# microsoft/tf2-gnn

Measured on AMD Instinct MI355X. Metric: edges/sec (fwd+bwd) RGCN H=320 L=4, PPI-shaped batch, 1/2/4/8 MI355X, higher is better.
Workload: dtype f32; 1 GPU; rmat30k: V=30000 E=900000 per GPU (one batch per rank, replicas) edge_types=4 D=320 H=320 layers=4 RGCN (PPI_RGCN.json stack settings), step = edge bucketing of the next batch (2nd stream, overlapped) + forward (training mode) + f...

## Files before the change

include/tfgnn.h:

```cpp
#ifndef TFGNN_H
#define TFGNN_H

#include <stddef.h>
#include <stdint.h>

#ifdef __cplusplus
extern "C" {
#endif

typedef enum {
  TFGNN_OK = 0,
  TFGNN_ERR_INVALID_ARGUMENT = -1,
  TFGNN_ERR_OUT_OF_RANGE = -2,
  TFGNN_ERR_HIP = -3,
  TFGNN_ERR_UNSUPPORTED = -4
} tfgnn_status;

typedef enum {
  TFGNN_ACT_NONE = 0,
  TFGNN_ACT_RELU = 1,
  TFGNN_ACT_TANH = 2,
  TFGNN_ACT_LEAKY_RELU = 3,
  TFGNN_ACT_ELU = 4,
  TFGNN_ACT_SELU = 5,
// ... 2 lines not shown
} tfgnn_activation;

typedef enum {
  TFGNN_REDUCE_SUM = 0,
  TFGNN_REDUCE_MAX = 1
} tfgnn_reduce;

const char* tfgnn_last_error(void);
const char* tfgnn_version(void);
#define TFGNN_ABI_VERSION 5
int tfgnn_abi_version(void);

typedef enum {
  TFGNN_KFAM_GEMM_FP32 = 0,
  TFGNN_KFAM_GEMM_BF16X3 = 1,
  TFGNN_KFAM_SP_NT = 2,
  TFGNN_KFAM_SP_TN = 3,
  TFGNN_KFAM_GATHER_SP = 4,
  TFGNN_KFAM_GATHER = 5,
  TFGNN_KFAM_FUSED_NT = 6,
  TFGNN_KFAM_GEMM_STREAM = 7,
  TFGNN_KFAM_STREAM_F16X2 = 8,
  TFGNN_KFAM_COUNT = 9
} tfgnn_kernel_family;
int tfgnn_launch_counts(int64_t* out_counts, int n);

typedef struct tfgnn_graph tfgnn_graph;

int tfgnn_graph_create(int num_edge_types, int64_t num_nodes, const int32_t* const* d_adjacency,
                       const int64_t* num_edges, void* stream, tfgnn_graph** out_graph);
int tfgnn_graph_destroy(tfgnn_graph* graph);
int tfgnn_graph_create_async(int num_edge_types, int64_t num_nodes, const int32_t* const* d_adjacency,
                             const int64_t* num_edges, void* stream, tfgnn_graph** out_graph);
int tfgnn_graph_wait(tfgnn_graph* graph);
int tfgnn_graph_destroy_async(tfgnn_graph* graph, void* last_use_stream);

typedef enum {
  TFGNN_GRAPH_PART_PLAN_TYPED = 1,
  TFGNN_GRAPH_PART_PLAN_NODE = 2,
  TFGNN_GRAPH_PART_COMPACT = 4,
  TFGNN_GRAPH_PART_EDGE_MAPS = 8,
  TFGNN_GRAPH_PART_EDGE_IDS = 16,
  TFGNN_GRAPH_PART_DST_PATTERN = 32,
  TFGNN_GRAPH_PARTS_DEFAULT = 31,
  TFGNN_GRAPH_PARTS_ALL = 63
} tfgnn_graph_part;
int tfgnn_graph_create_parts_async(int num_edge_types, int64_t num_nodes, const int32_t* const* d_adjacency,
                                   const int64_t* num_edges, unsigned parts, void* stream, tfgnn_graph** out_graph);
int tfgnn_graph_ensure(tfgnn_graph* graph, unsigned parts, void* stream);
unsigned tfgnn_graph_parts(const tfgnn_graph* graph);

typedef enum {
  TFGNN_G_ROWPTR_BY_DST = 0,
  TFGNN_G_COL_BY_DST = 1,
  TFGNN_G_EID_BY_DST = 2,
  TFGNN_G_COLL_BY_DST = 3,
  TFGNN_G_ROWPTR_BY_SRC = 4,
  TFGNN_G_COL_BY_SRC = 5,
  TFGNN_G_EID_BY_SRC = 6,
  TFGNN_G_COLL_BY_SRC = 7,
  TFGNN_G_INVDEG_BY_DST = 8,
  TFGNN_G_INVDEG_EDGE_BY_SRC = 9,
  TFGNN_G_NODEPTR_BY_DST = 10,
  TFGNN_G_NODEPTR_BY_SRC = 11,
  TFGNN_G_INVDEG_EDGE_BY_DST = 12,
  TFGNN_G_SRC2DST_POS = 13,
  TFGNN_G_TARGET_BY_DST = 14,
  TFGNN_G_NZ_CPOS_BY_DST = 15,
  TFGNN_G_NZ_ROW_BY_DST = 16,
  TFGNN_G_NZ_NODE_BY_DST = 17,
  TFGNN_G_NZ_OFF_BY_DST = 18,
  TFGNN_G_NZ_NODEPTR_BY_DST = 19,
  TFGNN_G_NZ_COL_BY_DST = 20,
  TFGNN_G_NZ_CPOS_BY_SRC = 21,
  TFGNN_G_NZ_ROW_BY_SRC = 22,
  TFGNN_G_NZ_NODE_BY_SRC = 23,
  TFGNN_G_NZ_OFF_BY_SRC = 24,
  TFGNN_G_NZ_NODEPTR_BY_SRC = 25,
  TFGNN_G_NZ_COL_BY_SRC = 26,
  TFGNN_G_PATTERN_POS_BY_DST = 27,
  TFGNN_G_PATTERN_NODE_BY_DST = 28,
  TFGNN_G_PATTERN_TILEMASK_BY_DST = 29,
  TFGNN_G_PATTERN_NODE_BY_SRC = 30,
  TFGNN_G_PATTERN_TILEMASK_BY_SRC = 31
} tfgnn_graph_array_id;

int tfgnn_graph_array(const tfgnn_graph* graph, int array_id, const void** d_ptr, int64_t* count);
int tfgnn_graph_nonempty_offsets(const tfgnn_graph* graph, int by_src, int32_t* h_offsets);
int tfgnn_graph_dims(const tfgnn_graph* graph, int64_t* num_nodes, int* num_edge_types,
                     int64_t* num_edges);

int tfgnn_graph_scales(const tfgnn_graph* graph, int normalize_by_num_incoming, int aggregation_mode,
                       float* d_row_scale, float* d_node_scale, float* d_edge_weight_by_src,
                       float* d_edge_weight_by_dst, void* stream);

int tfgnn_graph_target_multiplier(const tfgnn_graph* graph, const float* d_row_scale, float* d_k,
                                  int32_t* d_ident_ptr, int32_t* d_node_of_row, void* stream);

int tfgnn_csr_gather_reduce(const int32_t* d_rowptr, const int32_t* d_col,
                            const float* d_edge_weight, const float* d_row_scale,
                            int64_t num_rows, const float* d_in, int64_t ld_in, int width,
                            float* d_out, int64_t ld_out, int reduce_op, int pre_act, int post_act,
                            void* stream);

typedef enum {
  TFGNN_VIEW_BY_DST_TYPED = 0,
  TFGNN_VIEW_BY_DST_NODE = 1,
  TFGNN_VIEW_BY_SRC_TYPED = 2,
  TFGNN_VIEW_BY_SRC_NODE = 3,
  TFGNN_VIEW_BY_DST_TYPED_COMPACT = 4,
  TFGNN_VIEW_BY_SRC_TYPED_COMPACT = 5,
  TFGNN_VIEW_BY_DST_TYPED_PATTERN = 6
} tfgnn_graph_view;
size_t tfgnn_graph_gather_workspace_bytes(const tfgnn_graph* graph, int view, int width);
int tfgnn_graph_gather_reduce(const tfgnn_graph* graph, int view, const int32_t* d_col_override,
                              const float* d_edge_weight, int ew_heads, const float* d_row_scale,
                              const float* d_in, int64_t ld_in, int width, float* d_out, int64_t ld_out,
                              int reduce_op, int pre_act, int post_act, void* d_workspace,
                              size_t workspace_bytes, void* stream);

int tfgnn_edge_pair_combine(const int32_t* d_index_a, const int32_t* d_index_b, const float* d_P,
                            const float* d_Q, int64_t num_edges, int width, int act, float* d_out,
                            void* stream);

int tfgnn_film_edge_forward(const float* d_msg, const int32_t* d_msg_row, const float* d_film, const int32_t* d_film_row,
                            const float* d_edge_weight, int64_t num_edges, int width, float* d_out, void* stream);
int tfgnn_film_edge_backward(const float* d_grad, const float* d_msg, const int32_t* d_msg_row, const float* d_film,
                             const int32_t* d_film_row, const float* d_edge_weight, int64_t num_edges, int width,
                             float* d_grad_msg, float* d_grad_film, void* stream);

int tfgnn_edge_aggregate_backward(int64_t num_edges, int64_t width, const float* d_msg, int64_t ld_msg,
                                  const int32_t* d_msg_row, const int32_t* d_target, const float* d_edge_weight,
                                  const float* d_node_scale, int pre_act, int reduce_op, const float* d_grad_agg,
                                  const float* d_agg_max, const float* d_num_selected, int phase, float* d_out,
                                  void* stream);

int tfgnn_film_combine_forward(const float* d_Z, const float* d_film, const int32_t* d_rowptr_typed,
                               const float* d_node_scale, int64_t num_nodes, int num_edge_types, int64_t hidden,
                               int act, float* d_pre, float* d_out, void* stream);
int tfgnn_film_combine_backward(const float* d_grad_pre, const float* d_Z, const float* d_film,
                                const int32_t* d_rowptr_typed, const float* d_node_scale, int64_t num_nodes,
                                int num_edge_types, int64_t hidden, float* d_dZ, float* d_dfilm, void* stream);

int tfgnn_batch_offset_edges(const int32_t* d_local_edges, int64_t num_edges, const int32_t* d_edge_ptr,
                             const int32_t* d_node_ptr, int num_graphs, int32_t* d_out, int* d_bad_flag, void* stream);
int tfgnn_batch_node_to_graph_map(const int32_t* d_node_ptr, int num_graphs, int64_t num_nodes, int32_t* d_out,
                                  void* stream);
int tfgnn_adjacency_append(const int32_t* d_edges, int64_t num_edges, int flip, int32_t* d_out, void* stream);
int tfgnn_adjacency_self_loops(int64_t num_nodes, int32_t* d_out, void* stream);
int tfgnn_adjacency_in_degrees(const int32_t* d_edges, int64_t num_edges, int64_t num_nodes, float* d_counts,
                               void* stream);
int tfgnn_graph_original_order(const tfgnn_graph* graph, const float* d_weight_by_dst, int32_t* d_src_l,
                               int32_t* d_tgt_l, int32_t* d_tgt_node, float* d_weight, void* stream);

size_t tfgnn_gemm_workspace_bytes(int64_t M, int64_t N, int64_t K);
int tfgnn_gemm(int trans_a, int trans_b, int64_t M, int64_t N, int64_t K, const float* d_A,
               int64_t lda, const float* d_B, int64_t ldb, float* d_C, int64_t ldc,
               const float* d_bias, int act, int accumulate, void* d_workspace,
               size_t workspace_bytes, void* stream);

enum { TFGNN_GEMM_FP32 = 0, TFGNN_GEMM_F16X2 = 3, TFGNN_GEMM_BF16X3 = 6, TFGNN_GEMM_BF16X3_EXACT = 9 };
int tfgnn_gemm_set_mode(int mode);
int tfgnn_gemm_get_mode(void);

int tfgnn_gemm_grad_epilogue(int trans_a, int trans_b, int64_t M, int64_t N, int64_t K, const float* d_A,
                             int64_t lda, const float* d_B, int64_t ldb, float* d_C, int64_t ldc,
                             const float* d_mul, int64_t ld_mul, int act_of_saved, const float* d_saved,
// ... 422 lines not shown
```

tf2_gnn_amd/csrc/aux_jobs.hip:

```cpp
#include <algorithm>

#include "aux_jobs.hpp"

namespace tfgnn {

constexpr int AUX_MAX_JOBS = 8;
struct AuxJobTable {
  tfgnn_aux_job j[AUX_MAX_JOBS];
  int n;
};

typedef const __attribute__((address_space(4))) tfgnn_aux_job* aux_job_cptr;

template <class P>
__device__ __forceinline__ P aux_payload(aux_job_cptr j) {
  constexpr int W = (int)((sizeof(P) + 7) / 8);
  union {
    P p;
    unsigned long long w[W];
  } u;
  const __attribute__((address_space(4))) unsigned long long* src =
      (const __attribute__((address_space(4))) unsigned long long*)&j->payload[0];
#pragma unroll
  for (int i = 0; i < W; ++i) u.w[i] = src[i];
  return u.p;
}

__global__ void __launch_bounds__(256) aux_jobs_kernel(AuxJobTable table) {
  aux_job_cptr jobs = (aux_job_cptr)__builtin_amdgcn_kernarg_segment_ptr();
  unsigned b = blockIdx.x;
  int k = 0;
  const int n = table.n;
  while (k < n - 1 && b >= jobs[k].num_blocks) {
    b -= jobs[k].num_blocks;
    ++k;
  }
  aux_job_cptr j = jobs + k;
  const unsigned nb = j->num_blocks;
  if (b >= nb) return;
  switch (j->kind) {
    case AUX_SPLIT_ROWS: {
      const AuxSplitRows a = aux_payload<AuxSplitRows>(j);
      sp_split_rows_body(a.src, a.ld, a.seg_len, a.seg_stride, a.R, a.C, a.sb, a.dst, a.ld_dst, a.inv, a.fixed_inv, b);
      break;
    }
    case AUX_SPLIT_COLS: {
      const AuxSplitCols a = aux_payload<AuxSplitCols>(j);
      sp_split_cols_body(a.src, a.ld, a.K, a.N, a.dst, a.ld_dst, a.inv, b % a.ncx, b / a.ncx, a.ncy, a.colmax_parts, a.nparts);
      break;
    }
    case AUX_COL_ABSMAX: {
      const AuxColAbsmax a = aux_payload<AuxColAbsmax>(j);
      col_absmax_body(a, b);
      break;
    }
    case AUX_COMBINE_SP: {
      const AuxCombineSp a = aux_payload<AuxCombineSp>(j);
      combine_sp_body(a, b);
      break;
    }
    default:
      break;
  }
}

}

extern "C" int tfgnn_aux_launch(const tfgnn_aux_job* jobs, int num_jobs, void* stream) {
  using namespace tfgnn;
  TFGNN_REQUIRE(num_jobs >= 0 && (num_jobs == 0 || jobs != nullptr), "tfgnn_aux_launch: bad arguments");
  int i = 0;
  while (i < num_jobs) {
    AuxJobTable t{};
    uint64_t blocks = 0;
    while (i < num_jobs && t.n < AUX_MAX_JOBS) {
      const tfgnn_aux_job& j = jobs[i++];
      if (j.kind == AUX_NONE || j.num_blocks == 0) continue;
      TFGNN_REQUIRE(j.kind == AUX_SPLIT_ROWS || j.kind == AUX_SPLIT_COLS || j.kind == AUX_COMBINE_SP || j.kind == AUX_COL_ABSMAX,
                    "tfgnn_aux_launch: unknown job kind %d", j.kind);
      t.j[t.n++] = j;
      blocks += j.num_blocks;
    }
    if (t.n == 0) continue;
    TFGNN_REQUIRE(blocks < (1ull << 31), "tfgnn_aux_launch: too many workgroups");
    hipLaunchKernelGGL(aux_jobs_kernel, dim3((unsigned)blocks), dim3(256), 0, (hipStream_t)stream, t);
    TFGNN_LAUNCH_CHECK();
  }
  return TFGNN_OK;
}
```

tf2_gnn_amd/csrc/aux_jobs.hpp:

```cpp
#pragma once
#include <hip/hip_runtime.h>

#include <cstdint>

#include "common.hpp"
#include "sp16.hpp"
#include "tfgnn.h"

namespace tfgnn {

enum AuxKind { AUX_NONE = 0, AUX_SPLIT_ROWS = 1, AUX_SPLIT_COLS = 2, AUX_COMBINE_SP = 4, AUX_COL_ABSMAX = 6 };

struct AuxSplitRows {
  const float* src;
  int64_t ld, seg_len, seg_stride, R, C;
  int sb;
  uint8_t* dst;
  int64_t ld_dst;
  float* inv;
  const float* fixed_inv;
};
struct AuxSplitCols {
  const float* src;
  int64_t ld, K, N;
  uint8_t* dst;
  int64_t ld_dst;
  float* inv;
  unsigned ncx, ncy;
  const float* colmax_parts;
  int nparts;
};
struct AuxColAbsmax {
  const float* src;
  int64_t ld, K, N;
  float* part;
  int nparts;
  unsigned nchunks;
};
static_assert(sizeof(AuxColAbsmax) <= sizeof(((tfgnn_aux_job*)0)->payload), "tfgnn_aux_job payload too small");
struct AuxTnReduce {
  const float* partial;
  int splits;
  int64_t M, N;
  const float* ref;
  int64_t a_col0;
  int a_sb;
  float* C;
  int64_t group_rows, stride_group, stride_row, stride_col;
  int accumulate;
  int64_t slab;
  int ref_ld;
};
struct AuxCombineSp {
  const int32_t *multi_row, *multi_base, *multi_n;
  int num_multi;
  const float* row_scale;
  const float* partial;
  int width;
  const int32_t* out_row_map;
  uint8_t* out_sp;
  int64_t ld_out_sp;
  float* inv_out;
  const float* fixed_inv;
};
static_assert(sizeof(AuxSplitRows) <= sizeof(((tfgnn_aux_job*)0)->payload) && sizeof(AuxSplitCols) <= sizeof(((tfgnn_aux_job*)0)->payload) &&
                  sizeof(AuxCombineSp) <= sizeof(((tfgnn_aux_job*)0)->payload),
              "tfgnn_aux_job payload too small");

template <class P>
static inline void aux_job_set(tfgnn_aux_job* j, int kind, unsigned blocks, const P& p) {
  j->kind = kind;
  j->num_blocks = blocks;
  memset(j->payload, 0, sizeof(j->payload));
  memcpy(j->payload, &p, sizeof(P));
}

__device__ __forceinline__ void sp_split_rows_body(const float* __restrict__ src, int64_t ld, int64_t seg_len,
                                                   int64_t seg_stride, int64_t R, int64_t C, int sb,
                                                   uint8_t* __restrict__ dst, int64_t ld_dst, float* __restrict__ inv,
                                                   const float* __restrict__ fixed_inv, unsigned block) {
  const int lane = threadIdx.x & 63;
  const int nblk = (int)(C / sb);
  const int64_t item = (int64_t)block * 4 + (threadIdx.x >> 6);
  if (item >= R * nblk) return;
  const int64_t r = item / nblk;
  const int blk = (int)(item - r * nblk);
  const float* srow = src + r * ld;
  const int64_t c0 = (int64_t)blk * sb;
  float s, iv;
  if (fixed_inv) {
    iv = fixed_inv[0];
    s = 1.f / iv;
  } else {
    float mx = 0.f;
    for (int c = lane * 4; c < sb; c += 256) {
      const int64_t cc = c0 + c;
      const int64_t sg = cc / seg_len;
      const float4 v = *reinterpret_cast<const float4*>(srow + sg * seg_stride + (cc - sg * seg_len));
      mx = fmaxf(mx, fmaxf(fmaxf(fabsf(v.x), fabsf(v.y)), fmaxf(fabsf(v.z), fabsf(v.w))));
    }
    for (int o = 32; o; o >>= 1) mx = fmaxf(mx, __shfl_xor(mx, o, 64));
    s = sp_scale_for_max(mx, &iv);
  }
  if (inv && lane == 0) inv[item] = iv;
  uint8_t* drow = dst + r * ld_dst;
  for (int c = lane * 4; c < sb; c += 256) {
    const int64_t cc = c0 + c;
    const int64_t sg = cc / seg_len;
    const float4 v = *reinterpret_cast<const float4*>(srow + sg * seg_stride + (cc - sg * seg_len));
    sp_store4(drow, cc, v, s);
  }
}

__device__ __forceinline__ void col_absmax_body(const AuxColAbsmax& a, unsigned block) {
  const unsigned s = block / a.nchunks, chunk = block - s * a.nchunks;
  const int64_t per = (a.K + a.nparts - 1) / a.nparts;
  const int64_t k0 = (int64_t)s * per, k1 = k0 + per < a.K ? k0 + per : a.K;
  const int64_t c = ((int64_t)chunk * 256 + threadIdx.x) * 4;
  if (c >= a.N) return;
  const float* p = a.src + c;
  float4 mx = {0.f, 0.f, 0.f, 0.f};
  int64_t k = k0;
  for (; k + 8 <= k1; k += 8) {
    float4 v[8];
#pragma unroll
    for (int u = 0; u < 8; ++u) v[u] = *reinterpret_cast<const float4*>(p + (k + u) * a.ld);
#pragma unroll
    for (int u = 0; u < 8; ++u) {
      mx.x = fmaxf(mx.x, fabsf(v[u].x)); mx.y = fmaxf(mx.y, fabsf(v[u].y));
      mx.z = fmaxf(mx.z, fabsf(v[u].z)); mx.w = fmaxf(mx.w, fabsf(v[u].w));
    }
  }
  for (; k < k1; ++k) {
    const float4 v = *reinterpret_cast<const float4*>(p + k * a.ld);
    mx.x = fmaxf(mx.x, fabsf(v.x)); mx.y = fmaxf(mx.y, fabsf(v.y));
    mx.z = fmaxf(mx.z, fabsf(v.z)); mx.w = fmaxf(mx.w, fabsf(v.w));
  }
  *reinterpret_cast<float4*>(a.part + (int64_t)s * a.N + c) = mx;
}

__device__ __forceinline__ void sp_split_cols_body(const float* __restrict__ src, int64_t ld, int64_t K, int64_t N,
                                                   uint8_t* __restrict__ dst, int64_t ld_dst, float* __restrict__ inv,
                                                   unsigned bx, unsigned by, unsigned ny, const float* __restrict__ colmax_parts = nullptr,
                                                   int nparts = 0) {
  __shared__ float red[64][4];
  __shared__ float tile[2][16][65];
  __shared__ float sc[16];
  const int tid = threadIdx.x;
  const int64_t n0 = (int64_t)bx * 16;
// ... 45 lines not shown
    float* r = &red[(tid >> 6) * 4 + (tid & 3)][0];
    r[0] = mx.x; r[1] = mx.y; r[2] = mx.z; r[3] = mx.w;
  }
  __syncthreads();
  if (tid < 16) {
    float m = 0.f;
#pragma unroll
    for (int w = 0; w < 4; ++w) m = fmaxf(m, red[w * 4 + (tid >> 2)][tid & 3]);
    float iv;
    sc[tid] = sp_scale_for_max(m, &iv);
    if (inv && by == 0 && n0 + tid < N) inv[n0 + tid] = iv;
  }
  __syncthreads();
  const int64_t kper = (((K + ny - 1) / ny) + 63) & ~63ll;
  const int64_t kend = (by + 1) * kper < K ? (by + 1) * kper : K;
  const int rr = tid >> 4, k4 = (tid & 15) * 4;
  if (in_regs) {
    const int i0 = (int)((by * kper) >> 6), i1 = (int)((kend + 63) >> 6);
#pragma unroll
    for (int i = 0; i < NV; ++i) {
      if (i >= i0 && i < i1) {
        float (*t)[65] = tile[i & 1];
        t[nq + 0][kq] = v[i].x; t[nq + 1][kq] = v[i].y; t[nq + 2][kq] = v[i].z; t[nq + 3][kq] = v[i].w;
        __syncthreads();
        const int64_t kb = (int64_t)i * 64;
        if (n0 + rr < N && kb + k4 < K) {
          const float4 o = {t[rr][k4], t[rr][k4 + 1], t[rr][k4 + 2], t[rr][k4 + 3]};
          sp_store4(dst + (n0 + rr) * ld_dst, kb + k4, o, sc[rr]);
        }
      }
    }
    return;
  }
  for (int64_t kb = by * kper; kb < kend; kb += 64) {
    const int64_t k = kb + kq;
    float4 w4 = {0.f, 0.f, 0.f, 0.f};
    if (ok && k < K) w4 = *reinterpret_cast<const float4*>(src + k * ld + n0 + nq);
    tile[0][nq + 0][kq] = w4.x; tile[0][nq + 1][kq] = w4.y; tile[0][nq + 2][kq] = w4.z; tile[0][nq + 3][kq] = w4.w;
    __syncthreads();
    if (n0 + rr < N && kb + k4 < K) {
      const float4 o = {tile[0][rr][k4], tile[0][rr][k4 + 1], tile[0][rr][k4 + 2], tile[0][rr][k4 + 3]};
      sp_store4(dst + (n0 + rr) * ld_dst, kb + k4, o, sc[rr]);
    }
    __syncthreads();
  }
}

__device__ __forceinline__ void sp_tn_reduce_body(const AuxTnReduce& a, unsigned block, unsigned nblocks) {
  const int64_t total = a.M * a.N;
  for (int64_t i = (int64_t)block * 256 + threadIdx.x; i < total; i += (int64_t)nblocks * 256) {
    const int64_t m = i / a.N, n = i - m * a.N;
    const int64_t blk = (a.a_col0 + m) / a.a_sb;
    float s = 0.f;
    int z = 0;
    if (a.ref_ld > 0) {
      for (; z + 8 <= a.splits; z += 8) {
        float v[8], r[8];
#pragma unroll
        for (int u = 0; u < 8; ++u) {
          v[u] = a.partial[(int64_t)(z + u) * a.slab + i];
          r[u] = a.ref[(int64_t)(z + u) * a.ref_ld + blk];
        }
#pragma unroll
        for (int u = 0; u < 8; ++u) s += v[u] * r[u];
      }
      for (; z < a.splits; ++z) s += a.partial[(int64_t)z * a.slab + i] * a.ref[(int64_t)z * a.ref_ld + blk];
    } else {
      for (; z + 8 <= a.splits; z += 8) {
        float v[8];
#pragma unroll
        for (int u = 0; u < 8; ++u) v[u] = a.partial[(int64_t)(z + u) * a.slab + i];
#pragma unroll
        for (int u = 0; u < 8; ++u) s += v[u];
      }
      for (; z < a.splits; ++z) s += a.partial[(int64_t)z * a.slab + i];
      s *= a.ref[blk];
    }
    const int64_t gi = m / a.group_rows, mi = m - gi * a.group_rows;
    float* dst = a.C + gi * a.stride_group + mi * a.stride_row + n * a.stride_col;
    *dst = a.accumulate ? *dst + s : s;
  }
}

__device__ __forceinline__ void combine_sp_body(const AuxCombineSp& a, unsigned block) {
  const int m = (int)block * 4 + (threadIdx.x >> 6);
  if (m >= a.num_multi) return;
  const int lane = threadIdx.x & 63;
  const int64_t row = a.multi_row[m];
  const int32_t base = a.multi_base[m], n = a.multi_n[m];
  const float rs = a.row_scale ? a.row_scale[row] : 1.f;
  float4 sum[8];
  float mx = 0.f;
#pragma unroll
  for (int i = 0; i < 8; ++i) {
    const int c = (lane + i * 64) * 4;
    sum[i] = make_float4(0.f, 0.f, 0.f, 0.f);
    if (c < a.width) {
      int k = 0;
      for (; k + 4 <= n; k += 4) {
        float4 p[4];
#pragma unroll
        for (int u = 0; u < 4; ++u) p[u] = *reinterpret_cast<const float4*>(a.partial + (int64_t)(base + k + u) * a.width + c);
#pragma unroll
        for (int u = 0; u < 4; ++u) { sum[i].x += p[u].x; sum[i].y += p[u].y; sum[i].z += p[u].z; sum[i].w += p[u].w; }
      }
      for (; k < n; ++k) {
        const float4 p = *reinterpret_cast<const float4*>(a.partial + (int64_t)(base + k) * a.width + c);
        sum[i].x += p.x; sum[i].y += p.y; sum[i].z += p.z; sum[i].w += p.w;
      }
      sum[i].x *= rs; sum[i].y *= rs; sum[i].z *= rs; sum[i].w *= rs;
      mx = fmaxf(mx, fmaxf(fmaxf(fabsf(sum[i].x), fabsf(sum[i].y)), fmaxf(fabsf(sum[i].z), fabsf(sum[i].w))));
    }
  }
  const int64_t orow = a.out_row_map ? a.out_row_map[row] : row;
  float iv, sc;
  if (a.fixed_inv) {
    iv = a.fixed_inv[0];
    sc = 1.f / iv;
  } else {
#pragma unroll
    for (int o = 32; o; o >>= 1) mx = fmaxf(mx, __shfl_xor(mx, o, 64));
    sc = sp_scale_for_max(mx, &iv);
    if (lane == 0) a.inv_out[orow] = iv;
  }
  uint8_t* drow = a.out_sp + orow * a.ld_out_sp;
#pragma unroll
  for (int i = 0; i < 8; ++i) {
    const int c = (lane + i * 64) * 4;
    if (c < a.width) sp_store4(drow, c, sum[i], sc);
  }
}

}
```

tf2_gnn_amd/csrc/graph.hip:

```cpp
#include <algorithm>
#include <cstdlib>
#include <mutex>
#include <vector>

#include "common.hpp"
#include "graph.hpp"

namespace tfgnn {

static thread_local char g_err[512] = "";

void set_error(const char* fmt, ...) {
  va_list ap;
  va_start(ap, fmt);
  vsnprintf(g_err, sizeof(g_err), fmt, ap);
  va_end(ap);
}

static int64_t g_launch_counts[TFGNN_KFAM_COUNT] = {0};
void count_launch(int family) {
  if (family >= 0 && family < TFGNN_KFAM_COUNT) __atomic_fetch_add(&g_launch_counts[family], 1, __ATOMIC_RELAXED);
}

}
// ... 243 lines not shown
    if (valid && rank == 0) mine_base[d] = mine_base[d] + cnt;
    __builtin_amdgcn_wave_barrier();
  }
  __syncthreads();
  int32_t tot = 0, before = 0;
  {
    const int32_t* __restrict__ row = hist + (int64_t)(side * RS_RADIX + tid) * nblk_ld;
    const int me = (int)blockIdx.x;
    for (int b0 = 0; b0 < nblk; b0 += 16) {
      int4 v[4];
#pragma unroll
      for (int u = 0; u < 4; ++u)
        v[u] = b0 + 4 * u < nblk ? *reinterpret_cast<const int4*>(row + b0 + 4 * u) : make_int4(0, 0, 0, 0);
#pragma unroll
      for (int u = 0; u < 4; ++u) {
        const int b = b0 + 4 * u;
        const int e[4] = {v[u].x, v[u].y, v[u].z, v[u].w};
#pragma unroll
        for (int k = 0; k < 4; ++k)
          if (b + k < nblk) {
            tot += e[k];
            if (b + k < me) before += e[k];
          }
      }
    }
  }
  int32_t incl = tot;
#pragma unroll
  for (int o = 1; o < 64; o <<= 1) {
    const int32_t t = __shfl_up(incl, o, 64);
    if (lane >= o) incl += t;
  }
  if (lane == 63) wtot[wave] = incl;
  __syncthreads();
  {
    int32_t off = 0;
    for (int w = 0; w < wave; ++w) off += wtot[w];
    int32_t running = off + incl - tot + before;
#pragma unroll
    for (int w = 0; w < RS_WAVES; ++w) {
      const int32_t c = wbase[w][tid];
      wbase[w][tid] = running;
      running += c;
    }
  }
  __syncthreads();
#pragma unroll
  for (int r = 0; r < RS_ROUNDS; ++r) {
    const bool valid = (info[r] >> 16) & 1;
    const int d = (int)((key[r] >> shift) & (RS_RADIX - 1));
    const int rank = info[r] & 255, cnt = (info[r] >> 8) & 255;
    const int32_t b = valid ? mine_base[d] : 0;
    __builtin_amdgcn_wave_barrier();
    if (valid && rank == 0) mine_base[d] = b + cnt;
    __builtin_amdgcn_wave_barrier();
    if (valid) {
      kout[b + rank] = key[r];
      if (PAY) pout[b + rank] = pl[r];
    }
  }
}

template <typename KeyT>
__global__ void rowptr_from_sorted_kernel(const KeyT* __restrict__ comp_d, const KeyT* __restrict__ comp_s, int64_t E,
                                          int sec_bits, int64_t R, int32_t* __restrict__ rowptr_d,
                                          int32_t* __restrict__ rowptr_s) {
  const KeyT* __restrict__ comp = blockIdx.y ? comp_s : comp_d;
  int32_t* __restrict__ rowptr = blockIdx.y ? rowptr_s : rowptr_d;
  for (int64_t r = (int64_t)blockIdx.x * blockDim.x + threadIdx.x; r <= R; r += (int64_t)gridDim.x * blockDim.x) {
    int64_t lo = 0, hi = E;
    while (lo < hi) {
      const int64_t mid = (lo + hi) >> 1;
      if ((int64_t)((uint64_t)comp[mid] >> sec_bits) < r) lo = mid + 1; else hi = mid;
    }
    rowptr[r] = (int32_t)lo;
  }
}

struct PlanJob {
  const int32_t* rowptr;
  int64_t R;
  int thr, chunk;
  int32_t* counters;
  int32_t *item_row, *item_chunk, *item_slot, *multi_row, *multi_base, *multi_n;
  int32_t *bin_count, *bin_cursor, *short_rows;
  int want_items;
};
struct PlanJobs {
  PlanJob j[2];
};

__device__ __forceinline__ void plan_rows_body(const int32_t* __restrict__ rowptr, int64_t R, int long_threshold, int chunk_edges,
                                 int32_t* __restrict__ counters,
                                 int32_t* __restrict__ item_row, int32_t* __restrict__ item_chunk,
                                 int32_t* __restrict__ item_slot, int32_t* __restrict__ multi_row,
                                 int32_t* __restrict__ multi_base, int32_t* __restrict__ multi_n) {
  for (int64_t r = (int64_t)blockIdx.x * blockDim.x + threadIdx.x; r < R; r += (int64_t)gridDim.x * blockDim.x) {
    const int32_t len = rowptr[r + 1] - rowptr[r];
    if (len <= long_threshold) continue;
    const int32_t n = (len + chunk_edges - 1) / chunk_edges;
    const int32_t base = atomicAdd(&counters[0], n);
    int32_t pb = -1;
    if (n > 1) {
      const int32_t m = atomicAdd(&counters[1], 1);
      pb = atomicAdd(&counters[2], n);
      multi_row[m] = (int32_t)r;
      multi_base[m] = pb;
      multi_n[m] = n;
    }
    for (int32_t i = 0; i < n; ++i) {
      item_row[base + i] = (int32_t)r;
      item_chunk[base + i] = i;
      item_slot[base + i] = n > 1 ? pb + i : -1;
    }
  }
}

__device__ __forceinline__ void
short_hist_body(const int32_t* __restrict__ rowptr, int64_t R, int thr, int32_t* __restrict__ bin_count,
                int32_t* __restrict__ num_short, int* h, int& n_short) {
  for (int i = threadIdx.x; i <= thr; i += 256) h[i] = 0;
  if (threadIdx.x == 0) n_short = 0;
  __syncthreads();
  int mine = 0;
  for (int64_t r = (int64_t)blockIdx.x * blockDim.x + threadIdx.x; r < R; r += (int64_t)gridDim.x * blockDim.x) {
    const int32_t len = rowptr[r + 1] - rowptr[r];
    if (len <= thr) {
      atomicAdd(&h[len], 1);
      ++mine;
    }
  }
  if (mine) atomicAdd(&n_short, mine);
  __syncthreads();
  for (int i = threadIdx.x; i <= thr; i += 256)
    if (h[i]) atomicAdd(&bin_count[i], h[i]);
  if (threadIdx.x == 0 && n_short) atomicAdd(num_short, n_short);
}

__global__ void __launch_bounds__(256) plan_hist_kernel(PlanJobs jobs) {
  __shared__ int h[SHORT_BINS];
  __shared__ int n_short;
  const PlanJob& j = jobs.j[blockIdx.y & 1];
  if (j.R <= 0) return;
  if ((blockIdx.y >> 1) == 0) {
    short_hist_body(j.rowptr, j.R, j.thr, j.bin_count, j.counters + 3, h, n_short);
  } else if (j.want_items) {
    plan_rows_body(j.rowptr, j.R, j.thr, j.chunk, j.counters, j.item_row, j.item_chunk, j.item_slot, j.multi_row, j.multi_base,
                   j.multi_n);
  }
}

constexpr int SHORT_TILE_ROWS = 8;
__global__ void __launch_bounds__(256) short_scatter_kernel(PlanJobs jobs) {
  __shared__ int h[SHORT_BINS], base[SHORT_BINS], start[SHORT_BINS];
  const PlanJob& j = jobs.j[blockIdx.y];
  const int32_t* __restrict__ rowptr = j.rowptr;
  const int64_t R = j.R;
  const int thr = j.thr;
  const int32_t* __restrict__ bin_count = j.bin_count;
  int32_t* __restrict__ bin_cursor = j.bin_cursor;
  int32_t* __restrict__ short_rows = j.short_rows;
  if (R <= 0) return;
  if (threadIdx.x == 0) {
    int acc = 0;
    for (int i = thr; i >= 0; --i) {
      start[i] = acc;
      acc += bin_count[i];
    }
  }
  constexpr int TILE = 256 * SHORT_TILE_ROWS;
  for (int64_t tile = blockIdx.x; tile * TILE < R; tile += gridDim.x) {
    for (int i = threadIdx.x; i <= thr; i += 256) h[i] = 0;
    __syncthreads();
    int32_t len[SHORT_TILE_ROWS];
    int rank[SHORT_TILE_ROWS];
#pragma unroll
    for (int k = 0; k < SHORT_TILE_ROWS; ++k) {
      const int64_t r = tile * TILE + k * 256 + threadIdx.x;
      len[k] = r < R ? rowptr[r + 1] - rowptr[r] : -1;
      rank[k] = (len[k] >= 0 && len[k] <= thr) ? atomicAdd(&h[len[k]], 1) : 0;
    }
    __syncthreads();
    for (int i = threadIdx.x; i <= thr; i += 256)
      if (h[i]) base[i] = atomicAdd(&bin_cursor[i], h[i]);
    __syncthreads();
#pragma unroll
    for (int k = 0; k < SHORT_TILE_ROWS; ++k)
      if (len[k] >= 0 && len[k] <= thr)
        short_rows[start[len[k]] + base[len[k]] + rank[k]] = (int32_t)(tile * TILE + k * 256 + threadIdx.x);
    __syncthreads();
  }
}

__global__ void nz_flags_kernel(const int32_t* __restrict__ rowptr, int64_t V, int L, int32_t* __restrict__ flags,
                                int32_t* __restrict__ node_cnt) {
  const int64_t R = V * L;
  for (int64_t i = (int64_t)blockIdx.x * blockDim.x + threadIdx.x; i <= R; i += (int64_t)gridDim.x * blockDim.x) {
    if (i < R) {
      const int64_t l = i / V, v = i - l * V;
      const int64_t r = v * L + l;
      flags[i] = rowptr[r + 1] > rowptr[r] ? 1 : 0;
    } else {
      flags[i] = 0;
    }
    if (i <= V) {
      int32_t c = 0;
      if (i < V)
        for (int l = 0; l < L; ++l) c += rowptr[i * L + l + 1] > rowptr[i * L + l] ? 1 : 0;
      node_cnt[i] = c;
    }
  }
}

__global__ void nz_fill_kernel(const int32_t* __restrict__ rowptr, const int32_t* __restrict__ scan_t, int64_t V,
                               int L, int32_t* __restrict__ cpos, int32_t* __restrict__ nzrow,
                               int32_t* __restrict__ nz_node, int32_t* __restrict__ nz_off) {
  const int64_t R = V * L;
  for (int64_t i = (int64_t)blockIdx.x * blockDim.x + threadIdx.x; i < R; i += (int64_t)gridDim.x * blockDim.x) {
    const int64_t l = i / V, v = i - l * V;
    const int64_t r = v * L + l;
    const int32_t c = scan_t[i];
    if (rowptr[r + 1] > rowptr[r]) {
      cpos[r] = c;
      nzrow[c] = (int32_t)r;
      nz_node[c] = (int32_t)v;
    } else {
      cpos[r] = -1;
    }
    if (v == 0) nz_off[l] = c;
    if (i == R - 1) nz_off[L] = scan_t[R];
  }
// ... 179 lines not shown
  }
  {
    std::lock_guard<std::mutex> lock(g_pool_mutex);
    if (g_dev_pool.size() < POOL_MAX_ENTRIES) {
      g_dev_pool.push_back({p, bytes, ev});
      return;
    }
  }
  if (ev) (void)hipEventDestroy(ev);
  (void)hipFree(p);
}
static hipError_t pinned_alloc(void** p, size_t bytes, size_t* got) {
  if (bytes < 4096) bytes = 4096;
  *p = pool_take(g_pinned_pool, bytes, got, nullptr);
  if (*p) return hipSuccess;
  *got = bytes;
  return hipHostMalloc(p, bytes, hipHostMallocDefault);
}
static void pinned_release(void* p, size_t bytes) {
  if (!p) return;
  {
    std::lock_guard<std::mutex> lock(g_pool_mutex);
    if (g_pinned_pool.size() < POOL_MAX_ENTRIES) {
      g_pinned_pool.push_back({p, bytes, nullptr});
      return;
    }
  }
  (void)hipHostFree(p);
}
}

namespace {
struct SlabPlan {
  size_t total = 0;
  size_t take(size_t bytes) {
    size_t off = total;
    total += (bytes + 255) & ~(size_t)255;
    return off;
  }
};
}

static void graph_release_all(tfgnn_graph* g, hipStream_t last_use = nullptr, bool in_use = false) {
  using namespace tfgnn;
  if (!g) return;
  if (g->event) (void)hipEventDestroy((hipEvent_t)g->event);
  dev_release(g->scratch, g->scratch_bytes, last_use, in_use);
  dev_release(g->slab, g->slab_bytes, last_use, in_use);
  pinned_release(g->pinned, g->pinned_bytes);
  delete g;
}

namespace {
using namespace tfgnn;

constexpr unsigned kPartsAll = TFGNN_GRAPH_PART_PLAN_TYPED | TFGNN_GRAPH_PART_PLAN_NODE | TFGNN_GRAPH_PART_COMPACT |
                               TFGNN_GRAPH_PART_EDGE_MAPS | TFGNN_GRAPH_PART_EDGE_IDS | TFGNN_GRAPH_PART_DST_PATTERN;

void view_plan_parameters(int view_long[4], int view_chunk[4]) {
  const int dl[4] = {LONG_ROW_THRESHOLD_TYPED, LONG_ROW_THRESHOLD, LONG_ROW_THRESHOLD_TYPED, LONG_ROW_THRESHOLD};
  const int dc[4] = {ITEM_CHUNK_TYPED, ITEM_CHUNK, ITEM_CHUNK_TYPED, ITEM_CHUNK};
  for (int v = 0; v < 4; ++v) {
    view_long[v] = dl[v];
    view_chunk[v] = dc[v];
    if (view_long[v] > SHORT_BINS - 1) view_long[v] = SHORT_BINS - 1;
    if (view_chunk[v] < view_long[v]) view_chunk[v] = view_long[v];
  }
}

unsigned blocks_for(int64_t n) { return (unsigned)std::max<int64_t>(1, std::min<int64_t>(ceil_div(n, 256), 8192)); }

int build_plans(tfgnn_graph* g, int node_views, int32_t* counters, int32_t* bins, hipStream_t s) {
  PlanJobs jobs{};
  int64_t max_rows = 0;
  for (int k = 0; k < 2; ++k) {
    const int v = 2 * k + node_views;
    CsrPlan& pl = g->views[v].plan;
    PlanJob& j = jobs.j[k];
    j.rowptr = g->views[v].rowptr;
    j.R = g->views[v].num_rows;
    j.thr = pl.long_threshold;
    j.chunk = pl.item_chunk_edges;
    j.counters = counters + 16 + 4 * v;
    j.item_row = pl.item_row; j.item_chunk = pl.item_chunk; j.item_slot = pl.item_slot;
    j.multi_row = pl.multi_row; j.multi_base = pl.multi_base; j.multi_n = pl.multi_n;
    j.bin_count = bins + (size_t)v * 2 * SHORT_BINS;
    j.bin_cursor = j.bin_count + SHORT_BINS;
    j.short_rows = pl.short_rows;
    j.want_items = g->E > 0;
    max_rows = std::max(max_rows, j.R);
  }
  if (max_rows <= 0) return TFGNN_OK;
  hipLaunchKernelGGL(plan_hist_kernel, dim3(blocks_for(max_rows), 4), dim3(256), 0, s, jobs);
  TFGNN_LAUNCH_CHECK();
  const unsigned scat_blocks = (unsigned)std::min<int64_t>(ceil_div(max_rows, 256 * SHORT_TILE_ROWS), 4096);
  hipLaunchKernelGGL(short_scatter_kernel, dim3(scat_blocks, 2), dim3(256), 0, s, jobs);
  TFGNN_LAUNCH_CHECK();
  return TFGNN_OK;
}

size_t compact_scratch_bytes(int64_t R, int64_t V) {
  return (size_t)(R + 2) * 4 + 256 + (scan_scratch_elems(R + 1) + scan_scratch_elems(V + 1)) * 4 + 64;
}

int build_compact(tfgnn_graph* g, char* scratch, hipStream_t s) {
  const int L = g->L;
  const int64_t V = g->V, R = g->R;
  int32_t* flags = (int32_t*)scratch;
  int32_t* scan_tmp = (int32_t*)(scratch + (((size_t)(R + 2) * 4 + 255) & ~(size_t)255));
  for (int side = 0; side < 2; ++side) {
    CompactBuckets& cb = g->compact[side];
    const int32_t* rp = side == 0 ? g->rowptr_d : g->rowptr_s;
    if (L > 0) {
      hipLaunchKernelGGL(nz_flags_kernel, dim3(blocks_for(R + 1)), dim3(256), 0, s, rp, V, L, flags, cb.nodeptr_nz);
      int rc = exclusive_scan_i32(flags, flags, R + 1, scan_tmp, s);
      if (rc) return rc;
      rc = exclusive_scan_i32(cb.nodeptr_nz, cb.nodeptr_nz, V + 1, scan_tmp, s);
      if (rc) return rc;
      if (R > 0) {
        hipLaunchKernelGGL(nz_fill_kernel, dim3(blocks_for(R)), dim3(256), 0, s, rp, flags, V, L, cb.cpos, cb.nzrow,
                           cb.nz_node, cb.nz_off);
        hipLaunchKernelGGL(nz_cols_kernel, dim3(blocks_for(V)), dim3(256), 0, s, cb.cpos, cb.nodeptr_nz, V, L, cb.col_nz);
      } else {
        TFGNN_HIP_CHECK(hipMemsetAsync(cb.nz_off, 0, (size_t)(L + 1) * 4, s));
      }
    } else {
      TFGNN_HIP_CHECK(hipMemsetAsync(cb.nz_off, 0, (size_t)(L + 1) * 4, s));
      TFGNN_HIP_CHECK(hipMemsetAsync(cb.nodeptr_nz, 0, (V + 1) * 4, s));
    }
    TFGNN_HIP_CHECK(hipMemcpyAsync((char*)g->pinned + 256 + (size_t)(L + 1) * 16 + (size_t)side * (L + 1) * 4, cb.nz_off,
                                   (size_t)(L + 1) * 4, hipMemcpyDeviceToHost, s));
  }
  TFGNN_LAUNCH_CHECK();
  return TFGNN_OK;
}

int build_dst_pattern(tfgnn_graph* g, int32_t* pat, hipStream_t s) {
  if (g->V <= 0 || g->L <= 0 || g->L > 8) return TFGNN_OK;
  const unsigned blocks = (unsigned)std::min<int64_t>(ceil_div(g->V, 256), 1024);
  hipLaunchKernelGGL(pattern_count_kernel, dim3(blocks), dim3(256), 0, s, (const int32_t*)g->rowptr_d, g->V, g->L, pat);
  hipLaunchKernelGGL(pattern_place_kernel, dim3(blocks), dim3(256), 0, s, (const int32_t*)g->rowptr_d, g->V, g->L, (const int32_t*)pat,
                     pat + 256, g->pat_pos_d, g->pat_node_d, g->pat_rowmap_d);
  hipLaunchKernelGGL(pattern_tilemask_kernel, dim3((unsigned)ceil_div(g->V, 128)), dim3(128), 0, s, (const int32_t*)g->rowptr_d,
                     (const int32_t*)g->pat_node_d, g->V, g->L, g->pat_tilemask_d);
  int32_t* pat_s = pat + 512;
  hipLaunchKernelGGL(pattern_count_kernel, dim3(blocks), dim3(256), 0, s, (const int32_t*)g->rowptr_s, g->V, g->L, pat_s);
  hipLaunchKernelGGL(pattern_place_kernel, dim3(blocks), dim3(256), 0, s, (const int32_t*)g->rowptr_s, g->V, g->L, (const int32_t*)pat_s,
                     pat_s + 256, (int32_t*)nullptr, g->pat_node_s, (int32_t*)nullptr);
  hipLaunchKernelGGL(pattern_tilemask_kernel, dim3((unsigned)ceil_div(g->V, 128)), dim3(128), 0, s, (const int32_t*)g->rowptr_s,
                     (const int32_t*)g->pat_node_s, g->V, g->L, g->pat_tilemask_s);
  TFGNN_LAUNCH_CHECK();
  return TFGNN_OK;
}

int build_edge_maps(tfgnn_graph* g, hipStream_t s) {
  if (g->E > 0) {
    hipLaunchKernelGGL(src2dst_kernel, dim3(blocks_for(g->E)), dim3(256), 0, s, g->eid_s, g->eid2pos, g->E, g->src2dst, g->dst2src);
    TFGNN_LAUNCH_CHECK();
  }
  return TFGNN_OK;
}

template <typename KeyT, bool PAY>
int build_core(tfgnn_graph* g, const EdgeLists& el, char* keys, char* pays, int32_t* hist, int nblk, int nblk_ld,
               int32_t* counters, hipStream_t s) {
  const int64_t E = g->E, R = g->R, V = g->V;
  const int L = g->L;
  const int sec_bits = g->sec_bits, total_bits = g->total_bits;
// ... 58 lines not shown
    for (int l = 0; l < EL_INLINE; ++l) el.adj_v[l] = l < L ? g->h_adj[l] : nullptr;
    for (int l = 0; l <= EL_INLINE; ++l) el.off_v[l] = l <= L ? g->h_off[l] : g->E;
  } else {
    const int32_t** d_ptrs = (const int32_t**)(scratch + cs.ptrs);
    int64_t* d_off = (int64_t*)(scratch + cs.off);
    char* hp = (char*)g->pinned + 256;
    const int32_t** h_ptrs = (const int32_t**)hp;
    int64_t* h_off = (int64_t*)(hp + (size_t)(L + 1) * 8);
    for (int l = 0; l < L; ++l) h_ptrs[l] = g->h_adj[l];
    for (int l = 0; l <= L; ++l) h_off[l] = g->h_off[l];
    TFGNN_HIP_CHECK(hipMemcpyAsync(d_ptrs, h_ptrs, (size_t)L * 8, hipMemcpyHostToDevice, s));
    TFGNN_HIP_CHECK(hipMemcpyAsync(d_off, h_off, (size_t)(L + 1) * 8, hipMemcpyHostToDevice, s));
    el.adj = d_ptrs;
    el.edge_off = d_off;
  }
  char* keys = scratch + cs.keys;
  char* pays = scratch + cs.pays;
  int32_t* hist = (int32_t*)(scratch + cs.hist);
  int32_t* counters = (int32_t*)(scratch + cs.counters);
  if (g->total_bits <= 32)
    return pay ? build_core<uint32_t, true>(g, el, keys, pays, hist, cs.nblk, cs.nblk_ld, counters, s)
               : build_core<uint32_t, false>(g, el, keys, pays, hist, cs.nblk, cs.nblk_ld, counters, s);
  return pay ? build_core<uint64_t, true>(g, el, keys, pays, hist, cs.nblk, cs.nblk_ld, counters, s)
             : build_core<uint64_t, false>(g, el, keys, pays, hist, cs.nblk, cs.nblk_ld, counters, s);
}
}

static int graph_create_impl(int num_edge_types, int64_t num_nodes, const int32_t* const* d_adjacency,
                             const int64_t* num_edges, unsigned parts, void* stream, tfgnn_graph** out_graph) {
  using namespace tfgnn;
  TFGNN_REQUIRE(out_graph != nullptr, "out_graph is NULL");
  *out_graph = nullptr;
  TFGNN_REQUIRE(num_edge_types >= 0 && num_nodes >= 0, "negative sizes");
  TFGNN_REQUIRE(num_edge_types == 0 || (d_adjacency && num_edges), "adjacency arrays are NULL");
  TFGNN_REQUIRE((parts & ~kPartsAll) == 0, "unknown graph part bits 0x%x", parts);
  hipStream_t s = (hipStream_t)stream;
  (void)dropout_epoch_word();
  const int L = num_edge_types;
  const int64_t V = num_nodes;
  std::vector<int64_t> edge_off(L + 1, 0);
  for (int l = 0; l < L; ++l) {
    TFGNN_REQUIRE(num_edges[l] >= 0, "num_edges[%d] < 0", l);
    TFGNN_REQUIRE(num_edges[l] == 0 || d_adjacency[l] != nullptr, "adjacency list %d is NULL", l);
    edge_off[l + 1] = edge_off[l] + num_edges[l];
  }
  const int64_t E = edge_off[L];
  const int64_t R = V * (int64_t)L;
  TFGNN_REQUIRE(R < ((int64_t)1 << 31) - 1 && E < ((int64_t)1 << 31) - 1,
                "graph too large for int32 indexing (V*L=%lld, E=%lld)", (long long)R, (long long)E);
  TFGNN_REQUIRE(L <= 256, "at most 256 edge types are supported (got %d)", L);

  tfgnn_graph* g = new tfgnn_graph();
  g->L = L;
  g->V = V;
  g->E = E;
  g->R = R;

  SlabPlan plan;
  const size_t o_rowptr_d = plan.take((R + 1) * 4), o_rowptr_s = plan.take((R + 1) * 4);
  const size_t o_col_d = plan.take(E * 4), o_eid_d = plan.take(E * 4), o_coll_d = plan.take(E * 4);
  const size_t o_col_s = plan.take(E * 4), o_eid_s = plan.take(E * 4), o_coll_s = plan.take(E * 4);
  const size_t o_nodeptr_d = plan.take((V + 1) * 4), o_nodeptr_s = plan.take((V + 1) * 4);
  const size_t o_src2dst = plan.take(E * 4), o_dst2src = plan.take(E * 4);
  const size_t o_tgt_d = plan.take(E * 4), o_eid2pos = plan.take(E * 4);
  const size_t o_pat_pos = plan.take((V + 1) * 4), o_pat_node = plan.take((V + 1) * 4), o_pat_rowmap = plan.take((R + 1) * 4);
  const size_t o_pat_mask = plan.take((size_t)ceil_div(V > 0 ? V : 1, 128) + 16);
  const size_t o_pat_node_s = plan.take((V + 1) * 4), o_pat_mask_s = plan.take((size_t)ceil_div(V > 0 ? V : 1, 128) + 16);
  const size_t o_invdeg_d = plan.take((R + 1) * 4);
  const size_t o_invdeg_es = plan.take(E * 4), o_invdeg_ed = plan.take(E * 4);
  size_t o_cb[2][6];
  for (int side = 0; side < 2; ++side) {
    o_cb[side][0] = plan.take((R + 1) * 4);
    o_cb[side][1] = plan.take((R + 1) * 4);
    o_cb[side][2] = plan.take((R + 1) * 4);
    o_cb[side][3] = plan.take((size_t)(L + 1) * 4);
    o_cb[side][4] = plan.take((V + 1) * 4);
    o_cb[side][5] = plan.take((R + 1) * 4);
  }
  int view_long[4], view_chunk[4];
  view_plan_parameters(view_long, view_chunk);
  const int min_long = std::min(std::min(view_long[0], view_long[1]), std::min(view_long[2], view_long[3]));
  const int min_chunk = std::min(std::min(view_chunk[0], view_chunk[1]), std::min(view_chunk[2], view_chunk[3]));
  const size_t max_items = (size_t)(E / min_long + 1), max_multi = (size_t)(E / min_chunk + 1);
  size_t o_item[4][3], o_multi[4][3];
  for (int v = 0; v < 4; ++v) {
    for (int k = 0; k < 3; ++k) o_item[v][k] = plan.take(max_items * 4);
    for (int k = 0; k < 3; ++k) o_multi[v][k] = plan.take(max_multi * 4);
  }
  size_t o_short[4];
  for (int v = 0; v < 4; ++v) o_short[v] = plan.take((size_t)((v & 1) ? V : R) * 4 + 4);
  const size_t persistent = plan.total;
  if (parts & TFGNN_GRAPH_PART_EDGE_MAPS) parts |= TFGNN_GRAPH_PART_EDGE_IDS;
  const bool with_ids = (parts & TFGNN_GRAPH_PART_EDGE_IDS) != 0;
  const CoreScratch cs = core_scratch(E, L, with_ids);
  const size_t t_compact = (cs.total + 255) & ~(size_t)255;
  const size_t scratch_total = t_compact + ((parts & TFGNN_GRAPH_PART_COMPACT) ? compact_scratch_bytes(R, V) : 0);
  g->h_adj.assign(d_adjacency, d_adjacency + L);
  g->h_off = edge_off;
  {
    int sec_bits = 1;
    while (((int64_t)1 << sec_bits) < V) ++sec_bits;
    int row_bits = 1;
    while (((int64_t)1 << row_bits) < (R > 0 ? R : 1)) ++row_bits;
    g->sec_bits = sec_bits;
    g->total_bits = sec_bits + row_bits;
  }

  char* slab = nullptr;
  char* scratch = nullptr;
  const size_t pinned_need = 256 + (size_t)(L + 1) * 16 + (size_t)(L + 1) * 8;
  hipError_t he = dev_alloc((void**)&slab, persistent, &g->slab_bytes, s);
  if (he == hipSuccess) {
    g->slab = slab;
    he = dev_alloc((void**)&scratch, scratch_total, &g->scratch_bytes, s);
  }
  if (he == hipSuccess) {
    g->scratch = scratch;
    he = pinned_alloc(&g->pinned, pinned_need, &g->pinned_bytes);
  }
  if (he == hipSuccess) {
    hipEvent_t ev;
    he = hipEventCreateWithFlags(&ev, hipEventDisableTiming);
    if (he == hipSuccess) g->event = ev;
  }
  if (he != hipSuccess) {
    set_error("graph allocation failed (%zu + %zu bytes): %s", persistent, scratch_total, hipGetErrorString(he));
    graph_release_all(g);
    return TFGNN_ERR_HIP;
  }
  g->slab = slab;
  g->rowptr_d = (int32_t*)(slab + o_rowptr_d);
  g->rowptr_s = (int32_t*)(slab + o_rowptr_s);
  g->col_d = (int32_t*)(slab + o_col_d);
  g->eid_d = (int32_t*)(slab + o_eid_d);
  g->coll_d = (int32_t*)(slab + o_coll_d);
  g->col_s = (int32_t*)(slab + o_col_s);
  g->eid_s = (int32_t*)(slab + o_eid_s);
  g->coll_s = (int32_t*)(slab + o_coll_s);
  g->nodeptr_d = (int32_t*)(slab + o_nodeptr_d);
  g->nodeptr_s = (int32_t*)(slab + o_nodeptr_s);
  g->src2dst = (int32_t*)(slab + o_src2dst);
  g->dst2src = (int32_t*)(slab + o_dst2src);
  g->tgt_d = (int32_t*)(slab + o_tgt_d);
  g->eid2pos = (int32_t*)(slab + o_eid2pos);
  g->pat_pos_d = (int32_t*)(slab + o_pat_pos);
  g->pat_node_d = (int32_t*)(slab + o_pat_node);
  g->pat_rowmap_d = (int32_t*)(slab + o_pat_rowmap);
  g->pat_tilemask_d = (uint8_t*)(slab + o_pat_mask);
  g->pat_node_s = (int32_t*)(slab + o_pat_node_s);
  g->pat_tilemask_s = (uint8_t*)(slab + o_pat_mask_s);
  g->invdeg_d = (float*)(slab + o_invdeg_d);
  g->invdeg_edge_s = (float*)(slab + o_invdeg_es);
  g->invdeg_edge_d = (float*)(slab + o_invdeg_ed);
  for (int side = 0; side < 2; ++side) {
    CompactBuckets& cb = g->compact[side];
    cb.cpos = (int32_t*)(slab + o_cb[side][0]);
    cb.nzrow = (int32_t*)(slab + o_cb[side][1]);
    cb.nz_node = (int32_t*)(slab + o_cb[side][2]);
    cb.nz_off = (int32_t*)(slab + o_cb[side][3]);
    cb.nodeptr_nz = (int32_t*)(slab + o_cb[side][4]);
    cb.col_nz = (int32_t*)(slab + o_cb[side][5]);
  }
  g->views[0].rowptr = g->rowptr_d;  g->views[0].num_rows = R; g->views[0].col = g->col_d;
  g->views[1].rowptr = g->nodeptr_d; g->views[1].num_rows = V; g->views[1].col = g->coll_d;
  g->views[2].rowptr = g->rowptr_s;  g->views[2].num_rows = R; g->views[2].col = g->col_s;
  g->views[3].rowptr = g->nodeptr_s; g->views[3].num_rows = V; g->views[3].col = g->coll_s;
  for (int v = 0; v < 4; ++v) {
    CsrPlan& pl = g->views[v].plan;
    pl.item_row = (int32_t*)(slab + o_item[v][0]);
    pl.item_chunk = (int32_t*)(slab + o_item[v][1]);
    pl.item_slot = (int32_t*)(slab + o_item[v][2]);
    pl.multi_row = (int32_t*)(slab + o_multi[v][0]);
    pl.multi_base = (int32_t*)(slab + o_multi[v][1]);
    pl.multi_n = (int32_t*)(slab + o_multi[v][2]);
    pl.long_threshold = view_long[v];
    pl.item_chunk_edges = view_chunk[v];
    pl.short_rows = (int32_t*)(slab + o_short[v]);
  }

  int32_t* counters = (int32_t*)(scratch + cs.counters);
  int32_t* bins = counters + 64;

  int rc = TFGNN_OK;
  auto fail = [&](int code) {
    (void)hipStreamSynchronize(s);
    graph_release_all(g);
    return code;
  };
#define G_CHECK(expr)                                                                          \
  do {                                                                                         \
    hipError_t _e = (expr);                                                                    \
    if (_e != hipSuccess) {                                                                    \
      set_error("%s failed: %s (%s:%d)", #expr, hipGetErrorString(_e), __FILE__, __LINE__);    \
      return fail(TFGNN_ERR_HIP);                                                              \
    }                                                                                          \
  } while (0)

  G_CHECK(hipMemsetAsync(counters, 0, (size_t)(64 + 4 * 2 * SHORT_BINS + 1024) * 4, s));
  if (E > 0) {
    rc = run_core(g, with_ids, scratch, cs, s);
    if (rc) return fail(rc);
  } else {
    G_CHECK(hipMemsetAsync(g->rowptr_d, 0, (R + 1) * 4, s));
    G_CHECK(hipMemsetAsync(g->rowptr_s, 0, (R + 1) * 4, s));
    if (L > 0) {
      hipLaunchKernelGGL((unpack_kernel<uint32_t, false>), dim3(blocks_for(R + 1), 1), dim3(256), 0, s, (const uint32_t*)nullptr,
                         (const uint32_t*)nullptr, (const uint32_t*)nullptr, (const uint32_t*)nullptr, 0, (int64_t)0, L, R,
                         (const int32_t*)g->rowptr_d, (const int32_t*)g->rowptr_s, g->col_d, g->eid_d, g->coll_d, g->invdeg_edge_d,
                         g->eid2pos, g->tgt_d, g->col_s, g->eid_s, g->coll_s, g->invdeg_edge_s, g->invdeg_d, g->nodeptr_d,
                         g->nodeptr_s, 2);
    } else {
      G_CHECK(hipMemsetAsync(g->nodeptr_d, 0, (V + 1) * 4, s));
      G_CHECK(hipMemsetAsync(g->nodeptr_s, 0, (V + 1) * 4, s));
    }
  }
  if (parts & TFGNN_GRAPH_PART_PLAN_TYPED) {
    rc = build_plans(g, 0, counters, bins, s);
    if (rc) return fail(rc);
  }
  if (parts & TFGNN_GRAPH_PART_PLAN_NODE) {
    rc = build_plans(g, 1, counters, bins, s);
    if (rc) return fail(rc);
  }
  if (parts & TFGNN_GRAPH_PART_EDGE_MAPS) {
    rc = build_edge_maps(g, s);
    if (rc) return fail(rc);
  }
  if (parts & TFGNN_GRAPH_PART_DST_PATTERN) {
    rc = build_dst_pattern(g, bins + 4 * 2 * SHORT_BINS, s);
    if (rc) return fail(rc);
  }
  if (parts & TFGNN_GRAPH_PART_COMPACT) {
    rc = build_compact(g, scratch + t_compact, s);
    if (rc) return fail(rc);
  }
  {
    hipError_t le = hipGetLastError();
    if (le != hipSuccess) {
      set_error("graph build kernel launch failed: %s", hipGetErrorString(le));
      return fail(TFGNN_ERR_HIP);
    }
  }
  G_CHECK(hipMemcpyAsync(g->pinned, counters, 64 * 4, hipMemcpyDeviceToHost, s));
  G_CHECK(hipEventRecord((hipEvent_t)g->event, s));
#undef G_CHECK
  g->parts = parts;
  g->pending = true;
  *out_graph = g;
  return TFGNN_OK;
}

extern "C" int tfgnn_graph_create_async(int num_edge_types, int64_t num_nodes, const int32_t* const* d_adjacency,
                                        const int64_t* num_edges, void* stream, tfgnn_graph** out_graph) {
  return graph_create_impl(num_edge_types, num_nodes, d_adjacency, num_edges, TFGNN_GRAPH_PARTS_DEFAULT, stream, out_graph);
// ... 136 lines not shown
    if (r < R) {
      const float c = (float)(rowptr_d[r + 1] - rowptr_d[r]);
      k[r] = row_scale ? c * row_scale[r] : c;
      node_of_row[r] = (int32_t)(r / L);
    }
  }
}
}

extern "C" int tfgnn_graph_scales(const tfgnn_graph* g, int normalize_by_num_incoming, int aggregation_mode,
                                  float* d_row_scale, float* d_node_scale, float* d_edge_weight_by_src,
                                  float* d_edge_weight_by_dst, void* stream) {
  using namespace tfgnn;
  TFGNN_REQUIRE(g != nullptr, "graph is NULL");
  TFGNN_REQUIRE(aggregation_mode >= 0 && aggregation_mode <= 2, "unknown aggregation mode %d", aggregation_mode);
  const int64_t R = g->R, E = g->E;
  const int64_t n = R > E ? R : E;
  if (n == 0) return TFGNN_OK;
  TFGNN_REQUIRE((R == 0 || (d_row_scale && d_node_scale)) && (E == 0 || (d_edge_weight_by_src && d_edge_weight_by_dst)),
                "NULL output");
  unsigned blocks = (unsigned)std::min<int64_t>(ceil_div(n, 256), 8192);
  hipLaunchKernelGGL(graph_scales_kernel, dim3(blocks), dim3(256), 0, (hipStream_t)stream, g->nodeptr_d,
                     g->invdeg_d, g->invdeg_edge_s, g->invdeg_edge_d, g->col_s, g->V, g->L, E,
                     normalize_by_num_incoming, aggregation_mode, d_row_scale, d_node_scale,
                     d_edge_weight_by_src, d_edge_weight_by_dst);
  TFGNN_LAUNCH_CHECK();
  return TFGNN_OK;
}

extern "C" int tfgnn_graph_target_multiplier(const tfgnn_graph* g, const float* d_row_scale, float* d_k,
                                             int32_t* d_ident_ptr, int32_t* d_node_of_row, void* stream) {
  using namespace tfgnn;
  TFGNN_REQUIRE(g != nullptr && d_ident_ptr != nullptr, "NULL argument");
  TFGNN_REQUIRE(g->R == 0 || (d_k && d_node_of_row), "NULL output");
  unsigned blocks = (unsigned)std::min<int64_t>(ceil_div(g->R + 1, 256), 8192);
  hipLaunchKernelGGL(target_multiplier_kernel, dim3(blocks), dim3(256), 0, (hipStream_t)stream, g->rowptr_d,
                     d_row_scale, g->R, g->L > 0 ? g->L : 1, d_k, d_ident_ptr, d_node_of_row);
  TFGNN_LAUNCH_CHECK();
  return TFGNN_OK;
}

extern "C" int tfgnn_graph_destroy(tfgnn_graph* graph) {
  if (!graph) return TFGNN_OK;
  (void)hipDeviceSynchronize();
  graph_release_all(graph);
  return TFGNN_OK;
}

extern "C" int tfgnn_graph_destroy_async(tfgnn_graph* graph, void* last_use_stream) {
  if (!graph) return TFGNN_OK;
  if (graph->pending) (void)hipEventSynchronize((hipEvent_t)graph->event);
  graph_release_all(graph, (hipStream_t)last_use_stream, true);
  return TFGNN_OK;
}

extern "C" int tfgnn_graph_nonempty_offsets(const tfgnn_graph* g, int by_src, int32_t* h_offsets) {
  TFGNN_REQUIRE(g != nullptr && h_offsets != nullptr, "NULL argument");
  TFGNN_REQUIRE(!g->pending, "tfgnn_graph_wait has not been called");
  {
    const int rc = tfgnn::graph_require_parts(g, TFGNN_GRAPH_PART_COMPACT, "tfgnn_graph_nonempty_offsets");
    if (rc) return rc;
  }
  for (int l = 0; l <= g->L; ++l) h_offsets[l] = g->compact[by_src ? 1 : 0].h_nz_off[l];
  return TFGNN_OK;
}

extern "C" int tfgnn_graph_dims(const tfgnn_graph* g, int64_t* num_nodes, int* num_edge_types,
                                int64_t* num_edges) {
  TFGNN_REQUIRE(g != nullptr, "graph is NULL");
  if (num_nodes) *num_nodes = g->V;
  if (num_edge_types) *num_edge_types = g->L;
  if (num_edges) *num_edges = g->E;
  return TFGNN_OK;
}

extern "C" int tfgnn_graph_array(const tfgnn_graph* g, int array_id, const void** d_ptr, int64_t* count) {
  TFGNN_REQUIRE(g != nullptr && d_ptr != nullptr && count != nullptr, "NULL argument");
  {
    unsigned need = 0;
    if (array_id == TFGNN_G_SRC2DST_POS) need = TFGNN_GRAPH_PART_EDGE_MAPS;
    if (array_id == TFGNN_G_EID_BY_DST || array_id == TFGNN_G_EID_BY_SRC) need = TFGNN_GRAPH_PART_EDGE_IDS;
    if (array_id >= TFGNN_G_PATTERN_POS_BY_DST && array_id <= TFGNN_G_PATTERN_TILEMASK_BY_SRC) need = TFGNN_GRAPH_PART_DST_PATTERN;
    if (array_id >= TFGNN_G_NZ_CPOS_BY_DST && array_id <= TFGNN_G_NZ_COL_BY_SRC) need = TFGNN_GRAPH_PART_COMPACT;
    if (need) {
      const int rc = tfgnn::graph_require_parts(g, need, "tfgnn_graph_array");
      if (rc) return rc;
    }
  }
  switch (array_id) {
    case TFGNN_G_ROWPTR_BY_DST: *d_ptr = g->rowptr_d; *count = g->R + 1; break;
    case TFGNN_G_COL_BY_DST: *d_ptr = g->col_d; *count = g->E; break;
    case TFGNN_G_EID_BY_DST: *d_ptr = g->eid_d; *count = g->E; break;
    case TFGNN_G_COLL_BY_DST: *d_ptr = g->coll_d; *count = g->E; break;
    case TFGNN_G_ROWPTR_BY_SRC: *d_ptr = g->rowptr_s; *count = g->R + 1; break;
    case TFGNN_G_COL_BY_SRC: *d_ptr = g->col_s; *count = g->E; break;
    case TFGNN_G_EID_BY_SRC: *d_ptr = g->eid_s; *count = g->E; break;
    case TFGNN_G_COLL_BY_SRC: *d_ptr = g->coll_s; *count = g->E; break;
    case TFGNN_G_INVDEG_BY_DST: *d_ptr = g->invdeg_d; *count = g->R; break;
    case TFGNN_G_INVDEG_EDGE_BY_SRC: *d_ptr = g->invdeg_edge_s; *count = g->E; break;
    case TFGNN_G_NODEPTR_BY_DST: *d_ptr = g->nodeptr_d; *count = g->V + 1; break;
    case TFGNN_G_NODEPTR_BY_SRC: *d_ptr = g->nodeptr_s; *count = g->V + 1; break;
    case TFGNN_G_INVDEG_EDGE_BY_DST: *d_ptr = g->invdeg_edge_d; *count = g->E; break;
    case TFGNN_G_SRC2DST_POS: *d_ptr = g->src2dst; *count = g->E; break;
    case TFGNN_G_TARGET_BY_DST: *d_ptr = g->tgt_d; *count = g->E; break;
    case TFGNN_G_PATTERN_POS_BY_DST: *d_ptr = g->L <= 8 ? g->pat_pos_d : nullptr; *count = g->L <= 8 ? g->V : 0; break;
    case TFGNN_G_PATTERN_NODE_BY_DST: *d_ptr = g->L <= 8 ? g->pat_node_d : nullptr; *count = g->L <= 8 ? g->V : 0; break;
    case TFGNN_G_PATTERN_TILEMASK_BY_DST: *d_ptr = g->L <= 8 ? (const void*)g->pat_tilemask_d : nullptr; *count = g->L <= 8 ? ceil_div(g->V, 128) : 0; break;
    case TFGNN_G_PATTERN_NODE_BY_SRC: *d_ptr = g->L <= 8 ? g->pat_node_s : nullptr; *count = g->L <= 8 ? g->V : 0; break;
    case TFGNN_G_PATTERN_TILEMASK_BY_SRC: *d_ptr = g->L <= 8 ? (const void*)g->pat_tilemask_s : nullptr; *count = g->L <= 8 ? ceil_div(g->V, 128) : 0; break;
    case TFGNN_G_NZ_CPOS_BY_DST: case TFGNN_G_NZ_CPOS_BY_SRC:
      *d_ptr = g->compact[array_id >= TFGNN_G_NZ_CPOS_BY_SRC].cpos; *count = g->R; break;
    case TFGNN_G_NZ_ROW_BY_DST: case TFGNN_G_NZ_ROW_BY_SRC:
      *d_ptr = g->compact[array_id >= TFGNN_G_NZ_CPOS_BY_SRC].nzrow; *count = g->compact[array_id >= TFGNN_G_NZ_CPOS_BY_SRC].num_nz; break;
    case TFGNN_G_NZ_NODE_BY_DST: case TFGNN_G_NZ_NODE_BY_SRC:
      *d_ptr = g->compact[array_id >= TFGNN_G_NZ_CPOS_BY_SRC].nz_node; *count = g->compact[array_id >= TFGNN_G_NZ_CPOS_BY_SRC].num_nz; break;
    case TFGNN_G_NZ_OFF_BY_DST: case TFGNN_G_NZ_OFF_BY_SRC:
      *d_ptr = g->compact[array_id >= TFGNN_G_NZ_CPOS_BY_SRC].nz_off; *count = g->L + 1; break;
    case TFGNN_G_NZ_NODEPTR_BY_DST: case TFGNN_G_NZ_NODEPTR_BY_SRC:
      *d_ptr = g->compact[array_id >= TFGNN_G_NZ_CPOS_BY_SRC].nodeptr_nz; *count = g->V + 1; break;
    case TFGNN_G_NZ_COL_BY_DST: case TFGNN_G_NZ_COL_BY_SRC:
      *d_ptr = g->compact[array_id >= TFGNN_G_NZ_CPOS_BY_SRC].col_nz; *count = g->compact[array_id >= TFGNN_G_NZ_CPOS_BY_SRC].num_nz; break;
    default:
      tfgnn::set_error("unknown graph array id %d", array_id);
      return TFGNN_ERR_INVALID_ARGUMENT;
  }
  return TFGNN_OK;
}
```

tf2_gnn_amd/csrc/graph.hpp:

```cpp
#pragma once
#include <cstddef>
#include <cstdint>
#include <vector>

namespace tfgnn {

constexpr int LONG_ROW_THRESHOLD = 32;
constexpr int ITEM_CHUNK = 512;
constexpr int LONG_ROW_THRESHOLD_TYPED = 48;
constexpr int ITEM_CHUNK_TYPED = 512;

struct CsrPlan {
  int32_t long_threshold = LONG_ROW_THRESHOLD;
  int32_t item_chunk_edges = ITEM_CHUNK;
  int32_t num_items = 0;
  int32_t num_multi = 0;
  int32_t num_partials = 0;
  int32_t* item_row = nullptr;
  int32_t* item_chunk = nullptr;
  int32_t* item_slot = nullptr;
  int32_t* multi_row = nullptr;
  int32_t* multi_base = nullptr;
  int32_t* multi_n = nullptr;
  int32_t* short_rows = nullptr;
  int32_t num_short = 0;
};
constexpr int SHORT_BINS = 257;

struct CompactBuckets {
  int32_t num_nz = 0;
  int32_t* cpos = nullptr;
  int32_t* nzrow = nullptr;
  int32_t* nz_node = nullptr;
  int32_t* nz_off = nullptr;
  int32_t* nodeptr_nz = nullptr;
  int32_t* col_nz = nullptr;
  int32_t h_nz_off[257] = {0};
};

struct GraphView {
  const int32_t* rowptr = nullptr;
  int64_t num_rows = 0;
  const int32_t* col = nullptr;
  CsrPlan plan;
};

}

struct tfgnn_graph {
  int L = 0;
  int64_t V = 0, E = 0, R = 0;
  void* slab = nullptr;
  int32_t *rowptr_d = nullptr, *col_d = nullptr, *eid_d = nullptr, *coll_d = nullptr;
  int32_t *rowptr_s = nullptr, *col_s = nullptr, *eid_s = nullptr, *coll_s = nullptr;
  int32_t *nodeptr_d = nullptr, *nodeptr_s = nullptr, *src2dst = nullptr, *dst2src = nullptr, *tgt_d = nullptr;
  int32_t* eid2pos = nullptr;
  int32_t *pat_pos_d = nullptr, *pat_node_d = nullptr, *pat_rowmap_d = nullptr;
  uint8_t* pat_tilemask_d = nullptr;
  int32_t* pat_node_s = nullptr;
  uint8_t* pat_tilemask_s = nullptr;
  unsigned parts = 0;
  int sec_bits = 0, total_bits = 0;
  std::vector<const int32_t*> h_adj;
  std::vector<int64_t> h_off;
  float *invdeg_d = nullptr, *invdeg_edge_s = nullptr, *invdeg_edge_d = nullptr;
  tfgnn::GraphView views[4];
  tfgnn::CompactBuckets compact[2];
  size_t slab_bytes = 0;
  void* scratch = nullptr;
  size_t scratch_bytes = 0;
  void* pinned = nullptr;
  size_t pinned_bytes = 0;
  void* event = nullptr;
  bool pending = false;
};

namespace tfgnn {
int graph_require_parts(const tfgnn_graph* g, unsigned need, const char* who);
}
```

tf2_gnn_amd/csrc/mp_layer.hip:

```cpp
#include <cstring>

#include "common.hpp"
#include "tfgnn.h"

using namespace tfgnn;

extern "C" int tfgnn_mp_forward(const tfgnn_mp_forward_args* a, void* stream) {
  TFGNN_REQUIRE(a != nullptr && a->struct_size == sizeof(tfgnn_mp_forward_args),
                "tfgnn_mp_forward: args is NULL or was built against another header (struct_size)");
  TFGNN_REQUIRE(a->kind == TFGNN_MP_AGGREGATE_FIRST, "tfgnn_mp_forward: unknown layer kind %d", a->kind);
  TFGNN_REQUIRE(a->graph && a->x && a->wt_sp && a->wt_inv_scale && a->agg_sp && a->agg_inv_scale && (a->out || a->out_sp),
                "tfgnn_mp_forward: NULL pointer");
  TFGNN_REQUIRE(a->view == TFGNN_VIEW_BY_DST_TYPED || a->view == TFGNN_VIEW_BY_DST_TYPED_PATTERN,
                "tfgnn_mp_forward: the forward pass gathers over the by-target typed buckets (view %d)", a->view);
  int64_t V = 0, E = 0;
  int L = 0;
  int rc = tfgnn_graph_dims(a->graph, &V, &L, &E);
  if (rc) return rc;
  const int64_t D = a->in_dim, H = a->hidden_dim, K = (int64_t)L * D;
  TFGNN_REQUIRE(V > 0 && L > 0 && D > 0 && H > 0, "tfgnn_mp_forward: empty layer");
  tfgnn_aux_job own[2];
  std::memset(own, 0, sizeof(own));
  rc = tfgnn_graph_gather_reduce_sp_deferred(a->graph, a->view, nullptr, nullptr, a->row_scale, a->x, a->ldx, (int)D, a->agg_sp,
                                             D * 4, a->agg_inv_scale, nullptr, a->workspace, a->workspace_bytes, &own[0], stream);
  if (rc) return rc;
  if (a->w) {
    rc = tfgnn_sp_split_cols_job(a->w, H, K, H, a->wt_sp, a->ld_wt_sp_bytes, a->wt_inv_scale, &own[1]);
    if (rc) return rc;
  }
  rc = tfgnn_aux_launch(own, 2, stream);
  if (rc) return rc;
  return tfgnn_sp_gemm_nt_rows(V, H, K, a->agg_sp, K * 4, a->agg_inv_scale, (int)D, nullptr, a->wt_sp, a->ld_wt_sp_bytes, a->wt_inv_scale,
                               a->out, a->ld_out, a->bias, a->act, 0, nullptr, 0, TFGNN_ACT_NONE, nullptr, 0, 1.f, a->out_sp,
                               a->ld_out_sp_bytes, a->out_inv_scale, a->dropout_rate, a->dropout_seed, a->tile_kmask, a->row_map, stream);
}

extern "C" int tfgnn_mp_backward(const tfgnn_mp_backward_args* a, void* stream) {
  TFGNN_REQUIRE(a != nullptr && a->struct_size == sizeof(tfgnn_mp_backward_args),
                "tfgnn_mp_backward: args is NULL or was built against another header (struct_size)");
  TFGNN_REQUIRE(a->kind == TFGNN_MP_AGGREGATE_FIRST, "tfgnn_mp_backward: unknown layer kind %d", a->kind);
  TFGNN_REQUIRE(a->graph && a->d_pre && a->wh_sp && a->wh_inv_scale && a->g_sp && a->g_inv_scale && (a->dx || a->dx_sp),
                "tfgnn_mp_backward: NULL pointer");
  TFGNN_REQUIRE(!a->dw || (a->x_sp && a->x_inv_scale), "tfgnn_mp_backward: the kernel gradients need the layer input as a split operand");
  int64_t V = 0, E = 0;
  int L = 0;
  int rc = tfgnn_graph_dims(a->graph, &V, &L, &E);
  if (rc) return rc;
  const int64_t D = a->in_dim, H = a->hidden_dim, K = (int64_t)L * H;
  TFGNN_REQUIRE(V > 0 && L > 0 && D > 0 && H > 0, "tfgnn_mp_backward: empty layer");
  tfgnn_aux_job own[2];
  std::memset(own, 0, sizeof(own));
  rc = tfgnn_graph_gather_reduce_sp_deferred(a->graph, TFGNN_VIEW_BY_SRC_TYPED, nullptr, a->edge_weight, nullptr, a->d_pre, a->ld_d_pre,
                                                 (int)H, a->g_sp, H * 4, a->g_inv_scale, nullptr, a->workspace, a->workspace_bytes, &own[0],
                                                 stream);
  if (rc) return rc;
  if (a->w) {
    rc = tfgnn_sp_split_rows_job(a->w, H, H, D * H, D, K, (int)K, a->wh_sp, a->ld_wh_sp_bytes, a->wh_inv_scale, nullptr, &own[1]);
    if (rc) return rc;
  }
  rc = tfgnn_aux_launch(own, 2, stream);
  if (rc) return rc;
  rc = tfgnn_sp_gemm_nt_rows(V, D, K, a->g_sp, K * 4, a->g_inv_scale, (int)H, a->a_rows, a->wh_sp, a->ld_wh_sp_bytes, a->wh_inv_scale, a->dx,
                             a->ld_dx, nullptr, TFGNN_ACT_NONE, a->accumulate, a->mul, a->ld_mul, a->act_of_saved, a->saved, a->ld_saved,
                             a->saved_scale, a->dx_sp, a->ld_dx_sp_bytes, a->dx_inv_scale, a->dropout_rate, a->dropout_seed, a->tile_kmask,
                             a->row_map, stream);
  if (rc) return rc;
  if (a->dw)
    rc = tfgnn_sp_gemm_tn(K, D, V, a->g_sp, K * 4, 0, a->g_inv_scale, K, (int)H, a->x_sp, a->ld_x_sp_bytes, 0, a->x_inv_scale, a->dw, H, D * H, 1,
                          H, 0, a->tn_workspace, a->tn_workspace_bytes, stream);
  return rc;
}
```

tf2_gnn_amd/csrc/spmm.hip:

```cpp
#include <algorithm>
#include <cstdlib>

#include "aux_jobs.hpp"
#include "common.hpp"
#include "graph.hpp"
#include "sp16.hpp"

namespace tfgnn {

template <int VEC>
struct VecT;
template <>
struct VecT<4> {
  using type = float4;
};
template <>
struct VecT<1> {
  using type = float;
};

template <int VEC>
__device__ __forceinline__ typename VecT<VEC>::type vload(const float* p);
template <>
__device__ __forceinline__ float4 vload<4>(const float* p) {
  return *reinterpret_cast<const float4*>(p);
}
template <>
__device__ __forceinline__ float vload<1>(const float* p) {
  return *p;
}

template <int VEC>
__device__ __forceinline__ void vstore(float* p, const float* v);
template <>
__device__ __forceinline__ void vstore<4>(float* p, const float* v) {
  *reinterpret_cast<float4*>(p) = make_float4(v[0], v[1], v[2], v[3]);
}
template <>
__device__ __forceinline__ void vstore<1>(float* p, const float* v) {
  *p = v[0];
}

template <int VEC>
__device__ __forceinline__ void vunpack(const typename VecT<VEC>::type& v, float* o);
template <>
__device__ __forceinline__ void vunpack<4>(const float4& v, float* o) {
  o[0] = v.x;
  o[1] = v.y;
  o[2] = v.z;
  o[3] = v.w;
}
template <>
__device__ __forceinline__ void vunpack<1>(const float& v, float* o) {
  o[0] = v;
}

enum { MODE_SUM = 0, MODE_HEADS = 1, MODE_GENERAL = 2, MODE_HEADS_DOT = 3 };
__host__ __device__ constexpr bool mode_heads(int mode) { return mode == MODE_HEADS || mode == MODE_HEADS_DOT; }

template <int S>
__device__ __forceinline__ float dpp_partner(float v) {
  constexpr int ctrl = S == 0 ? 0xB1 : S == 1 ? 0x4E : S == 2 ? 0x141 : 0x140;
  return __int_as_float(__builtin_amdgcn_update_dpp(0, __float_as_int(v), ctrl, 0xF, 0xF, false));
}
template <int N, int L2>
__device__ __forceinline__ float dpp_split_sum(const float (&p)[N], int lane, int& which) {
  static_assert(N == 1 || N == 2 || N == 4, "values per lane");
  static_assert((1 << L2) >= N && L2 <= 4, "group");
  if constexpr (N == 4) {
    const bool hi = (lane >> (L2 - 1)) & 1;
    float q[2];
    q[0] = (hi ? p[2] : p[0]) + dpp_partner<L2 - 1>(hi ? p[0] : p[2]);
    q[1] = (hi ? p[3] : p[1]) + dpp_partner<L2 - 1>(hi ? p[1] : p[3]);
    int w;
    const float r = dpp_split_sum<2, L2 - 1>(q, lane, w);
    which = (hi ? 2 : 0) + w;
    return r;
  } else if constexpr (N == 2) {
    const bool hi = (lane >> (L2 - 1)) & 1;
    float q[1];
    q[0] = (hi ? p[1] : p[0]) + dpp_partner<L2 - 1>(hi ? p[0] : p[1]);
    int w;
    const float r = dpp_split_sum<1, L2 - 1>(q, lane, w);
    which = hi ? 1 : 0;
    return r;
  } else {
    float v = p[0];
    if constexpr (L2 >= 4) v += dpp_partner<3>(v);
    if constexpr (L2 >= 3) v += dpp_partner<2>(v);
    if constexpr (L2 >= 2) v += dpp_partner<1>(v);
    if constexpr (L2 >= 1) v += dpp_partner<0>(v);
    which = 0;
    return v;
  }
}

__device__ __forceinline__ float dpp_group_sum(float v, int log2n) {
  int x;
  if (log2n >= 1) { x = __builtin_amdgcn_update_dpp(0, __float_as_int(v), 0xB1, 0xF, 0xF, false); v += __int_as_float(x); }
  if (log2n >= 2) { x = __builtin_amdgcn_update_dpp(0, __float_as_int(v), 0x4E, 0xF, 0xF, false); v += __int_as_float(x); }
  if (log2n >= 3) { x = __builtin_amdgcn_update_dpp(0, __float_as_int(v), 0x141, 0xF, 0xF, false); v += __int_as_float(x); }
  if (log2n >= 4) { x = __builtin_amdgcn_update_dpp(0, __float_as_int(v), 0x140, 0xF, 0xF, false); v += __int_as_float(x); }
  return v;
}

struct GatherArgs {
  const int32_t* rowptr;
  const int32_t* col;
  const int32_t* short_rows;
  int64_t num_short;
  const float* ew;
  const float* row_scale;
  int64_t num_rows;
  const float* in;
  int64_t ld_in;
  int width;
  float* out;
  int64_t ld_out;
  int pre_act;
  int post_act;
  int is_max;
  int ew_heads;
  int head_width;
  const float* dot_rows;
  int64_t ld_dot;
  float* dot_out;
  const int32_t* dot_pos;
  int dot_lph_log2;
  int long_threshold;
  const int32_t* out_row_map;
  const int32_t* item_row;
  const int32_t* item_chunk;
  const int32_t* item_slot;
  float* partial;
  int item_chunk_edges;
  const int32_t* multi_row;
  const int32_t* multi_base;
  const int32_t* multi_n;
  int num_multi;
  uint8_t* out_sp;
  int64_t ld_out_sp;
  float* inv_out;
  const float* fixed_inv;
  tfgnn_aux_job* combine_job;
  bool multi_pairs;
};

template <int LANES>
__device__ __forceinline__ float sp_row_scale(const GatherArgs& a, float mx, int64_t orow, bool writer) {
  float iv, sc;
  if (a.fixed_inv) {
    iv = a.fixed_inv[0];
    sc = 1.f / iv;
  } else {
#pragma unroll
    for (int o = LANES / 2; o; o >>= 1) mx = fmaxf(mx, __shfl_xor(mx, o, LANES));
    sc = sp_scale_for_max(mx, &iv);
    if (writer) a.inv_out[orow] = iv;
  }
  return sc;
}

template <int LPR, int VPL, int VEC, int UNROLL, int MODE>
__device__ __forceinline__ void accumulate_edges(const GatherArgs& a, int32_t beg, int32_t end, int f0,
                                                 const bool (&live)[VPL], float (&acc)[VPL][VEC], int64_t row) {
  using V = typename VecT<VEC>::type;
  const bool is_max = MODE == MODE_GENERAL && a.is_max;
  int hidx[VPL];
  if (mode_heads(MODE)) {
#pragma unroll
    for (int i = 0; i < VPL; ++i) hidx[i] = live[i] ? (f0 + i * LPR * VEC) / a.head_width : 0;
  }
  float yv[VPL][VEC];
  bool dot_writer = false;
  if constexpr (MODE == MODE_HEADS_DOT) {
    const float* yrow = a.dot_rows + row * a.ld_dot + f0;
#pragma unroll
    for (int i = 0; i < VPL; ++i) {
#pragma unroll
      for (int c = 0; c < VEC; ++c) yv[i][c] = 0.f;
      if (live[i]) vunpack<VEC>(vload<VEC>(yrow + i * LPR * VEC), yv[i]);
    }
    dot_writer = ((threadIdx.x % LPR) & ((1 << a.dot_lph_log2) - 1)) == 0;
  }
  constexpr bool CAN_SPLIT = MODE == MODE_HEADS_DOT && (VPL == 2 || VPL == 4);
  const bool split = CAN_SPLIT && (1 << a.dot_lph_log2) >= VPL;
  bool split_writer = false;
  int split_head = 0;
  if (split) {
    constexpr int SPLIT_BITS = VPL == 4 ? 2 : 1;
    const int lane = threadIdx.x % LPR;
    const int which = (lane >> (a.dot_lph_log2 - SPLIT_BITS)) & (VPL - 1);
    const int f = f0 + which * LPR * VEC;
    split_writer = (lane & ((1 << (a.dot_lph_log2 - SPLIT_BITS)) - 1)) == 0 && f < a.width;
    split_head = f / a.head_width;
  }
  for (int32_t e = beg; e < end; e += UNROLL) {
    int32_t idx[UNROLL];
    int32_t eid[UNROLL];
    int32_t dpos[UNROLL];
    float w[UNROLL];
    bool ok[UNROLL];
#pragma unroll
    for (int u = 0; u < UNROLL; ++u) {
      int32_t ee = e + u;
      ok[u] = ee < end;
      ee = ok[u] ? ee : end - 1;
      eid[u] = ee;
      idx[u] = a.col[ee];
      if constexpr (MODE == MODE_HEADS_DOT) dpos[u] = a.dot_pos ? a.dot_pos[ee] : ee;
      w[u] = (!mode_heads(MODE) && a.ew) ? a.ew[ee] : 1.f;
    }
    V v[UNROLL][VPL];
    float wh[UNROLL][VPL];
#pragma unroll
    for (int u = 0; u < UNROLL; ++u) {
      const float* src = a.in + (int64_t)idx[u] * a.ld_in + f0;
#pragma unroll
      for (int i = 0; i < VPL; ++i) {
        if (live[i]) {
          v[u][i] = vload<VEC>(src + i * LPR * VEC);
          if (mode_heads(MODE)) wh[u][i] = a.ew[(int64_t)eid[u] * a.ew_heads + hidx[i]];
        }
      }
    }
#pragma unroll
    for (int u = 0; u < UNROLL; ++u) {
// ... 162 lines not shown
  for (int r = 0; r < R; ++r)
#pragma unroll
    for (int i = 0; i < VPL; ++i)
#pragma unroll
      for (int c = 0; c < VEC; ++c) acc[r][i][c] = 0.f;

  for (int32_t j = 0; j < maxlen; j += U) {
    int32_t idx[R][U];
    float w[R][U];
    bool ok[R][U];
#pragma unroll
    for (int r = 0; r < R; ++r)
#pragma unroll
      for (int u = 0; u < U; ++u) {
        ok[r][u] = j + u < len[r];
        idx[r][u] = 0;
        w[r][u] = 1.f;
        if (ok[r][u]) {
          const int32_t e = beg[r] + j + u;
          idx[r][u] = a.col[e];
          if (a.ew) w[r][u] = a.ew[e];
        }
      }
    V v[R][U][VPL];
#pragma unroll
    for (int r = 0; r < R; ++r)
#pragma unroll
      for (int u = 0; u < U; ++u)
        if (ok[r][u]) {
          const float* src = a.in + (int64_t)idx[r][u] * a.ld_in + f0;
#pragma unroll
          for (int i = 0; i < VPL; ++i)
            if (live[i]) v[r][u][i] = vload<VEC>(src + i * LPR * VEC);
        }
#pragma unroll
    for (int r = 0; r < R; ++r)
#pragma unroll
      for (int u = 0; u < U; ++u)
        if (ok[r][u]) {
#pragma unroll
          for (int i = 0; i < VPL; ++i)
            if (live[i]) {
              float x[VEC];
              vunpack<VEC>(v[r][u][i], x);
#pragma unroll
              for (int c = 0; c < VEC; ++c) {
                float m = w[r][u] * x[c];
                acc[r][i][c] += m;
              }
            }
        }
  }

#pragma unroll
  for (int r = 0; r < R; ++r) {
    if (!on[r]) continue;
    if constexpr (SP) {
      float mx = 0.f;
#pragma unroll
      for (int i = 0; i < VPL; ++i)
#pragma unroll
        for (int c = 0; c < VEC; ++c) {
          acc[r][i][c] *= rs[r];
          if (live[i]) mx = fmaxf(mx, fabsf(acc[r][i][c]));
        }
      const float sc = sp_row_scale<LPR>(a, mx, orow[r], gl == 0);
      uint8_t* drow = a.out_sp + orow[r] * a.ld_out_sp;
#pragma unroll
      for (int i = 0; i < VPL; ++i)
        if (live[i])
          sp_store4(drow, f0 + i * LPR * VEC,
                    make_float4(acc[r][i][0], acc[r][i][VEC > 1 ? 1 : 0], acc[r][i][VEC > 2 ? 2 : 0], acc[r][i][VEC > 3 ? 3 : 0]), sc);
    } else {
      float* dst = a.out + orow[r] * a.ld_out + f0;
#pragma unroll
      for (int i = 0; i < VPL; ++i)
        if (live[i]) {
          float o[VEC];
#pragma unroll
          for (int c = 0; c < VEC; ++c) o[c] = act_apply(a.post_act, acc[r][i][c] * rs[r]);
          vstore<VEC>(dst + i * LPR * VEC, o);
        }
    }
  }
}

template <int LPR, int VPL, int VEC, int UNROLL, int MODE, bool SP = false>
__device__ __forceinline__ void gather_item_block(const GatherArgs& a, int item, unsigned window,
                                                  float (&red)[256 / LPR][LPR * VPL * VEC]) {
  constexpr int GROUPS = 256 / LPR;
  constexpr int WINDOW = LPR * VPL * VEC;
  const int tid = threadIdx.x;
  const int group = tid / LPR;
  const int gl = tid % LPR;
  const int64_t row = a.item_row[item];
  const int32_t rbeg = a.rowptr[row], rend = a.rowptr[row + 1];
  const int32_t ibeg = rbeg + a.item_chunk[item] * a.item_chunk_edges;
  const int32_t iend = min(rend, ibeg + a.item_chunk_edges);
  int per = (iend - ibeg + GROUPS - 1) / GROUPS;
  per = (per + UNROLL - 1) / UNROLL * UNROLL;
  const int32_t beg = min(iend, ibeg + group * per);
  const int32_t end = min(iend, beg + per);
  const int w0 = window * WINDOW;
  const int f0 = w0 + gl * VEC;
  const bool is_max = MODE == MODE_GENERAL && a.is_max;

  float acc[VPL][VEC];
  bool live[VPL];
#pragma unroll
  for (int i = 0; i < VPL; ++i) {
    live[i] = (f0 + i * LPR * VEC) < a.width;
#pragma unroll
    for (int c = 0; c < VEC; ++c) acc[i][c] = is_max ? kFloatLowest : 0.f;
  }
  accumulate_edges<LPR, VPL, VEC, UNROLL, MODE>(a, beg, end, f0, live, acc, row);
#pragma unroll
  for (int i = 0; i < VPL; ++i)
#pragma unroll
    for (int c = 0; c < VEC; ++c) red[group][(gl + i * LPR) * VEC + c] = acc[i][c];
  __syncthreads();
  const int32_t slot = a.item_slot[item];
  const float rs = a.row_scale ? a.row_scale[row] : 1.f;
  if constexpr (SP) {
    if (slot < 0) {
      float mx = 0.f;
      for (int f = tid; f < WINDOW; f += 256) {
        if (w0 + f >= a.width) break;
        float v = red[0][f];
#pragma unroll
        for (int g = 1; g < GROUPS; ++g) v += red[g][f];
        v *= rs;
        red[0][f] = v;
        mx = fmaxf(mx, fabsf(v));
      }
#pragma unroll
      for (int o = 32; o; o >>= 1) mx = fmaxf(mx, __shfl_xor(mx, o, 64));
      __syncthreads();
      if ((tid & 63) == 0) red[1][tid >> 6] = mx;
      __syncthreads();
      mx = fmaxf(fmaxf(red[1][0], red[1][1]), fmaxf(red[1][2], red[1][3]));
      const int64_t orow = a.out_row_map ? a.out_row_map[row] : row;
      float iv, sc;
      if (a.fixed_inv) {
        iv = a.fixed_inv[0];
        sc = 1.f / iv;
      } else {
        sc = sp_scale_for_max(mx, &iv);
        if (tid == 0) a.inv_out[orow] = iv;
      }
      uint8_t* drow = a.out_sp + orow * a.ld_out_sp;
      for (int c4 = tid; c4 * 4 < WINDOW; c4 += 256)
        if (w0 + c4 * 4 < a.width)
          sp_store4(drow, w0 + c4 * 4, make_float4(red[0][c4 * 4], red[0][c4 * 4 + 1], red[0][c4 * 4 + 2], red[0][c4 * 4 + 3]), sc);
      return;
    }
  }
  for (int f = tid; f < WINDOW; f += 256) {
    if (w0 + f >= a.width) break;
    float s = red[0][f];
#pragma unroll
    for (int g = 1; g < GROUPS; ++g) s = is_max ? fmaxf(s, red[g][f]) : s + red[g][f];
    if (slot < 0) {
      const int64_t orow = a.out_row_map ? a.out_row_map[row] : row;
      a.out[orow * a.ld_out + w0 + f] = act_apply(a.post_act, s * rs);
    } else {
      a.partial[(int64_t)slot * a.width + w0 + f] = s;
    }
  }
}

__global__ void __launch_bounds__(256) csr_gather_combine_kernel(GatherArgs a) {
  const int64_t total = (int64_t)a.num_multi * a.width;
  for (int64_t i = (int64_t)blockIdx.x * blockDim.x + threadIdx.x; i < total; i += (int64_t)gridDim.x * blockDim.x) {
    const int m = (int)(i / a.width);
    const int f = (int)(i - (int64_t)m * a.width);
    const int64_t row = a.multi_row[m];
    const int32_t base = a.multi_base[m], n = a.multi_n[m];
    float s = a.partial[(int64_t)base * a.width + f];
    for (int k = 1; k < n; ++k) {
      const float p = a.partial[(int64_t)(base + k) * a.width + f];
      s = a.is_max ? fmaxf(s, p) : s + p;
    }
    const float rs = a.row_scale ? a.row_scale[row] : 1.f;
    const int64_t orow = a.out_row_map ? a.out_row_map[row] : row;
    a.out[orow * a.ld_out + f] = act_apply(a.post_act, s * rs);
  }
}

static AuxCombineSp combine_sp_args(const GatherArgs& a) {
  AuxCombineSp c{};
  c.multi_row = a.multi_row; c.multi_base = a.multi_base; c.multi_n = a.multi_n; c.num_multi = a.num_multi;
  c.row_scale = a.row_scale; c.partial = a.partial; c.width = a.width; c.out_row_map = a.out_row_map;
  c.out_sp = a.out_sp; c.ld_out_sp = a.ld_out_sp; c.inv_out = a.inv_out; c.fixed_inv = a.fixed_inv;
  return c;
}
__global__ void __launch_bounds__(256) csr_gather_combine_sp_kernel(AuxCombineSp a) { combine_sp_body(a, blockIdx.x); }

template <int LPR, int VPL, int VEC, int UNROLL, int MODE, bool SP = false>
__global__ void __launch_bounds__(256) csr_gather_reduce_kernel(GatherArgs a, int num_items) {
  __shared__ float red[256 / LPR][LPR * VPL * VEC];
  const unsigned unit = blockIdx.x, window = blockIdx.y;
  if ((int)unit < num_items)
    gather_item_block<LPR, VPL, VEC, UNROLL, MODE, SP>(a, (int)unit, window, red);
  else
    gather_rows_block<LPR, VPL, VEC, UNROLL, MODE, SP>(a, unit - (unsigned)num_items, window);
}

template <int LPR, int VPL, int VEC, int UNROLL, bool SP, int R, int U>
__global__ void __launch_bounds__(256) csr_gather_reduce_multi_kernel(GatherArgs a, int num_items) {
  __shared__ float red[256 / LPR][LPR * VPL * VEC];
  const unsigned unit = blockIdx.x;
  if ((int)unit < num_items)
    gather_item_block<LPR, VPL, VEC, UNROLL, MODE_SUM, SP>(a, (int)unit, 0, red);
  else
    gather_rows_block_multi<LPR, VPL, VEC, SP, R, U>(a, unit - (unsigned)num_items);
}

template <int LPR, int VPL, int VEC, int UNROLL, bool SP, int R, int U>
static void launch_multi(GatherArgs a, int num_items, hipStream_t s) {
  const unsigned units = (unsigned)(num_items + ceil_div(a.short_rows ? a.num_short : a.num_rows, (256 / LPR) * R));
  hipLaunchKernelGGL((csr_gather_reduce_multi_kernel<LPR, VPL, VEC, UNROLL, SP, R, U>), dim3(units, 1), dim3(256), 0, s, a, num_items);
}

template <int LPR, int VPL, int VEC, int UNROLL, int MODE, bool SP = false>
static int launch_mode(GatherArgs a, int num_items, hipStream_t s) {
  constexpr int GROUPS_PER_BLOCK = 256 / LPR;
  constexpr int WINDOW = LPR * VPL * VEC;
  const unsigned windows = (unsigned)ceil_div(a.width, WINDOW);
  const unsigned units = (unsigned)(num_items + ceil_div(a.short_rows ? a.num_short : a.num_rows, GROUPS_PER_BLOCK));
  dim3 block(256);
  bool multi_done = false;
  if constexpr (MODE == MODE_SUM && VEC == 4 && LPR * VPL <= 128) {
    if (a.multi_pairs && windows == 1 && (!SP || a.width <= 2048)) {
      launch_multi<LPR, VPL, VEC, UNROLL, SP, 2, 1>(a, num_items, s);
      multi_done = true;
    }
  }
  if constexpr (SP) {
    if (windows != 1 || a.width > 2048) {
      set_error("SP16 gather output needs the whole row in one feature window (width %d)", a.width);
      return TFGNN_ERR_UNSUPPORTED;
    }
    if (!multi_done)
      hipLaunchKernelGGL((csr_gather_reduce_kernel<LPR, VPL, VEC, UNROLL, MODE, true>), dim3(units, 1), block, 0, s, a, num_items);
    TFGNN_LAUNCH_CHECK();
    if (a.num_multi > 0) {
      if (a.combine_job) {
        aux_job_set(a.combine_job, AUX_COMBINE_SP, (unsigned)ceil_div(a.num_multi, 4), combine_sp_args(a));
      } else {
        hipLaunchKernelGGL(csr_gather_combine_sp_kernel, dim3((unsigned)ceil_div(a.num_multi, 4)), block, 0, s, combine_sp_args(a));
        TFGNN_LAUNCH_CHECK();
      }
    }
    return TFGNN_OK;
  }
  if (!multi_done)
    hipLaunchKernelGGL((csr_gather_reduce_kernel<LPR, VPL, VEC, UNROLL, MODE>), dim3(units, windows), block, 0, s, a,
                       num_items);
  TFGNN_LAUNCH_CHECK();
  if (a.num_multi > 0) {
    const int64_t total = (int64_t)a.num_multi * a.width;
    hipLaunchKernelGGL(csr_gather_combine_kernel, dim3((unsigned)std::min<int64_t>(ceil_div(total, 256), 4096)), block, 0, s, a);
    TFGNN_LAUNCH_CHECK();
  }
  return TFGNN_OK;
}

template <int LPR, int VPL, int VEC, int UNROLL>
static int launch_variant(const GatherArgs& a, int mode, int num_items, hipStream_t s) {
  if (mode == MODE_SUM) return launch_mode<LPR, VPL, VEC, UNROLL, MODE_SUM>(a, num_items, s);
  if (mode == MODE_HEADS) return launch_mode<LPR, VPL, VEC, UNROLL, MODE_HEADS>(a, num_items, s);
  if (mode == MODE_HEADS_DOT) {
    if constexpr (VEC == 4) {
      TFGNN_REQUIRE((1 << a.dot_lph_log2) <= LPR, "fused edge products: a head is wider than a lane group (width %d)", a.width);
      return launch_mode<LPR, VPL, VEC, UNROLL, MODE_HEADS_DOT>(a, num_items, s);
    } else {
      set_error("fused edge products need 16-byte aligned rows");
      return TFGNN_ERR_UNSUPPORTED;
    }
  }
  return launch_mode<LPR, VPL, VEC, UNROLL, MODE_GENERAL>(a, num_items, s);
}

constexpr double kMultiAvgLen = 1.5;

static int gather_dispatch(GatherArgs a, int num_items, hipStream_t s) {
  int mode = MODE_SUM;
  if (a.is_max || a.pre_act != TFGNN_ACT_NONE) mode = MODE_GENERAL;
  if (a.ew && a.ew_heads > 1) {
    TFGNN_REQUIRE(mode == MODE_SUM, "per-head edge weights only support plain sums");
    TFGNN_REQUIRE(a.head_width > 0 && a.width % a.head_width == 0 && a.width / a.head_width == a.ew_heads,
                  "width %d is not ew_heads %d x head_width %d", a.width, a.ew_heads, a.head_width);
    mode = MODE_HEADS;
    if (a.dot_out) {
      TFGNN_REQUIRE(a.dot_rows && a.ld_dot >= a.width && a.ld_dot % 4 == 0 && (uintptr_t)a.dot_rows % 16 == 0,
                    "fused edge products: bad row operand");
      mode = MODE_HEADS_DOT;
    }
  }
  TFGNN_REQUIRE(!a.dot_out || mode == MODE_HEADS_DOT, "fused edge products ride on the per-head weighted sums only");
  const bool vec4 = (a.width % 4 == 0) && (a.ld_in % 4 == 0) && (a.ld_out % 4 == 0) &&
                    (((uintptr_t)a.in | (uintptr_t)a.out) % 16 == 0) && (!a.out_sp || a.ld_out_sp % 64 == 0) &&
                    (!mode_heads(mode) || a.head_width % 4 == 0);
  TFGNN_REQUIRE(vec4 || !a.out_sp, "SP16 gather output needs 16-byte aligned rows");
  if (!vec4) {
    return launch_variant<16, 4, 1, 2>(a, mode, num_items, s);
  }
  const int chunks = a.width / 4;
  if (a.out_sp) {
    TFGNN_REQUIRE(mode == MODE_SUM && a.width % 16 == 0, "SP16 gather output: plain sums of rows with width %% 16 == 0 only");
    if (chunks <= 8) return launch_mode<8, 1, 4, 8, MODE_SUM, true>(a, num_items, s);
    if (chunks <= 16) return launch_mode<16, 1, 4, 8, MODE_SUM, true>(a, num_items, s);
    if (chunks <= 32) return launch_mode<16, 2, 4, 4, MODE_SUM, true>(a, num_items, s);
    if (chunks <= 64) return launch_mode<16, 4, 4, 2, MODE_SUM, true>(a, num_items, s);
    if (chunks <= 80) return launch_mode<16, 5, 4, 2, MODE_SUM, true>(a, num_items, s);
    return launch_mode<32, 4, 4, 2, MODE_SUM, true>(a, num_items, s);
  }
  if (chunks <= 8) return launch_variant<8, 1, 4, 8>(a, mode, num_items, s);
  if (chunks <= 16) return launch_variant<16, 1, 4, 8>(a, mode, num_items, s);
  if (chunks <= 32) return launch_variant<16, 2, 4, 4>(a, mode, num_items, s);
  if (chunks <= 64) return launch_variant<16, 4, 4, 2>(a, mode, num_items, s);
  if (chunks % 80 == 0 || chunks <= 80) return launch_variant<16, 5, 4, 2>(a, mode, num_items, s);
  return launch_variant<32, 4, 4, 2>(a, mode, num_items, s);
}

static int check_common(int64_t num_rows, const void* rowptr, const void* in, const void* out, int64_t ld_in,
                        int64_t ld_out, int width, int reduce_op) {
  TFGNN_REQUIRE(rowptr && in && out, "NULL pointer");
  TFGNN_REQUIRE(ld_in >= width && ld_out >= width, "leading dimension smaller than width");
  TFGNN_REQUIRE(reduce_op == TFGNN_REDUCE_SUM || reduce_op == TFGNN_REDUCE_MAX, "unknown reduce op %d", reduce_op);
  TFGNN_REQUIRE(num_rows < ((int64_t)1 << 31), "too many rows");
  return TFGNN_OK;
}

}

extern "C" int tfgnn_csr_gather_reduce(const int32_t* d_rowptr, const int32_t* d_col,
                                       const float* d_edge_weight, const float* d_row_scale,
                                       int64_t num_rows, const float* d_in, int64_t ld_in, int width,
                                       float* d_out, int64_t ld_out, int reduce_op, int pre_act,
                                       int post_act, void* stream) {
  using namespace tfgnn;
  TFGNN_REQUIRE(num_rows >= 0 && width >= 0, "negative size");
  if (num_rows == 0 || width == 0) return TFGNN_OK;
  int rc = check_common(num_rows, d_rowptr, d_in, d_out, ld_in, ld_out, width, reduce_op);
  if (rc) return rc;
  GatherArgs a{};
  a.rowptr = d_rowptr; a.col = d_col; a.ew = d_edge_weight; a.row_scale = d_row_scale;
  a.num_rows = num_rows; a.in = d_in; a.ld_in = ld_in; a.width = width; a.out = d_out; a.ld_out = ld_out;
  a.pre_act = pre_act; a.post_act = post_act; a.is_max = reduce_op == TFGNN_REDUCE_MAX;
  a.ew_heads = 1; a.head_width = width;
  return gather_dispatch(a, 0, (hipStream_t)stream);
}

extern "C" size_t tfgnn_graph_gather_workspace_bytes(const tfgnn_graph* g, int view, int width) {
  if (!g || view < 0 || view > 7 || width <= 0) return 0;
  if (view >= 4) view = (view == 4 || view == 6) ? 0 : 2;
  return (size_t)g->views[view].plan.num_partials * (size_t)width * 4;
}

extern "C" int tfgnn_graph_gather_dot_supported(int width, int ew_heads);
static int graph_gather_impl(const tfgnn_graph* g, int view, const int32_t* d_col_override,
                             const float* d_edge_weight, int ew_heads, const float* d_row_scale,
                             const float* d_in, int64_t ld_in, int width, float* d_out,
                             int64_t ld_out, int reduce_op, int pre_act, int post_act,
                             void* d_workspace, size_t workspace_bytes, void* stream, void* d_out_sp, int64_t ld_out_sp,
                             float* d_inv_scale, const float* d_fixed_inv, tfgnn_aux_job* combine_job = nullptr,
                             const float* d_dot_rows = nullptr, int64_t ld_dot = 0, const int32_t* d_dot_pos = nullptr,
                             float* d_dot_out = nullptr) {
  using namespace tfgnn;
  TFGNN_REQUIRE(g != nullptr, "graph is NULL");
  TFGNN_REQUIRE(view >= 0 && view <= 6, "unknown graph view %d", view);
  TFGNN_REQUIRE(width >= 0 && ew_heads >= 1, "bad sizes");
  {
    unsigned need = (view == 1 || view == 3) ? TFGNN_GRAPH_PART_PLAN_NODE : TFGNN_GRAPH_PART_PLAN_TYPED;
    if (view == 4 || view == 5) need |= TFGNN_GRAPH_PART_COMPACT;
    if (view == 6) need |= TFGNN_GRAPH_PART_DST_PATTERN;
    const int prc = graph_require_parts(g, need, "tfgnn_graph_gather_reduce");
    if (prc) return prc;
  }
  const int32_t* out_map = nullptr;
  int64_t compact_nz = -1;
  if (view == 6) {
    TFGNN_REQUIRE(g->L <= 8, "TFGNN_VIEW_BY_DST_TYPED_PATTERN: at most 8 edge types");
    out_map = g->pat_rowmap_d;
    view = 0;
  } else if (view >= 4) {
    out_map = g->compact[view - 4].cpos;
    compact_nz = g->compact[view - 4].num_nz;
    view = view == 4 ? 0 : 2;
  }
  const GraphView& gv = g->views[view];
  if (gv.num_rows == 0 || width == 0) return TFGNN_OK;
  int rc = check_common(gv.num_rows, gv.rowptr, d_in, d_out_sp ? (const void*)d_out_sp : (const void*)d_out, ld_in,
                        d_out_sp ? (int64_t)width : ld_out, width, reduce_op);
  if (rc) return rc;
  const CsrPlan& p = gv.plan;
  TFGNN_REQUIRE(p.num_partials == 0 || (d_workspace && workspace_bytes >= (size_t)p.num_partials * width * 4),
                "workspace too small: need %zu bytes", (size_t)p.num_partials * width * 4);
  GatherArgs a{};
  a.rowptr = gv.rowptr; a.col = d_col_override ? d_col_override : gv.col; a.ew = d_edge_weight;
  a.row_scale = d_row_scale; a.num_rows = gv.num_rows; a.in = d_in; a.ld_in = ld_in; a.width = width;
  a.out = d_out; a.ld_out = d_out_sp ? (int64_t)width : ld_out; a.pre_act = pre_act; a.post_act = post_act;
  a.out_sp = (uint8_t*)d_out_sp; a.ld_out_sp = ld_out_sp; a.inv_out = d_inv_scale; a.fixed_inv = d_fixed_inv;
  a.combine_job = combine_job;
  if (combine_job) combine_job->kind = 0, combine_job->num_blocks = 0;
  a.is_max = reduce_op == TFGNN_REDUCE_MAX; a.ew_heads = ew_heads; a.head_width = width / ew_heads;
  a.long_threshold = p.long_threshold;
  a.out_row_map = out_map;
  if (d_dot_out) {
    TFGNN_REQUIRE(ew_heads > 1 && d_edge_weight && width % ew_heads == 0, "tfgnn_graph_gather_reduce_dot: per-head edge weights only");
    const int lph = width / ew_heads / 4;
    TFGNN_REQUIRE(tfgnn_graph_gather_dot_supported(width, ew_heads), "tfgnn_graph_gather_reduce_dot: unsupported head width %d",
                  width / ew_heads);
    a.dot_rows = d_dot_rows; a.ld_dot = ld_dot; a.dot_out = d_dot_out; a.dot_pos = d_dot_pos;
    a.dot_lph_log2 = 31 - __builtin_clz((unsigned)lph);
  }
  a.item_row = p.item_row; a.item_chunk = p.item_chunk; a.item_slot = p.item_slot;
  a.partial = (float*)d_workspace; a.item_chunk_edges = p.item_chunk_edges;
  a.multi_row = p.multi_row; a.multi_base = p.multi_base; a.multi_n = p.multi_n; a.num_multi = p.num_multi;
  a.short_rows = p.short_rows;
  a.num_short = p.num_short;
  if (compact_nz >= 0) a.num_short = std::max<int64_t>(0, (int64_t)p.num_short - (gv.num_rows - compact_nz));
  {
    const char* multi_env = getenv("TFGNN_GATHER_MULTI");
    const int multi_knob = multi_env ? atoi(multi_env) : 0;
    const int64_t nslots = a.short_rows ? a.num_short : a.num_rows;
    if (multi_knob == 21) a.multi_pairs = true;
    else if (multi_knob == 0) a.multi_pairs = nslots > 0 && !a.is_max && ew_heads == 1 && (double)g->E <= kMultiAvgLen * (double)nslots;
  }
  count_launch(d_out_sp ? TFGNN_KFAM_GATHER_SP : TFGNN_KFAM_GATHER);
  return gather_dispatch(a, p.num_items, (hipStream_t)stream);
}

extern "C" int tfgnn_graph_gather_reduce(const tfgnn_graph* g, int view, const int32_t* d_col_override,
                                         const float* d_edge_weight, int ew_heads, const float* d_row_scale,
                                         const float* d_in, int64_t ld_in, int width, float* d_out,
                                         int64_t ld_out, int reduce_op, int pre_act, int post_act,
                                         void* d_workspace, size_t workspace_bytes, void* stream) {
  return graph_gather_impl(g, view, d_col_override, d_edge_weight, ew_heads, d_row_scale, d_in, ld_in, width, d_out, ld_out,
                           reduce_op, pre_act, post_act, d_workspace, workspace_bytes, stream, nullptr, 0, nullptr, nullptr);
}

extern "C" int tfgnn_graph_gather_dot_supported(int width, int ew_heads) {
  if (width <= 0 || ew_heads <= 1 || width % ew_heads) return 0;
  const int hw = width / ew_heads;
  if (hw % 4 || width % 4) return 0;
  const int lph = hw / 4, chunks = width / 4;
  if (lph & (lph - 1)) return 0;
  const int lanes_per_row = chunks <= 8 ? 8 : (chunks <= 80 ? 16 : 32);
  return lph <= 16 && lph <= lanes_per_row;
}

extern "C" int tfgnn_graph_gather_reduce_dot(const tfgnn_graph* g, int view, const float* d_edge_weight, int ew_heads,
                                             const float* d_in, int64_t ld_in, int width, float* d_out, int64_t ld_out,
                                             const float* d_dot_rows, int64_t ld_dot, const int32_t* d_dot_pos, float* d_dot_out,
                                             void* d_workspace, size_t workspace_bytes, void* stream) {
  using namespace tfgnn;
  TFGNN_REQUIRE(d_dot_rows && d_dot_out, "tfgnn_graph_gather_reduce_dot: NULL pointer");
  return graph_gather_impl(g, view, nullptr, d_edge_weight, ew_heads, nullptr, d_in, ld_in, width, d_out, ld_out, TFGNN_REDUCE_SUM,
                           TFGNN_ACT_NONE, TFGNN_ACT_NONE, d_workspace, workspace_bytes, stream, nullptr, 0, nullptr, nullptr, nullptr,
                           d_dot_rows, ld_dot, d_dot_pos, d_dot_out);
}

extern "C" int tfgnn_graph_gather_reduce_sp(const tfgnn_graph* g, int view, const int32_t* d_col_override,
                                            const float* d_edge_weight, const float* d_row_scale, const float* d_in,
                                            int64_t ld_in, int width, void* d_out_sp, int64_t ld_out_sp_bytes,
                                            float* d_inv_scale, const float* d_fixed_inv_scale, void* d_workspace,
                                            size_t workspace_bytes, void* stream) {
  using namespace tfgnn;
  TFGNN_REQUIRE(d_out_sp && (d_inv_scale || d_fixed_inv_scale), "tfgnn_graph_gather_reduce_sp: NULL output");
  TFGNN_REQUIRE(ld_out_sp_bytes >= (int64_t)width * 4 && ld_out_sp_bytes % 64 == 0 && (uintptr_t)d_out_sp % 64 == 0,
                "tfgnn_graph_gather_reduce_sp: bad SP16 leading dimension / alignment");
  return graph_gather_impl(g, view, d_col_override, d_edge_weight, 1, d_row_scale, d_in, ld_in, width, nullptr, 0,
                           TFGNN_REDUCE_SUM, TFGNN_ACT_NONE, TFGNN_ACT_NONE, d_workspace, workspace_bytes, stream, d_out_sp,
                           ld_out_sp_bytes, d_inv_scale, d_fixed_inv_scale);
}

extern "C" int tfgnn_graph_gather_reduce_sp_deferred(const tfgnn_graph* g, int view, const int32_t* d_col_override,
                                                     const float* d_edge_weight, const float* d_row_scale, const float* d_in,
                                                     int64_t ld_in, int width, void* d_out_sp, int64_t ld_out_sp_bytes,
                                                     float* d_inv_scale, const float* d_fixed_inv_scale, void* d_workspace,
                                                     size_t workspace_bytes, tfgnn_aux_job* combine_job, void* stream) {
  using namespace tfgnn;
  TFGNN_REQUIRE(d_out_sp && (d_inv_scale || d_fixed_inv_scale) && combine_job, "tfgnn_graph_gather_reduce_sp_deferred: NULL output");
  TFGNN_REQUIRE(ld_out_sp_bytes >= (int64_t)width * 4 && ld_out_sp_bytes % 64 == 0 && (uintptr_t)d_out_sp % 64 == 0,
                "tfgnn_graph_gather_reduce_sp_deferred: bad SP16 leading dimension / alignment");
  return graph_gather_impl(g, view, d_col_override, d_edge_weight, 1, d_row_scale, d_in, ld_in, width, nullptr, 0,
                           TFGNN_REDUCE_SUM, TFGNN_ACT_NONE, TFGNN_ACT_NONE, d_workspace, workspace_bytes, stream, d_out_sp,
                           ld_out_sp_bytes, d_inv_scale, d_fixed_inv_scale, combine_job);
}
```

tf2_gnn_amd/layers/gnn.py:

```python
from __future__ import annotations

from typing import Any, Dict, List, NamedTuple, Optional, Sequence, Tuple

import torch

from .. import ops
from ..utils.param_helpers import get_activation_function
from .graph_global_exchange import (
    GraphGlobalExchange,
    GraphGlobalExchangeInput,
    GraphGlobalGRUExchange,
    GraphGlobalMeanExchange,
    GraphGlobalMLPExchange,
)
from .message_passing import MessagePassing, MessagePassingInput, get_message_passing_class
from .message_passing.message_passing import Variable, _num_edge_types, default_device, get_graph, glorot_uniform


class GNNInput(NamedTuple):

    node_features: torch.Tensor
    adjacency_lists: Tuple[torch.Tensor, ...]
    node_to_graph_map: torch.Tensor
    num_graphs: Any
# ... 88 lines not shown
    variables = trainable_variables

    def zero_grad(self):
        for v in self.trainable_variables:
            v.grad = None

    def build(self, tensor_shapes: GNNInput):
        dev = default_device()
        D_in = int(tensor_shapes.node_features[-1])
        adjacency_list_shapes = tuple(tensor_shapes.adjacency_lists)
        H = self._hidden_dim
        embedded_shape = (None, H)
        name = f"{self._message_passing_class.__name__}_GNN"
        self._initial_projection_layer = Variable(
            f"{name}/gnn_initial_node_projection/kernel", glorot_uniform((D_in, H), device=dev)
        )
        for layer_idx in range(self._num_layers):
            mp = self._message_passing_class(self._params)
            mp.build(MessagePassingInput(embedded_shape, adjacency_list_shapes))
            for v in mp.variables:
                v.name = f"{name}/Layer_{layer_idx}/MessagePassing/{v.name}"
            self._mp_layers.append(mp)
            if self._use_inter_layer_layernorm:
                self._inter_layer_layernorms.append(
                    (
                        Variable(f"{name}/Layer_{layer_idx}/LayerNorm/gamma", torch.ones(H, dtype=torch.float32, device=dev)),
                        Variable(f"{name}/Layer_{layer_idx}/LayerNorm/beta", torch.zeros(H, dtype=torch.float32, device=dev)),
                    )
                )
            if layer_idx % self._dense_every_num_layers == 0:
                self._dense_layers[str(layer_idx)] = Variable(
                    f"{name}/Layer_{layer_idx}/Dense/kernel", glorot_uniform((H, H), device=dev)
                )
            if layer_idx and layer_idx % self._global_exchange_every_num_layers == 0:
                mode = self._params["global_exchange_mode"].lower()
                cls = {"mean": GraphGlobalMeanExchange, "gru": GraphGlobalGRUExchange, "mlp": GraphGlobalMLPExchange}[mode]
                ex = cls(
                    hidden_dim=H,
                    weighting_fun=self._params["global_exchange_weighting_fun"],
                    num_heads=self._params["global_exchange_num_heads"],
                    dropout_rate=self._params["global_exchange_dropout_rate"],
                )
                ex.build(GraphGlobalExchangeInput(embedded_shape, (None,), ()))
                for v in ex.trainable_variables:
                    v.name = f"{name}/Layer_{layer_idx}/Global_Exchange/{v.name}"
                self._global_exchange_layers[str(layer_idx)] = ex
        self.built = True

    def __call__(self, inputs: GNNInput, training: bool = False, return_all_representations: bool = False):
        if not self.built:
            self.build(
                GNNInput(
                    tuple(inputs.node_features.shape),
                    tuple((None, 2) for _ in range(_num_edge_types(inputs.adjacency_lists))),
                    (None,),
                    (),
                )
            )
        return self.call(inputs, training, return_all_representations)

    def call(self, inputs: GNNInput, training: bool = False, return_all_representations: bool = False):
        cur, all_reprs = self._internal_call(inputs, training, need_all_representations=return_all_representations)
        if return_all_representations:
            return cur, all_reprs
        return cur

    def graph_parts(self, num_nodes: int, edges_per_type) -> int:
        if not self._mp_layers:
            return ops.G_PARTS_DEFAULT
        parts = 0
        for mp in self._mp_layers:
            parts |= mp.graph_parts(num_nodes, edges_per_type, self._hidden_dim)
        return parts

    def _dense_f16x2(self, in_dim: int, out_dim: int) -> bool:
        if (not self._dense_split_ok or self._dense_tn_wide) and ops.REARM_EPOCH[0] != self._dense_demoted_epoch:
            self._dense_split_ok = True
            self._dense_tn_wide = False
            self._guard_sync_passes = max(self._guard_sync_passes, self._guard_sync_passes_init)
        if ops.env("TFGNN_DENSE_F16X2", "1") == "0" or not self._dense_split_ok:
            return False
        return ops.get_gemm_mode() == ops.GEMM_F16X2 and in_dim % 16 == 0 and in_dim >= 32 and ops.sp_tiles(out_dim)

    def _dense(self, x, w: Variable, act_name, drop=None):
        if x.shape[0] > 0 and self._dense_f16x2(w.value.shape[0], w.value.shape[1]):
            wt = ops.sp_weight_operand(w.value, "cols", lambda: ops.sp_split_cols(w.value, defer=True))
            if act_name == "gelu":
                pre = ops.sp_gemm_nt(ops.sp_rows_of(x), wt)
                return ops.activation_forward("gelu", pre), pre, False
            if drop is not None and ops.sp_one_tile(w.value.shape[1]):
                out, _ = ops.sp_gemm_nt_split(ops.sp_rows_of(x), wt, act=act_name, dropout=drop)
                return out, None, True
            return ops.sp_gemm_nt(ops.sp_rows_of(x), wt, act=act_name), None, False
        if act_name == "gelu":
            pre = ops.gemm(x, w.value)
            return ops.activation_forward("gelu", pre), pre, False
        return ops.gemm(x, w.value, act=act_name), None, False

    def _dense_backward(self, x, w: Variable, gpre, act_grad=None, need_input_grad=True):
        d_in, d_out = w.value.shape
        if x.shape[0] > 0 and self._dense_f16x2(d_in, d_out):
            g_sp = ops.sp_rows_of(gpre)
            if self._dense_tn_wide:
                w.grad = ops.sp_gemm_tn(ops.sp_rows_of(x), g_sp, out=torch.empty_like(w.value), wide=True)
            else:
                w.grad = ops.sp_gemm_tn(ops.sp_rows_of(x), g_sp)
            if not need_input_grad:
                return None
            if ops.sp_tiles(d_in):
                wr = ops.sp_weight_operand(w.value, "rows", lambda: ops.sp_split_rows(w.value, defer=True))
                return ops.sp_gemm_nt(g_sp, wr, act_grad=act_grad)
            return ops.gemm_grad(gpre, w.value, trans_b=True, act_grad=act_grad)
        w.grad = ops.gemm(x, gpre, trans_a=True)
        return ops.gemm_grad(gpre, w.value, trans_b=True, act_grad=act_grad) if need_input_grad else None

    def _fuse_dropout_statically(self, layer_idx: int) -> bool:
        if ops.get_gemm_mode() != ops.GEMM_F16X2:
            return False
        if layer_idx % self._residual_every_num_layers == 0 and not (layer_idx == 0 and self._residual_every_num_layers >= self._num_layers):
            return False
        if layer_idx == 0:
            return True
        prev = layer_idx - 1
        return not self._use_inter_layer_layernorm and str(prev) not in self._global_exchange_layers

    def _recompute_dropout(self, layer_idx: int, mp_layer, V: int, D: int, L: int) -> bool:
        if ops.env("TFGNN_RECOMPUTE_DROPOUT", "1") == "0" or ops.get_gemm_mode() != ops.GEMM_F16X2:
            return False
        if layer_idx % self._residual_every_num_layers == 0 and not (layer_idx == 0 and self._residual_every_num_layers >= self._num_layers):
            return False
        return bool(getattr(mp_layer, "built", False) and mp_layer.recomputes_input_dropout(V, D, L))

    def _internal_call(self, inputs: GNNInput, training: bool = False, need_all_representations: bool = True):
        X = inputs.node_features
        V = X.shape[0]
        adj = inputs.adjacency_lists
        if self._tn_demoted_epoch is not None and ops.REARM_EPOCH[0] != self._tn_demoted_epoch:
            for mp in self._mp_layers:
                if mp._grouped_tn_split_ok is False:
                    mp._grouped_tn_split_ok = True
            self._tn_demoted_epoch = None
            self._guard_sync_passes = max(self._guard_sync_passes, self._guard_sync_passes_init)
        graph = adj if isinstance(adj, ops.Graph) else get_graph(
            adj, V, parts=self.graph_parts(V, [int(a.shape[0]) if a.numel() else 0 for a in adj]))
        graph = get_graph(graph, V)
        rate = float(self._params["layer_input_dropout_rate"])
        steps = []
        NL = self._num_layers

        drop_seed, ex_seed = [None] * NL, {}
        for i in range(NL):
            if training and rate > 0.0:
                self._dropout_calls += 1
                drop_seed[i] = self.dropout_seed * 1000003 + self._dropout_calls
            if str(i) in self._global_exchange_layers:
                self._dropout_calls += 1
                ex_seed[i] = self.dropout_seed * 1000003 + self._dropout_calls

        def drop_for(i, producer_output_is_read):
            if i >= NL or drop_seed[i] is None or producer_output_is_read or not self._fuse_dropout_statically(i):
                return None
            return (rate, drop_seed[i])

        cur, pre0, dropped = self._dense(X, self._initial_projection_layer, self._init_act,
                                         drop=drop_for(0, need_all_representations))
        ctx = {"X": X, "h0": cur, "pre0": pre0, "steps": steps, "h0_scale": (1.0 - rate) if dropped else 1.0,
               "all_representations": need_all_representations}
        last = cur
        all_reprs = [cur]
        for layer_idx, mp_layer in enumerate(self._mp_layers):
            st = {}
            if drop_seed[layer_idx] is not None:
                if dropped:
                    st["drop"] = ops.DropoutSpec(rate, drop_seed[layer_idx], tuple(cur.shape), cur.device)
                    st["drop_by_producer"] = True
                elif self._recompute_dropout(layer_idx, mp_layer, V, int(cur.shape[1]), graph.num_edge_types):
                    st["drop"] = ops.DropoutSpec(rate, drop_seed[layer_idx], tuple(cur.shape), cur.device)
                    cur, _ = ops.dropout_forward(cur, rate, drop_seed[layer_idx], want_mask=False)
                else:
                    cur, st["mask"] = ops.dropout_forward(cur, rate, drop_seed[layer_idx])
            dropped = False
            if layer_idx % self._residual_every_num_layers == 0:
                tmp = cur
                if layer_idx > 0:
                    cur = ops.add_scale(cur, last, 0.5)
                last = tmp
            dense_here = layer_idx % self._dense_every_num_layers == 0
            has_ex = str(layer_idx) in self._global_exchange_layers
            want_split = (dense_here and not has_ex
                          and not self._use_inter_layer_layernorm and self._dense_f16x2(self._hidden_dim, self._hidden_dim))
            direct = not (dense_here or has_ex or self._use_inter_layer_layernorm)
            cur, dropped = mp_layer.call_with_epilogue(
                MessagePassingInput(node_embeddings=cur, adjacency_lists=graph), training=training, want_split_output=want_split,
                output_dropout=drop_for(layer_idx + 1, need_all_representations) if direct else None)
            all_reprs.append(cur)
            if has_ex:
                ex = self._global_exchange_layers[str(layer_idx)]
                ex.dropout_seed = ex_seed[layer_idx]
                cur = ex(GraphGlobalExchangeInput(cur, inputs.node_to_graph_map, inputs.num_graphs), training=training)
            if self._use_inter_layer_layernorm:
                g_, b_ = self._inter_layer_layernorms[layer_idx]
                st["ln_in"] = cur
                cur, st["ln_mean"], st["ln_rstd"] = ops.layernorm_forward(cur, g_.value, b_.value, 1e-3)
            if dense_here:
                st["dense_in"] = cur
                cur, st["dense_pre"], dropped = self._dense(cur, self._dense_layers[str(layer_idx)], self._dense_act,
                                                            drop=drop_for(layer_idx + 1, False))
                st["dense_out"] = cur
                st["dense_out_scale"] = (1.0 - rate) if dropped else 1.0
            steps.append(st)
        self._ctx = ctx
        return cur, (tuple(all_reprs) if need_all_representations else None)

    def dropout_masks(self):
        if self._ctx is None:
            raise RuntimeError("no forward pass recorded")
        out = []
        for st in self._ctx["steps"]:
            out.append(st["mask"] if "mask" in st else (st["drop"].mask() if "drop" in st else None))
        return out

    def _tail_first_backward_op(self, layer_idx: int, ctx):
        if layer_idx == 0:
            if self._init_act is None:
                return None
            return self._init_act, (ctx["pre0"] if self._init_act == "gelu" else ctx["h0"]), ctx.get("h0_scale", 1.0)
        prev = layer_idx - 1
        st = ctx["steps"][prev]
        if prev % self._dense_every_num_layers == 0:
            if self._dense_act is None:
                return None
            return (self._dense_act, (st["dense_pre"] if self._dense_act == "gelu" else st["dense_out"]),
                    st.get("dense_out_scale", 1.0))
        if self._use_inter_layer_layernorm or str(prev) in self._global_exchange_layers:
            return None
        return self._mp_layers[prev].activation_backward_spec()

    def backward(self, grad_output: Optional[torch.Tensor], need_input_grad: bool = False,
                 grad_all_representations: Optional[Sequence[Optional[torch.Tensor]]] = None):
        ctx = self._ctx
        if ctx is None:
            raise RuntimeError("backward called before a forward pass")
        extras = list(grad_all_representations) if grad_all_representations is not None else [None] * (self._num_layers + 1)
        if len(extras) != self._num_layers + 1:
            raise ValueError(f"grad_all_representations needs {self._num_layers + 1} entries, got {len(extras)}")
        if grad_all_representations is not None and not ctx.get("all_representations", True) and any(e is not None for e in extras):
            raise ValueError("grad_all_representations given, but the forward pass ran without return_all_representations=True "
                             "(the intermediate results were not materialised)")
        g = grad_output
# ... 10 lines not shown
                    raise RuntimeError("tf2_gnn_amd: this GNN's first backward passes are checked synchronously "
                                       f"(TFGNN_GUARD_SYNC_PASSES, {self._guard_sync_passes} left); run them eagerly before "
                                       "capturing the step (capture.CapturedStep warmup)")
                periodic = False
            if not (was_f16x2 and (self._guard_sync_passes > 0 or periodic)):
                self.guard_tripped_last_backward = bool(was_f16x2 and ops.f16x2_guard_flag_async())
                if was_f16x2:
                    self._unchecked_split_passes += 1
                    self._unchecked_epoch = ops.REARM_EPOCH[0]
                return self._backward_walk(ctx, g, g_is_pre, g_last, extras, need_input_grad)
            if self._guard_sync_passes > 0:
                self._guard_sync_passes -= 1
            self.guard_tripped_last_backward = False
            self._unchecked_split_passes = 0
            with ops.hold_spread_guard():
                result = self._backward_walk(ctx, g, g_is_pre, g_last, extras, need_input_grad)
                for attempt in range(4):
                    if not ops.f16x2_guard_tripped_sync():
                        break
                    self.guard_tripped_last_backward = True
                    what = self._demote_fragile_weight_gradients() if attempt < 3 else None
                    if what:
                        ops.rearm_spread_guard()
                        import warnings

                        warnings.warn(f"tf2_gnn_amd: operand rows of a weight-gradient product of this GNN are spread beyond the range "
                                      f"of the split-operand product that ran: {what}; the pass was recomputed")
                    else:
                        ops.demote_gemm_mode()
                    for v in self.trainable_variables:
                        v.grad = None
                    result = self._backward_walk(ctx, g, False, None, extras, need_input_grad)
            return result
        finally:
            ops.aux_flush()

    def guard_state(self) -> Dict[str, Any]:
        stage = "none"
        if self._dense_tn_wide:
            stage = "1a"
        if not self._dense_split_ok:
            stage = "1b"
        if self._tn_demoted_epoch is not None:
            stage = "2"
        if self._backward_passes and ops.get_gemm_mode() != ops.GEMM_F16X2:
            stage = "3" if stage != "none" or ops.f16x2_guard_flag_async() else stage
        return {"tripped": self.guard_tripped_last_backward, "stage": stage, "checked_passes_left": self._guard_sync_passes}

    def _on_late_guard_trip(self) -> Optional[str]:
        if self._unchecked_split_passes == 0 or self._unchecked_epoch != ops.REARM_EPOCH[0]:
            return None
        if self._late_trip_pass == self._backward_passes:
            return "(this stack's policy has moved a step for that pass already)"
        what = self._demote_fragile_weight_gradients()
        if what:
            self._late_trip_pass = self._backward_passes
            self._guard_sync_passes = max(self._guard_sync_passes, self._guard_sync_passes_init)
            self.guard_tripped_last_backward = True
        return what

    def _demote_fragile_weight_gradients(self) -> Optional[str]:
        if self._dense_split_ok and self._dense_f16x2(self._hidden_dim, self._hidden_dim):
            self._dense_demoted_epoch = ops.REARM_EPOCH[0]
            if not self._dense_tn_wide:
                self._dense_tn_wide = True
                return "the Dense / projection weight gradients (now on the two-factor split-operand product)"
            self._dense_split_ok = False
            return "the Dense / projection products (now on the exact bf16x3 kernels)"
        did = False
        for mp in self._mp_layers:
            if mp._grouped_tn_used and mp._grouped_tn_split_ok:
                mp._grouped_tn_split_ok = False
                did = True
        if did:
            self._tn_demoted_epoch = ops.REARM_EPOCH[0]
        return "the per-relation MLP weight gradients (now on the exact bf16x3 kernels)" if did else None

    @staticmethod
    def _activation_backward_scaled(act, g, saved, saved_scale):
        _, spec = ops.plain_epilogue(None, (act, saved, saved_scale))
        return ops.activation_backward(act, g, spec[1])

    def _backward_walk(self, ctx, g, g_is_pre, g_last, extras, need_input_grad):
        for layer_idx in range(self._num_layers - 1, -1, -1):
            st = ctx["steps"][layer_idx]
            mp = self._mp_layers[layer_idx]
            has_ln = self._use_inter_layer_layernorm
            has_ex = str(layer_idx) in self._global_exchange_layers
            if layer_idx % self._dense_every_num_layers == 0:
                w = self._dense_layers[str(layer_idx)]
                gpre = g
                if self._dense_act is not None and not g_is_pre:
                    gpre = self._activation_backward_scaled(
                        self._dense_act, g, st["dense_pre"] if self._dense_act == "gelu" else st["dense_out"],
                        st.get("dense_out_scale", 1.0))
                nxt = None if (has_ln or has_ex or extras[layer_idx + 1] is not None) else mp.activation_backward_spec()
                g = self._dense_backward(st["dense_in"], w, gpre, act_grad=nxt)
                g_is_pre = nxt is not None
            if has_ln:
                gam, bet = self._inter_layer_layernorms[layer_idx]
                g, gam.grad, bet.grad = ops.layernorm_backward(g, st["ln_in"], gam.value, st["ln_mean"], st["ln_rstd"])
            if has_ex:
                g = self._global_exchange_layers[str(layer_idx)].backward(g)
            if extras[layer_idx + 1] is not None:
                g = ops.add_scale(g, extras[layer_idx + 1], 1.0)
            residual_here = layer_idx % self._residual_every_num_layers == 0 and not (layer_idx == 0 and g_last is None)
            mask = st.get("mask", st.get("drop"))
            if not residual_here:
                nxt = None if extras[layer_idx] is not None else self._tail_first_backward_op(layer_idx, ctx)
                below_is_dense = layer_idx == 0 or (layer_idx - 1) % self._dense_every_num_layers == 0
                want_split = nxt is not None and below_is_dense and self._dense_f16x2(self._hidden_dim, self._hidden_dim)
                g = mp.backward_with_epilogue(g, grad_is_pre_activation=g_is_pre, out_mul=mask, out_act_grad=nxt,
                                              want_split_input_grad=want_split)
                g_is_pre = nxt is not None
            else:
                g = mp.backward_with_epilogue(g, grad_is_pre_activation=g_is_pre)
                g_is_pre = False
                if layer_idx > 0:
                    half = ops.add_scale(g, g, 0.25)
                    g = half if g_last is None else ops.add_scale(half, g_last, 1.0)
                    g_last = half
                else:
                    g = ops.add_scale(g, g_last, 1.0)
                    g_last = None
                if mask is not None:
                    g = ops.mul(g, mask.mask() if isinstance(mask, ops.DropoutSpec) else mask)
        if extras[0] is not None:
            g = ops.add_scale(g, extras[0], 1.0)
        gpre = g
        if self._init_act is not None and not g_is_pre:
            gpre = self._activation_backward_scaled(self._init_act, g, ctx["pre0"] if self._init_act == "gelu" else ctx["h0"],
                                                    ctx.get("h0_scale", 1.0))
        return self._dense_backward(ctx["X"], self._initial_projection_layer, gpre, need_input_grad=need_input_grad)


def _act_name(fn):
    return None if fn is None else fn.tfgnn_name
```

tf2_gnn_amd/layers/message_passing/gnn_edge_mlp.py:

```python
from __future__ import annotations

from typing import Any, Dict, List, Optional

import torch

from ... import _lib, ops
from .message_passing import (
    apply_gradient_epilogue,
    MessagePassing,
    MessagePassingInput,
    Variable,
    _edge_identity,
    default_device,
    get_graph,
    glorot_uniform,
    register_message_passing_implementation,
)


def mlp_hidden_sizes(out_size: int, hidden_layers) -> List[int]:
    if isinstance(hidden_layers, int):
        return [out_size] * hidden_layers
    return list(hidden_layers)

# ... 233 lines not shown
        if is_max:
            ctx["agg_max"] = out
        if separate_post:
            return ops.activation_forward(fuse_act, out)
        return self._split_gelu(out, fuse_act, ctx)

    @staticmethod
    def _split_gelu(pre, fuse_act, ctx):
        if fuse_act != "gelu":
            return pre
        ctx["pre"] = pre
        return ops.activation_forward("gelu", pre)

    def _message_grads(self, g, d_agg, ctx, msgs, msg_row, target, ew, node_scale, sel_col):
        pre = self._activation_name if self._pre_activation() else None
        d_agg = d_agg.contiguous()
        if self._aggregation_name == "max":
            sel = ops.edge_aggregate_backward(msgs, target, None, msg_row=msg_row, edge_weight=ew, pre_act=pre,
                                              reduce=ops.REDUCE_MAX, agg_max=ctx["agg_max"], phase=0)
            nsel = ops.graph_gather(g, ops.VIEW_BY_DST_NODE, sel, col=sel_col)
            return ops.edge_aggregate_backward(msgs, target, d_agg, msg_row=msg_row, edge_weight=ew, pre_act=pre,
                                               reduce=ops.REDUCE_MAX, agg_max=ctx["agg_max"], num_selected=nsel)
        return ops.edge_aggregate_backward(msgs, target, d_agg, msg_row=msg_row, edge_weight=ew, node_scale=node_scale,
                                           pre_act=pre, reduce=ops.REDUCE_SUM)

    @staticmethod
    def _ident_nz(g, nz):
        ident = g._cache.get(("ident_nz", nz))
        if ident is None:
            ident = torch.arange(nz + 1, dtype=torch.int32, device=g.device)
            g._cache[("ident_nz", nz)] = ident
        return ident

    @staticmethod
    def _orig_src_node(g, src_l):
        src_node = g._cache.get("orig_src_node")
        if src_node is None:
            src_node = torch.div(src_l, g.num_edge_types, rounding_mode="floor").to(torch.int32)
            g._cache["orig_src_node"] = src_node
        return src_node

    SPARSE_BUCKET_THRESHOLD = 0.85

    def _use_compact_buckets(self, g) -> bool:
        if not self._compact_opt_in:
            return False
        if self._use_target_state_as_input or g.num_edge_types == 0 or g.num_edges == 0:
            return False
        nz = g.nonempty_offsets(False)[-1]
        return nz < self.SPARSE_BUCKET_THRESHOLD * g.num_nodes * g.num_edge_types

    def _forward_A_compact(self, X, g, fuse_act):
        row_scale, _, _, _ = self._scales(g)
        W = self._edge_type_mlps.kernels[0]
        off_h = g.nonempty_offsets(False)
        Ac = ops.graph_gather(g, ops.VIEW_BY_DST_TYPED_COMPACT, X, row_scale=row_scale)
        Yc = ops.gemm_grouped_rows(Ac, g.array(ops.G_NZ_OFF_BY_DST), off_h, W)
        gelu_split = fuse_act == "gelu"
        pre = ops.gather_reduce(
            g.array(ops.G_NZ_NODEPTR_BY_DST), g.array(ops.G_NZ_COL_BY_DST), Yc, post_act=None if gelu_split else fuse_act
        )
        ctx = {"path": "Ac", "fused_act": fuse_act}
        return self._split_gelu(pre, fuse_act, ctx), ctx, False

    def _backward_A_compact(self, d_agg, ctx):
        g, X = ctx["graph"], ctx["X"]
        mlps = self._edge_type_mlps
        W = mlps.kernels[0]
        L = g.num_edge_types
        _, _, ew_s, _ = self._scales(g)
        off_h = g.nonempty_offsets(True)
        nz = off_h[-1]
        off_d = g.array(ops.G_NZ_OFF_BY_SRC)
        Gc = ops.graph_gather(g, ops.VIEW_BY_SRC_TYPED_COMPACT, d_agg, edge_weight=ew_s)
        Zc = ops.gemm_grouped_rows(Gc, off_d, off_h, W, trans_b=True)
        dX = ops.gather_reduce(g.array(ops.G_NZ_NODEPTR_BY_SRC), g.array(ops.G_NZ_COL_BY_SRC), Zc)
        Xc = ops.gather_reduce(self._ident_nz(g, nz), g.array(ops.G_NZ_NODE_BY_SRC), X)
        mlps.set_grads([ops.gemm_grouped_k(Xc, Gc, off_d, off_h, L)])
        return dX

    def _f16x2_eligible(self, V, D, L, H) -> bool:
        return (ops.get_gemm_mode() == ops.GEMM_F16X2 and not self._use_target_state_as_input and L > 0 and V > 0
                and D % 16 == 0 and D <= 512 and 32 <= H <= 512 and ops.sp_tiles(H) and ops.sp_tiles(D))

    def _forward_A(self, X, g, fuse_act, want_split=False, drop=None):
        if self._use_compact_buckets(g):
            return self._forward_A_compact(X, g, fuse_act)
        V, D = X.shape
        L, H = g.num_edge_types, self._hidden_dim
        T = self._use_target_state_as_input
        row_scale, _, _, _ = self._scales(g)
        W = self._edge_type_mlps.kernels[0]
        Din = W.shape[1]
        if not T and messages_per_edge(self, g, D, H):
            _, ew_d, _, node_scale = self._scales(g)
            src_l, _, _, _, off, _ = self._original_order(g, ew_d)
            src_node = self._orig_src_node(g, src_l)
            msgs = torch.empty((g.num_edges, H), dtype=torch.float32, device=X.device)
            for l, sl in _type_slices(off):
                ops.gemm_gathered(X, src_node[sl], W[l], out=msgs[sl])
            ctx = {"path": "A", "A": None, "fused_act": fuse_act, "f16x2": self._f16x2_eligible(V, D, L, H)}
            return self._gather_messages(g, msgs, g.array(ops.G_EID_BY_DST), ew_d, node_scale, fuse_act, ctx), ctx, False
        if self._f16x2_eligible(V, D, L, H):
            skip = _skip_empty_blocks(L, Din)
            kmask = g.array(ops.G_PATTERN_TILEMASK_BY_DST) if skip else None
            rmap = g.array(ops.G_PATTERN_NODE_BY_DST) if skip else None
            view = ops.VIEW_BY_DST_TYPED_PATTERN if skip else ops.VIEW_BY_DST_TYPED
            gelu_split = fuse_act == "gelu"
            want_split = want_split or self._always_split_output
            out_scale = 1.0
            fuse_drop = drop is not None and not gelu_split and ops.sp_one_tile(H) and type(self)._finish is GNN_Edge_MLP._finish
            split_out = fuse_drop or (want_split and not gelu_split and ops.sp_one_tile(H))
            if ops.mp_entry_enabled() and Din == D:
                pre, _ = ops.mp_forward(g, view, X, W, row_scale=row_scale, act=None if gelu_split else fuse_act,
                                        dropout=drop if fuse_drop else None, tile_kmask=kmask, row_map=rmap, want_split=split_out)
            else:
                A_sp = ops.graph_gather_sp(g, view, X, row_scale=row_scale, rows_per_operand_row=L, defer_combine=True)
                Wt_sp = ops.sp_weight_operand(W, "cols", lambda: ops.sp_split_cols(W.view(L * Din, H), defer=True))
                if split_out:
                    pre, _ = ops.sp_gemm_nt_split(A_sp, Wt_sp, act=fuse_act, dropout=drop if fuse_drop else None, tile_kmask=kmask,
                                                  row_map=rmap)
                else:
                    pre = ops.sp_gemm_nt(A_sp, Wt_sp, act=None if gelu_split else fuse_act, tile_kmask=kmask, row_map=rmap)
            if fuse_drop:
                out_scale = 1.0 - float(drop[0])
            ctx = {"path": "A", "A": None, "fused_act": fuse_act, "f16x2": True, "out_scale": out_scale}
            return self._split_gelu(pre, fuse_act, ctx), ctx, fuse_drop
        A = torch.empty((V, L * Din), dtype=torch.float32, device=X.device)
        Arows = A.view(V * L, Din)
        ops.graph_gather(g, ops.VIEW_BY_DST_TYPED, X, row_scale=row_scale, out=Arows[:, :D])
        if T:
            from ..graph_scales import target_multiplier

            k, ident_ptr, node_of_row = target_multiplier(g, row_scale)
            ops.gather_reduce(ident_ptr, node_of_row, X, edge_weight=k, out=Arows[:, D:])
        act = None if fuse_act == "gelu" else fuse_act
        if ops.get_gemm_mode() != ops.GEMM_FP32:
            Wt = ops.sp_weight_operand(W, "transposed", lambda: ops.transpose_batched(W.view(L * Din, H)))
            pre = ops.gemm(A, Wt, trans_b=True, act=act)
        else:
            pre = ops.gemm(A, W.view(L * Din, H), act=act)
        ctx = {"path": "A", "A": A, "fused_act": fuse_act}
        return self._split_gelu(pre, fuse_act, ctx), ctx, False

    @staticmethod
    def _skip_args(g, L, width, by_src):
        if not _skip_empty_blocks(L, width):
            return {}
        node_at = g.array(ops.G_PATTERN_NODE_BY_SRC if by_src else ops.G_PATTERN_NODE_BY_DST)
        kmask = g.array(ops.G_PATTERN_TILEMASK_BY_SRC if by_src else ops.G_PATTERN_TILEMASK_BY_DST)
        return dict(tile_kmask=kmask, a_rows=node_at, row_map=node_at)

    def _backward_A_f16x2(self, d_agg, ctx, g, X, ew_s, epilogue=None, want_split=False, accumulate=None):
        V, D = X.shape
        L, H = g.num_edge_types, self._hidden_dim
        mlps = self._edge_type_mlps
        W = mlps.kernels[0]
        skip = self._skip_args(g, L, H, True) if V > 0 else {}
        applied = accumulate is not None or epilogue is not None
        split = False
        if accumulate is not None:
            kw = dict(out=accumulate[0], accumulate=True, out_mul=accumulate[1])
        elif epilogue is not None:
            kw = dict(out_mul=epilogue[0], act_grad=epilogue[1])
            split = bool(want_split) and ops.sp_one_tile(D)
        else:
# ... 482 lines not shown
```

tf2_gnn_amd/layers/message_passing/message_passing.py:

```python
from __future__ import annotations

from abc import abstractmethod
from collections import OrderedDict
from typing import Any, Dict, List, NamedTuple, Optional, Sequence, Tuple, Union

import torch

from ... import ops
from ...utils.param_helpers import get_activation_function, get_aggregation_function


class MessagePassingInput(NamedTuple):

    node_embeddings: torch.Tensor
    adjacency_lists: Union[Tuple[torch.Tensor, ...], "ops.Graph"]


class Variable:

    def __init__(self, name: str, value: torch.Tensor, trainable: bool = True):
        self.name = name
        self.value = value
        self.trainable = trainable
        self.grad: Optional[torch.Tensor] = None
# ... 252 lines not shown
        for v in getattr(self, "_variables", []):
            if v.trainable and v.value.requires_grad:
                v.value.grad = None
                v.value.requires_grad_(False)

    def backward(self, grad_output: torch.Tensor) -> torch.Tensor:
        ctx = self._ctx
        if ctx is None or "per_type" not in ctx:
            raise RuntimeError("backward called before a forward pass in training mode (the generic path records its "
                               "autograd tape only when training=True or layer.record_tape_in_eval is set)")
        try:
            return self._generic_backward(ctx, grad_output)
        finally:
            self._release_tape()

    def _generic_backward(self, ctx, grad_output: torch.Tensor) -> torch.Tensor:
        if type(self)._compute_new_node_embeddings is not MessagePassing._compute_new_node_embeddings:
            raise NotImplementedError(
                f"{type(self).__name__} overrides _compute_new_node_embeddings; the generic backward covers the base class "
                "aggregation (message_passing.py:135-179) - implement backward() next to the override"
            )
        X, adjacency_lists, messages_per_type = ctx["X"], ctx["adjacency_lists"], ctx["messages"]
        V, H = X.shape[0], self._hidden_dim
        g = get_graph(adjacency_lists, V)
        E = g.num_edges
        dX = torch.zeros_like(X)
        for v in self._variables:
            v.grad = None
        if E == 0:
            for v in self._variables:
                if v.trainable:
                    v.grad = torch.zeros_like(v.value)
            return dX
        from ..graph_scales import graph_scales

        act = self._activation_name
        pre = act if self._message_activation_before_aggregation else None
        is_max = self._aggregation_name == "max"
        node_scale = graph_scales(g, False, self._aggregation_name)[3]
        eid_d = g.array(ops.G_EID_BY_DST)
        messages = torch.cat([m.detach() for m in messages_per_type], dim=0).contiguous()
        target = torch.cat([a[:, 1] for a in adjacency_lists], dim=0).to(torch.int32).contiguous()
        agg_raw = None
        if is_max or (pre is None and act == "gelu"):
            agg_raw = ops.graph_gather(g, ops.VIEW_BY_DST_NODE, messages, col=eid_d, row_scale=node_scale,
                                       reduce=ops.REDUCE_MAX if is_max else ops.REDUCE_SUM, pre_act=pre)
        d_agg = grad_output.contiguous()
        if pre is None and act is not None:
            d_agg = ops.activation_backward(act, d_agg, agg_raw if act == "gelu" else ctx["out"])
        if is_max:
            sel = ops.edge_aggregate_backward(messages, target, None, pre_act=pre, reduce=ops.REDUCE_MAX, agg_max=agg_raw, phase=0)
            nsel = ops.graph_gather(g, ops.VIEW_BY_DST_NODE, sel, col=eid_d)
            dM = ops.edge_aggregate_backward(messages, target, d_agg, pre_act=pre, reduce=ops.REDUCE_MAX, agg_max=agg_raw,
                                             num_selected=nsel)
        else:
            dM = ops.edge_aggregate_backward(messages, target, d_agg, node_scale=node_scale, pre_act=pre, reduce=ops.REDUCE_SUM)
        d_src, d_tgt, off = [], [], 0
        leaves = [v.value for v in self._variables if v.trainable]
        for (xs, xt), m in zip(ctx["per_type"], messages_per_type):
            n = m.shape[0]
            if n and m.grad_fn is None:
                raise NotImplementedError(
                    f"{type(self).__name__}._message_function returned a tensor without an autograd history (built from "
                    "kernels outside torch autograd?): write it with torch operations, or override backward()"
                )
            if n:
                torch.autograd.backward([m], [dM[off : off + n]], inputs=[xs, xt] + leaves)
            d_src.append(xs.grad if xs.grad is not None else torch.zeros_like(xs))
            d_tgt.append(xt.grad if xt.grad is not None else torch.zeros_like(xt))
            off += n
        dX = ops.graph_gather(g, ops.VIEW_BY_SRC_NODE, torch.cat(d_src, dim=0).contiguous(), col=g.array(ops.G_EID_BY_SRC))
        dX = ops.add_scale(dX, ops.graph_gather(g, ops.VIEW_BY_DST_NODE, torch.cat(d_tgt, dim=0).contiguous(), col=eid_d), 1.0)
        for v in self._variables:
            if v.trainable:
                v.grad = v.value.grad if v.value.grad is not None else torch.zeros_like(v.value)
        return dX

    def activation_backward_spec(self):
        return None

    def recomputes_input_dropout(self, num_nodes: int, in_dim: int, num_edge_types: int) -> bool:
        return False

    def call_with_epilogue(self, inputs: MessagePassingInput, training: bool = False, *, want_split_output: bool = False,
                           output_dropout=None):
        return self(inputs, training=training), False

    def backward_with_epilogue(self, grad_output, grad_is_pre_activation=False, out_mul=None, out_act_grad=None,
                               want_split_input_grad=False):
        if grad_is_pre_activation:
            raise ValueError(f"{type(self).__name__} does not accept an already activation-multiplied gradient")
        return apply_gradient_epilogue(self.backward(grad_output), out_mul, out_act_grad)


def apply_gradient_epilogue(g, out_mul, out_act_grad):
    out_mul, out_act_grad = ops.plain_epilogue(out_mul, out_act_grad)
    if out_mul is not None and out_act_grad is not None:
        return ops.activation_backward(out_act_grad[0], g, out_act_grad[1], mul=out_mul)
    if out_mul is not None:
        g = ops.mul(g, out_mul)
    if out_act_grad is not None:
        g = ops.activation_backward(out_act_grad[0], g, out_act_grad[1])
    return g


def _num_edge_types(adjacency_lists) -> int:
    if isinstance(adjacency_lists, ops.Graph):
        return adjacency_lists.num_edge_types
    return len(adjacency_lists)


def gather_rows(params: torch.Tensor, ids: torch.Tensor) -> torch.Tensor:
    n = ids.shape[0]
    if params.shape[0] == 0 and n:
        raise ValueError("gather from an empty tensor")
    rowptr = torch.arange(n + 1, dtype=torch.int32, device=params.device)
    if n and (int(ids.min()) < 0 or int(ids.max()) >= params.shape[0]):
        raise ValueError("index out of range in gather")
    return ops.gather_reduce(rowptr, ids.to(torch.int32).contiguous(), params.reshape(params.shape[0], -1))


MESSAGE_PASSING_IMPLEMENTATIONS: Dict[str, type] = {}


def register_message_passing_implementation(cls):
    MESSAGE_PASSING_IMPLEMENTATIONS[cls.__name__.lower()] = cls
    return cls


def calculate_type_to_num_incoming_edges(node_embeddings, adjacency_lists):
    num_nodes = node_embeddings.shape[0]
    g = get_graph(adjacency_lists, num_nodes)
    L = g.num_edge_types
    rowptr = g.array(ops.G_ROWPTR_BY_DST)
    counts = (rowptr[1:] - rowptr[:-1]).reshape(num_nodes, L)
    return counts.t().to(torch.float32).contiguous()
```

tf2_gnn_amd/ops.py:

```python
from __future__ import annotations

import ctypes
import threading
import weakref
import os
from typing import Optional, Sequence

import torch

from . import _lib

ACT_NONE, ACT_RELU, ACT_TANH, ACT_LEAKY_RELU, ACT_ELU, ACT_SELU, ACT_GELU, ACT_SIGMOID = range(8)
REDUCE_SUM, REDUCE_MAX = 0, 1

_ACT_BY_NAME = {
    "none": ACT_NONE,
    "relu": ACT_RELU,
    "tanh": ACT_TANH,
    "leaky_relu": ACT_LEAKY_RELU,
    "elu": ACT_ELU,
    "selu": ACT_SELU,
    "gelu": ACT_GELU,
    "sigmoid": ACT_SIGMOID,
}
# ... 75 lines not shown
            aux_flush()
        _AUX_STREAM[0] = st
        _AUX_PENDING.append((stage, job, keep))


def aux_flush() -> None:
    with _AUX_LOCK:
        batch = list(_AUX_PENDING)
        del _AUX_PENDING[:]
        for stage in (0, 1):
            live = [j for s, j, _ in batch if s == stage]
            if live:
                jobs = (_lib.AuxJob * len(live))(*live)
                _lib.check(_lib.load().tfgnn_aux_launch(jobs, len(jobs), _AUX_STREAM[0]))


def _ptr(t: Optional[torch.Tensor]):
    return None if t is None else ctypes.c_void_p(t.data_ptr())


def _require_dev(t: torch.Tensor, dtype, what: str):
    if not t.is_cuda:
        raise RuntimeError(
            f"tf2_gnn_amd: {what} must live on a ROCm device (got {t.device}); there is no CPU fallback"
        )
    if t.dtype != dtype:
        raise TypeError(f"tf2_gnn_amd: {what} must be {dtype}, got {t.dtype}")


def _rowmajor(t: torch.Tensor, what: str):
    if t.dim() != 2:
        raise ValueError(f"{what} must be 2-D, got shape {tuple(t.shape)}")
    if t.shape[1] > 1 and t.stride(1) != 1:
        t = t.contiguous()
    ld = t.stride(0) if t.shape[0] > 1 else max(t.shape[1], 1)
    if ld < t.shape[1]:
        t = t.contiguous()
        ld = max(t.shape[1], 1)
    return t, ld


def _writes_out(fn):
    import functools

    import inspect

    try:
        out_pos = list(inspect.signature(fn).parameters).index("out")
    except ValueError:
        out_pos = None

    @functools.wraps(fn)
    def wrapper(*args, **kwargs):
        res = fn(*args, **kwargs)
        out = kwargs.get("out")
        if out is None and out_pos is not None and len(args) > out_pos:
            out = args[out_pos]
        if isinstance(out, torch.Tensor):
            torch.autograd.graph.increment_version(out)
        return res

    return wrapper


class _DevArray:

    def __init__(self, ptr: int, count: int, typestr: str, owner):
        self._owner = owner
        self.__cuda_array_interface__ = {
            "shape": (count,),
            "typestr": typestr,
            "data": (ptr, False),
            "version": 2,
            "strides": None,
        }


(G_ROWPTR_BY_DST, G_COL_BY_DST, G_EID_BY_DST, G_COLL_BY_DST, G_ROWPTR_BY_SRC, G_COL_BY_SRC, G_EID_BY_SRC,
 G_COLL_BY_SRC, G_INVDEG_BY_DST, G_INVDEG_EDGE_BY_SRC, G_NODEPTR_BY_DST, G_NODEPTR_BY_SRC,
 G_INVDEG_EDGE_BY_DST, G_SRC2DST_POS, G_TARGET_BY_DST, G_NZ_CPOS_BY_DST, G_NZ_ROW_BY_DST, G_NZ_NODE_BY_DST,
 G_NZ_OFF_BY_DST, G_NZ_NODEPTR_BY_DST, G_NZ_COL_BY_DST, G_NZ_CPOS_BY_SRC, G_NZ_ROW_BY_SRC, G_NZ_NODE_BY_SRC,
 G_NZ_OFF_BY_SRC, G_NZ_NODEPTR_BY_SRC, G_NZ_COL_BY_SRC, G_PATTERN_POS_BY_DST, G_PATTERN_NODE_BY_DST,
 G_PATTERN_TILEMASK_BY_DST, G_PATTERN_NODE_BY_SRC, G_PATTERN_TILEMASK_BY_SRC) = range(32)
_FLOAT_ARRAYS = {G_INVDEG_BY_DST, G_INVDEG_EDGE_BY_SRC, G_INVDEG_EDGE_BY_DST}
_BYTE_ARRAYS = {G_PATTERN_TILEMASK_BY_DST, G_PATTERN_TILEMASK_BY_SRC}
G_PART_PLAN_TYPED, G_PART_PLAN_NODE, G_PART_COMPACT, G_PART_EDGE_MAPS, G_PART_EDGE_IDS, G_PART_DST_PATTERN, G_PARTS_ALL = 1, 2, 4, 8, 16, 32, 63
G_PARTS_DEFAULT = G_PARTS_ALL & ~G_PART_DST_PATTERN
_VIEW_PARTS = {0: G_PART_PLAN_TYPED, 1: G_PART_PLAN_NODE, 2: G_PART_PLAN_TYPED, 3: G_PART_PLAN_NODE,
               4: G_PART_PLAN_TYPED | G_PART_COMPACT, 5: G_PART_PLAN_TYPED | G_PART_COMPACT,
               6: G_PART_PLAN_TYPED | G_PART_DST_PATTERN, 7: G_PART_PLAN_TYPED | G_PART_DST_PATTERN}


def _array_parts(array_id: int) -> int:
    if array_id == G_SRC2DST_POS:
        return G_PART_EDGE_MAPS | G_PART_EDGE_IDS
    if array_id in (G_EID_BY_DST, G_EID_BY_SRC):
        return G_PART_EDGE_IDS
    if G_PATTERN_POS_BY_DST <= array_id <= G_PATTERN_TILEMASK_BY_SRC:
        return G_PART_DST_PATTERN
    return G_PART_COMPACT if G_NZ_CPOS_BY_DST <= array_id <= G_NZ_COL_BY_SRC else 0


class Graph:

    def __init__(self, adjacency_lists: Sequence[torch.Tensor], num_nodes: int, wait: bool = True, parts: int = G_PARTS_DEFAULT):
        lib = _lib.load()
        adjs = []
        for i, a in enumerate(adjacency_lists):
            _require_dev(a, torch.int32, f"adjacency_lists[{i}]")
            if a.dim() != 2 or a.shape[1] != 2:
                if a.numel() == 0:
                    a = a.reshape(0, 2)
                else:
                    raise ValueError(f"adjacency_lists[{i}] must have shape [E, 2], got {tuple(a.shape)}")
            adjs.append(a.contiguous())
        self._keep = adjs
        L = len(adjs)
        ptrs = (ctypes.c_void_p * max(L, 1))(*[a.data_ptr() if a.numel() else None for a in adjs])
        counts = (ctypes.c_int64 * max(L, 1))(*[a.shape[0] for a in adjs])
        handle = ctypes.c_void_p()
        self._h = None
        _lib.check(
            lib.tfgnn_graph_create_parts_async(L, int(num_nodes), ptrs, counts, int(parts) & G_PARTS_ALL, _stream(),
                                               ctypes.byref(handle))
        )
        self._h = handle
        self.parts = int(parts) & G_PARTS_ALL
        if self.parts & G_PART_EDGE_MAPS:
            self.parts |= G_PART_EDGE_IDS
        self._lists = adjs
        self._pending = True
        self.num_nodes = int(num_nodes)
        self.num_edge_types = L
        self.num_edges = int(sum(a.shape[0] for a in adjs))
        self.edges_per_type = tuple(int(a.shape[0]) for a in adjs)
        self.device = adjs[0].device if adjs else torch.device("cuda")
        self._cache = {}
        if wait:
            self.wait()

    def wait(self):
        if self._pending:
            if capturing():
                raise RuntimeError("tf2_gnn_amd: a batch's edges cannot be bucketed inside a hipGraph capture (the build reads "
                                   "sizes back); run the step eagerly once on the same adjacency tensors first (CapturedStep warmup)")
            self._pending = False
            self._keep = None
            try:
                _lib.check(_lib.load().tfgnn_graph_wait(self._h))
            except Exception:
                self.close()
                raise
        return self

    def ensure(self, parts: int) -> "Graph":
        if parts & ~self.parts:
            self.wait()
            _lib.check(_lib.load().tfgnn_graph_ensure(self._h, int(parts), _stream()))
            self.parts |= int(parts)
        return self

    def array(self, array_id: int) -> torch.Tensor:
        if array_id in self._cache:
            return self._cache[array_id]
        self.ensure(_array_parts(array_id))
        lib = _lib.load()
        p = ctypes.c_void_p()
        n = ctypes.c_int64()
        _lib.check(lib.tfgnn_graph_array(self._h, array_id, ctypes.byref(p), ctypes.byref(n)))
        if n.value == 0 or not p.value:
            dt = torch.float32 if array_id in _FLOAT_ARRAYS else torch.uint8 if array_id in _BYTE_ARRAYS else torch.int32
            t = torch.empty(0, dtype=dt, device=self.device)
        else:
            typestr = "<f4" if array_id in _FLOAT_ARRAYS else "|u1" if array_id in _BYTE_ARRAYS else "<i4"
            t = torch.as_tensor(_DevArray(p.value, n.value, typestr, self), device=self.device)
        self._cache[array_id] = t
        return t

    def nonempty_offsets(self, by_src: bool):
        key = ("nz_off", bool(by_src))
        off = self._cache.get(key)
        if off is None:
# ... 1510 lines not shown
    b0, N = b_cols if b_cols is not None else (0, b.cols)
    K = a.rows
    if out is None:
        if scatter is not None or accumulate:
            raise ValueError("scatter / accumulate need out")
        out = torch.empty((M, N), dtype=torch.float32, device=a.data.device)
    if not out.is_contiguous() or out.numel() != M * N:
        raise ValueError(f"out must be contiguous with {M * N} elements")
    gr, sg, sr, sc = scatter if scatter is not None else (M, 0, N, 1)
    ws_bytes = (lib.tfgnn_sp_gemm_tn_wide_workspace_bytes if wide else lib.tfgnn_sp_gemm_tn_workspace_bytes)(M, N, K, a.cols, a.scale_block)
    ws = _workspace(a.data.device, ws_bytes + 256) if ws_bytes else None
    ws_ptr, ws_len = None, 0
    if ws is not None:
        off = (-ws.data_ptr()) % 256
        ws_ptr, ws_len = ctypes.c_void_p(ws.data_ptr() + off), ws.numel() - off
    _lib.check(
        (lib.tfgnn_sp_gemm_tn_wide if wide else lib.tfgnn_sp_gemm_tn)(
            M, N, K, _ptr(a.data), a.data.stride(0), a0, _ptr(a.inv_scale), a.cols, a.scale_block, _ptr(b.data),
            b.data.stride(0), b0, _ptr(b.inv_scale), _ptr(out), gr, sg, sr, sc, int(accumulate), ws_ptr, ws_len, _stream(),
        )
    )
    return out


def tensor_inv_scale(bound: torch.Tensor) -> torch.Tensor:
    lib = _lib.load()
    out = torch.empty(1, dtype=torch.float32, device=bound.device)
    _lib.check(lib.tfgnn_sp_inv_scale_from_bound(_ptr(bound.contiguous()), _ptr(out), _stream()))
    return out


def absmax(x: torch.Tensor, scale: float = 1.0) -> torch.Tensor:
    lib = _lib.load()
    _require_dev(x, torch.float32, "x")
    x = x.contiguous()
    out = torch.zeros(1, dtype=torch.float32, device=x.device)
    _lib.check(lib.tfgnn_absmax(_ptr(x), x.numel(), float(scale), _ptr(out), _stream()))
    return out


_sp_weight_cache: "dict" = {}
_CHECK_WEIGHT_CACHE = [None]


def clear_weight_operand_cache() -> None:
    _sp_weight_cache.clear()


def notify_weights_changed(tensor: Optional[torch.Tensor] = None) -> None:
    aux_flush()
    if tensor is None:
        _sp_weight_cache.clear()
        return
    base = tensor._base if tensor._base is not None else tensor
    lo = base.data_ptr()
    hi = lo + base.numel() * base.element_size()
    for key in [k for k in _sp_weight_cache if lo <= k[0] < hi]:
        del _sp_weight_cache[key]


def _weight_key(w: torch.Tensor, kind: str):
    return (w.data_ptr(), tuple(w.shape), tuple(w.stride()), kind)


def _weight_checksum(w: torch.Tensor):
    if _CHECK_WEIGHT_CACHE[0] is None:
        import os

        _CHECK_WEIGHT_CACHE[0] = os.environ.get("TFGNN_CHECK_WEIGHT_CACHE", "0") == "1"
    if not _CHECK_WEIGHT_CACHE[0]:
        return None
    v = w.detach().double()
    return (float(v.sum()), float(v.abs().sum()))


def sp_weight_operand(w: torch.Tensor, kind: str, build):
    op = _cached_weight_operand(w, kind)
    if op is None:
        op = build()
        _cache_weight_operand(w, kind, op)
    return op


def _cached_weight_operand(w: torch.Tensor, kind: str):
    hit = _sp_weight_cache.get(_weight_key(w, kind))
    if hit is not None and hit[0] == w._version and hit[2]() is not None:
        if hit[3] is not None and hit[3] != _weight_checksum(w):
            raise RuntimeError("a weight tensor changed without a version bump (update through .data or a raw pointer?): "
                               "call Variable.mark_updated() / ops.notify_weights_changed() after such an update")
        return hit[1]
    if hit is not None:
        aux_flush()
    return None


def _cache_weight_operand(w: torch.Tensor, kind: str, op) -> None:
    import weakref

    if len(_sp_weight_cache) > 256:
        _sp_weight_cache.clear()
    base = w._base if w._base is not None else w
    _sp_weight_cache[_weight_key(w, kind)] = (w._version, op, weakref.ref(base), _weight_checksum(w))
```

Measured before the change: 375.6 million edges/s.

## Fuse long-row combine into gather kernel via arrival counters; presplit weights in batch

Removes the separate combine kernel and the deferred combine aux job for multi-chunk long rows. Each chunk of a long row now bumps a per-row arrival counter, and the last chunk to arrive reads the partials and writes the quantized output inside the gather kernel itself. This saves a launch and a pass over the partials, at the cost of atomics and cross-workgroup visibility concerns. Separately, all weight split operands for a forward or backward walk are built up front and flushed in one aux batch, rather than split lazily per layer.

```diff
diff --git a/include/tfgnn.h b/include/tfgnn.h
--- a/include/tfgnn.h
+++ b/include/tfgnn.h
@@ -108,7 +108,8 @@
   TFGNN_G_PATTERN_NODE_BY_DST = 28,
   TFGNN_G_PATTERN_TILEMASK_BY_DST = 29,
   TFGNN_G_PATTERN_NODE_BY_SRC = 30,
-  TFGNN_G_PATTERN_TILEMASK_BY_SRC = 31
+  TFGNN_G_PATTERN_TILEMASK_BY_SRC = 31,
+  TFGNN_G_GATHER_ARRIVALS_VIEW0 = 32
 } tfgnn_graph_array_id;
 
 int tfgnn_graph_array(const tfgnn_graph* graph, int array_id, const void** d_ptr, int64_t* count);
diff --git a/tf2_gnn_amd/csrc/aux_jobs.hip b/tf2_gnn_amd/csrc/aux_jobs.hip
--- a/tf2_gnn_amd/csrc/aux_jobs.hip
+++ b/tf2_gnn_amd/csrc/aux_jobs.hip
@@ -54,11 +54,6 @@
       col_absmax_body(a, b);
       break;
     }
-    case AUX_COMBINE_SP: {
-      const AuxCombineSp a = aux_payload<AuxCombineSp>(j);
-      combine_sp_body(a, b);
-      break;
-    }
     default:
       break;
   }
@@ -76,7 +71,7 @@
     while (i < num_jobs && t.n < AUX_MAX_JOBS) {
       const tfgnn_aux_job& j = jobs[i++];
       if (j.kind == AUX_NONE || j.num_blocks == 0) continue;
-      TFGNN_REQUIRE(j.kind == AUX_SPLIT_ROWS || j.kind == AUX_SPLIT_COLS || j.kind == AUX_COMBINE_SP || j.kind == AUX_COL_ABSMAX,
+      TFGNN_REQUIRE(j.kind == AUX_SPLIT_ROWS || j.kind == AUX_SPLIT_COLS || j.kind == AUX_COL_ABSMAX,
                     "tfgnn_aux_launch: unknown job kind %d", j.kind);
       t.j[t.n++] = j;
       blocks += j.num_blocks;
diff --git a/tf2_gnn_amd/csrc/aux_jobs.hpp b/tf2_gnn_amd/csrc/aux_jobs.hpp
--- a/tf2_gnn_amd/csrc/aux_jobs.hpp
+++ b/tf2_gnn_amd/csrc/aux_jobs.hpp
@@ -9,7 +9,7 @@
 
 namespace tfgnn {
 
-enum AuxKind { AUX_NONE = 0, AUX_SPLIT_ROWS = 1, AUX_SPLIT_COLS = 2, AUX_COMBINE_SP = 4, AUX_COL_ABSMAX = 6 };
+enum AuxKind { AUX_NONE = 0, AUX_SPLIT_ROWS = 1, AUX_SPLIT_COLS = 2, AUX_COL_ABSMAX = 6 };
 
 struct AuxSplitRows {
   const float* src;
@@ -51,20 +51,7 @@
   int64_t slab;
   int ref_ld;
 };
-struct AuxCombineSp {
-  const int32_t *multi_row, *multi_base, *multi_n;
-  int num_multi;
-  const float* row_scale;
-  const float* partial;
-  int width;
-  const int32_t* out_row_map;
-  uint8_t* out_sp;
-  int64_t ld_out_sp;
-  float* inv_out;
-  const float* fixed_inv;
-};
-static_assert(sizeof(AuxSplitRows) <= sizeof(((tfgnn_aux_job*)0)->payload) && sizeof(AuxSplitCols) <= sizeof(((tfgnn_aux_job*)0)->payload) &&
-                  sizeof(AuxCombineSp) <= sizeof(((tfgnn_aux_job*)0)->payload),
+static_assert(sizeof(AuxSplitRows) <= sizeof(((tfgnn_aux_job*)0)->payload) && sizeof(AuxSplitCols) <= sizeof(((tfgnn_aux_job*)0)->payload),
               "tfgnn_aux_job payload too small");
 
 template <class P>
@@ -276,53 +263,4 @@
   }
 }
 
-__device__ __forceinline__ void combine_sp_body(const AuxCombineSp& a, unsigned block) {
-  const int m = (int)block * 4 + (threadIdx.x >> 6);
-  if (m >= a.num_multi) return;
-  const int lane = threadIdx.x & 63;
-  const int64_t row = a.multi_row[m];
-  const int32_t base = a.multi_base[m], n = a.multi_n[m];
-  const float rs = a.row_scale ? a.row_scale[row] : 1.f;
-  float4 sum[8];
-  float mx = 0.f;
-#pragma unroll
-  for (int i = 0; i < 8; ++i) {
-    const int c = (lane + i * 64) * 4;
-    sum[i] = make_float4(0.f, 0.f, 0.f, 0.f);
-    if (c < a.width) {
-      int k = 0;
-      for (; k + 4 <= n; k += 4) {
-        float4 p[4];
-#pragma unroll
-        for (int u = 0; u < 4; ++u) p[u] = *reinterpret_cast<const float4*>(a.partial + (int64_t)(base + k + u) * a.width + c);
-#pragma unroll
-        for (int u = 0; u < 4; ++u) { sum[i].x += p[u].x; sum[i].y += p[u].y; sum[i].z += p[u].z; sum[i].w += p[u].w; }
-      }
-      for (; k < n; ++k) {
-        const float4 p = *reinterpret_cast<const float4*>(a.partial + (int64_t)(base + k) * a.width + c);
-        sum[i].x += p.x; sum[i].y += p.y; sum[i].z += p.z; sum[i].w += p.w;
-      }
-      sum[i].x *= rs; sum[i].y *= rs; sum[i].z *= rs; sum[i].w *= rs;
-      mx = fmaxf(mx, fmaxf(fmaxf(fabsf(sum[i].x), fabsf(sum[i].y)), fmaxf(fabsf(sum[i].z), fabsf(sum[i].w))));
-    }
-  }
-  const int64_t orow = a.out_row_map ? a.out_row_map[row] : row;
-  float iv, sc;
-  if (a.fixed_inv) {
-    iv = a.fixed_inv[0];
-    sc = 1.f / iv;
-  } else {
-#pragma unroll
-    for (int o = 32; o; o >>= 1) mx = fmaxf(mx, __shfl_xor(mx, o, 64));
-    sc = sp_scale_for_max(mx, &iv);
-    if (lane == 0) a.inv_out[orow] = iv;
-  }
-  uint8_t* drow = a.out_sp + orow * a.ld_out_sp;
-#pragma unroll
-  for (int i = 0; i < 8; ++i) {
-    const int c = (lane + i * 64) * 4;
-    if (c < a.width) sp_store4(drow, c, sum[i], sc);
-  }
-}
-
-}
+}
diff --git a/tf2_gnn_amd/csrc/graph.hip b/tf2_gnn_amd/csrc/graph.hip
--- a/tf2_gnn_amd/csrc/graph.hip
+++ b/tf2_gnn_amd/csrc/graph.hip
@@ -349,7 +349,8 @@
   int64_t R;
   int thr, chunk;
   int32_t* counters;
-  int32_t *item_row, *item_chunk, *item_slot, *multi_row, *multi_base, *multi_n;
+  int32_t *item_row, *item_chunk, *item_slot, *item_multi, *multi_row, *multi_base, *multi_n;
+  uint32_t* arrive;
   int32_t *bin_count, *bin_cursor, *short_rows;
   int want_items;
 };
@@ -360,25 +361,28 @@
 __device__ __forceinline__ void plan_rows_body(const int32_t* __restrict__ rowptr, int64_t R, int long_threshold, int chunk_edges,
                                  int32_t* __restrict__ counters,
                                  int32_t* __restrict__ item_row, int32_t* __restrict__ item_chunk,
-                                 int32_t* __restrict__ item_slot, int32_t* __restrict__ multi_row,
-                                 int32_t* __restrict__ multi_base, int32_t* __restrict__ multi_n) {
+                                 int32_t* __restrict__ item_slot, int32_t* __restrict__ item_multi,
+                                 int32_t* __restrict__ multi_row, int32_t* __restrict__ multi_base,
+                                 int32_t* __restrict__ multi_n, uint32_t* __restrict__ arrive) {
   for (int64_t r = (int64_t)blockIdx.x * blockDim.x + threadIdx.x; r < R; r += (int64_t)gridDim.x * blockDim.x) {
     const int32_t len = rowptr[r + 1] - rowptr[r];
     if (len <= long_threshold) continue;
     const int32_t n = (len + chunk_edges - 1) / chunk_edges;
     const int32_t base = atomicAdd(&counters[0], n);
-    int32_t pb = -1;
+    int32_t pb = -1, m = -1;
     if (n > 1) {
-      const int32_t m = atomicAdd(&counters[1], 1);
+      m = atomicAdd(&counters[1], 1);
       pb = atomicAdd(&counters[2], n);
       multi_row[m] = (int32_t)r;
       multi_base[m] = pb;
       multi_n[m] = n;
+      for (int w = 0; w < ARRIVE_WINDOWS; ++w) arrive[(size_t)m * ARRIVE_WINDOWS + w] = 0u;
     }
     for (int32_t i = 0; i < n; ++i) {
       item_row[base + i] = (int32_t)r;
       item_chunk[base + i] = i;
       item_slot[base + i] = n > 1 ? pb + i : -1;
+      item_multi[base + i] = m;
     }
   }
 }
@@ -412,8 +416,8 @@
   if ((blockIdx.y >> 1) == 0) {
     short_hist_body(j.rowptr, j.R, j.thr, j.bin_count, j.counters + 3, h, n_short);
   } else if (j.want_items) {
-    plan_rows_body(j.rowptr, j.R, j.thr, j.chunk, j.counters, j.item_row, j.item_chunk, j.item_slot, j.multi_row, j.multi_base,
-                   j.multi_n);
+    plan_rows_body(j.rowptr, j.R, j.thr, j.chunk, j.counters, j.item_row, j.item_chunk, j.item_slot, j.item_multi, j.multi_row,
+                   j.multi_base, j.multi_n, j.arrive);
   }
 }
 
@@ -759,8 +763,8 @@
     j.thr = pl.long_threshold;
     j.chunk = pl.item_chunk_edges;
     j.counters = counters + 16 + 4 * v;
-    j.item_row = pl.item_row; j.item_chunk = pl.item_chunk; j.item_slot = pl.item_slot;
-    j.multi_row = pl.multi_row; j.multi_base = pl.multi_base; j.multi_n = pl.multi_n;
+    j.item_row = pl.item_row; j.item_chunk = pl.item_chunk; j.item_slot = pl.item_slot; j.item_multi = pl.item_multi;
+    j.multi_row = pl.multi_row; j.multi_base = pl.multi_base; j.multi_n = pl.multi_n; j.arrive = pl.arrive;
     j.bin_count = bins + (size_t)v * 2 * SHORT_BINS;
     j.bin_cursor = j.bin_count + SHORT_BINS;
     j.short_rows = pl.short_rows;
@@ -985,10 +989,11 @@
   const int min_long = std::min(std::min(view_long[0], view_long[1]), std::min(view_long[2], view_long[3]));
   const int min_chunk = std::min(std::min(view_chunk[0], view_chunk[1]), std::min(view_chunk[2], view_chunk[3]));
   const size_t max_items = (size_t)(E / min_long + 1), max_multi = (size_t)(E / min_chunk + 1);
-  size_t o_item[4][3], o_multi[4][3];
+  size_t o_item[4][4], o_multi[4][3], o_arrive[4];
   for (int v = 0; v < 4; ++v) {
-    for (int k = 0; k < 3; ++k) o_item[v][k] = plan.take(max_items * 4);
+    for (int k = 0; k < 4; ++k) o_item[v][k] = plan.take(max_items * 4);
     for (int k = 0; k < 3; ++k) o_multi[v][k] = plan.take(max_multi * 4);
+    o_arrive[v] = plan.take(max_multi * ARRIVE_WINDOWS * 4);
   }
   size_t o_short[4];
   for (int v = 0; v < 4; ++v) o_short[v] = plan.take((size_t)((v & 1) ? V : R) * 4 + 4);
@@ -1073,6 +1078,8 @@
     pl.item_row = (int32_t*)(slab + o_item[v][0]);
     pl.item_chunk = (int32_t*)(slab + o_item[v][1]);
     pl.item_slot = (int32_t*)(slab + o_item[v][2]);
+    pl.item_multi = (int32_t*)(slab + o_item[v][3]);
+    pl.arrive = (uint32_t*)(slab + o_arrive[v]);
     pl.multi_row = (int32_t*)(slab + o_multi[v][0]);
     pl.multi_base = (int32_t*)(slab + o_multi[v][1]);
     pl.multi_n = (int32_t*)(slab + o_multi[v][2]);
@@ -1375,6 +1382,8 @@
     if (array_id == TFGNN_G_EID_BY_DST || array_id == TFGNN_G_EID_BY_SRC) need = TFGNN_GRAPH_PART_EDGE_IDS;
     if (array_id >= TFGNN_G_PATTERN_POS_BY_DST && array_id <= TFGNN_G_PATTERN_TILEMASK_BY_SRC) need = TFGNN_GRAPH_PART_DST_PATTERN;
     if (array_id >= TFGNN_G_NZ_CPOS_BY_DST && array_id <= TFGNN_G_NZ_COL_BY_SRC) need = TFGNN_GRAPH_PART_COMPACT;
+    if (array_id >= TFGNN_G_GATHER_ARRIVALS_VIEW0 && array_id <= TFGNN_G_GATHER_ARRIVALS_VIEW0 + 3)
+      need = ((array_id - TFGNN_G_GATHER_ARRIVALS_VIEW0) & 1) ? TFGNN_GRAPH_PART_PLAN_NODE : TFGNN_GRAPH_PART_PLAN_TYPED;
     if (need) {
       const int rc = tfgnn::graph_require_parts(g, need, "tfgnn_graph_array");
       if (rc) return rc;
@@ -1413,6 +1422,11 @@
       *d_ptr = g->compact[array_id >= TFGNN_G_NZ_CPOS_BY_SRC].nodeptr_nz; *count = g->V + 1; break;
     case TFGNN_G_NZ_COL_BY_DST: case TFGNN_G_NZ_COL_BY_SRC:
       *d_ptr = g->compact[array_id >= TFGNN_G_NZ_CPOS_BY_SRC].col_nz; *count = g->compact[array_id >= TFGNN_G_NZ_CPOS_BY_SRC].num_nz; break;
+    case TFGNN_G_GATHER_ARRIVALS_VIEW0: case TFGNN_G_GATHER_ARRIVALS_VIEW0 + 1: case TFGNN_G_GATHER_ARRIVALS_VIEW0 + 2:
+    case TFGNN_G_GATHER_ARRIVALS_VIEW0 + 3: {
+      const tfgnn::CsrPlan& pl = g->views[array_id - TFGNN_G_GATHER_ARRIVALS_VIEW0].plan;
+      *d_ptr = pl.arrive; *count = (int64_t)pl.num_multi * tfgnn::ARRIVE_WINDOWS; break;
+    }
     default:
       tfgnn::set_error("unknown graph array id %d", array_id);
       return TFGNN_ERR_INVALID_ARGUMENT;
diff --git a/tf2_gnn_amd/csrc/graph.hpp b/tf2_gnn_amd/csrc/graph.hpp
--- a/tf2_gnn_amd/csrc/graph.hpp
+++ b/tf2_gnn_amd/csrc/graph.hpp
@@ -9,6 +9,7 @@
 constexpr int ITEM_CHUNK = 512;
 constexpr int LONG_ROW_THRESHOLD_TYPED = 48;
 constexpr int ITEM_CHUNK_TYPED = 512;
+constexpr int ARRIVE_WINDOWS = 8;
 
 struct CsrPlan {
   int32_t long_threshold = LONG_ROW_THRESHOLD;
@@ -19,9 +20,11 @@
   int32_t* item_row = nullptr;
   int32_t* item_chunk = nullptr;
   int32_t* item_slot = nullptr;
+  int32_t* item_multi = nullptr;
   int32_t* multi_row = nullptr;
   int32_t* multi_base = nullptr;
   int32_t* multi_n = nullptr;
+  uint32_t* arrive = nullptr;
   int32_t* short_rows = nullptr;
   int32_t num_short = 0;
 };
diff --git a/tf2_gnn_amd/csrc/mp_layer.hip b/tf2_gnn_amd/csrc/mp_layer.hip
--- a/tf2_gnn_amd/csrc/mp_layer.hip
+++ b/tf2_gnn_amd/csrc/mp_layer.hip
@@ -19,17 +19,17 @@
   if (rc) return rc;
   const int64_t D = a->in_dim, H = a->hidden_dim, K = (int64_t)L * D;
   TFGNN_REQUIRE(V > 0 && L > 0 && D > 0 && H > 0, "tfgnn_mp_forward: empty layer");
-  tfgnn_aux_job own[2];
-  std::memset(own, 0, sizeof(own));
-  rc = tfgnn_graph_gather_reduce_sp_deferred(a->graph, a->view, nullptr, nullptr, a->row_scale, a->x, a->ldx, (int)D, a->agg_sp,
-                                             D * 4, a->agg_inv_scale, nullptr, a->workspace, a->workspace_bytes, &own[0], stream);
+  rc = tfgnn_graph_gather_reduce_sp(a->graph, a->view, nullptr, nullptr, a->row_scale, a->x, a->ldx, (int)D, a->agg_sp, D * 4,
+                                    a->agg_inv_scale, nullptr, a->workspace, a->workspace_bytes, stream);
   if (rc) return rc;
   if (a->w) {
-    rc = tfgnn_sp_split_cols_job(a->w, H, K, H, a->wt_sp, a->ld_wt_sp_bytes, a->wt_inv_scale, &own[1]);
+    tfgnn_aux_job job;
+    std::memset(&job, 0, sizeof(job));
+    rc = tfgnn_sp_split_cols_job(a->w, H, K, H, a->wt_sp, a->ld_wt_sp_bytes, a->wt_inv_scale, &job);
+    if (rc) return rc;
+    rc = tfgnn_aux_launch(&job, 1, stream);
     if (rc) return rc;
   }
-  rc = tfgnn_aux_launch(own, 2, stream);
-  if (rc) return rc;
   return tfgnn_sp_gemm_nt_rows(V, H, K, a->agg_sp, K * 4, a->agg_inv_scale, (int)D, nullptr, a->wt_sp, a->ld_wt_sp_bytes, a->wt_inv_scale,
                                a->out, a->ld_out, a->bias, a->act, 0, nullptr, 0, TFGNN_ACT_NONE, nullptr, 0, 1.f, a->out_sp,
                                a->ld_out_sp_bytes, a->out_inv_scale, a->dropout_rate, a->dropout_seed, a->tile_kmask, a->row_map, stream);
@@ -48,18 +48,17 @@
   if (rc) return rc;
   const int64_t D = a->in_dim, H = a->hidden_dim, K = (int64_t)L * H;
   TFGNN_REQUIRE(V > 0 && L > 0 && D > 0 && H > 0, "tfgnn_mp_backward: empty layer");
-  tfgnn_aux_job own[2];
-  std::memset(own, 0, sizeof(own));
-  rc = tfgnn_graph_gather_reduce_sp_deferred(a->graph, TFGNN_VIEW_BY_SRC_TYPED, nullptr, a->edge_weight, nullptr, a->d_pre, a->ld_d_pre,
-                                                 (int)H, a->g_sp, H * 4, a->g_inv_scale, nullptr, a->workspace, a->workspace_bytes, &own[0],
-                                                 stream);
+  rc = tfgnn_graph_gather_reduce_sp(a->graph, TFGNN_VIEW_BY_SRC_TYPED, nullptr, a->edge_weight, nullptr, a->d_pre, a->ld_d_pre, (int)H,
+                                    a->g_sp, H * 4, a->g_inv_scale, nullptr, a->workspace, a->workspace_bytes, stream);
   if (rc) return rc;
   if (a->w) {
-    rc = tfgnn_sp_split_rows_job(a->w, H, H, D * H, D, K, (int)K, a->wh_sp, a->ld_wh_sp_bytes, a->wh_inv_scale, nullptr, &own[1]);
+    tfgnn_aux_job job;
+    std::memset(&job, 0, sizeof(job));
+    rc = tfgnn_sp_split_rows_job(a->w, H, H, D * H, D, K, (int)K, a->wh_sp, a->ld_wh_sp_bytes, a->wh_inv_scale, nullptr, &job);
+    if (rc) return rc;
+    rc = tfgnn_aux_launch(&job, 1, stream);
     if (rc) return rc;
   }
-  rc = tfgnn_aux_launch(own, 2, stream);
-  if (rc) return rc;
   rc = tfgnn_sp_gemm_nt_rows(V, D, K, a->g_sp, K * 4, a->g_inv_scale, (int)H, a->a_rows, a->wh_sp, a->ld_wh_sp_bytes, a->wh_inv_scale, a->dx,
                              a->ld_dx, nullptr, TFGNN_ACT_NONE, a->accumulate, a->mul, a->ld_mul, a->act_of_saved, a->saved, a->ld_saved,
                              a->saved_scale, a->dx_sp, a->ld_dx_sp_bytes, a->dx_inv_scale, a->dropout_rate, a->dropout_seed, a->tile_kmask,
diff --git a/tf2_gnn_amd/csrc/spmm.hip b/tf2_gnn_amd/csrc/spmm.hip
--- a/tf2_gnn_amd/csrc/spmm.hip
+++ b/tf2_gnn_amd/csrc/spmm.hip
@@ -1,7 +1,7 @@
 #include <algorithm>
 #include <cstdlib>
-
-#include "aux_jobs.hpp"
+#include <cstring>
+
 #include "common.hpp"
 #include "graph.hpp"
 #include "sp16.hpp"
@@ -132,17 +132,16 @@
   const int32_t* item_row;
   const int32_t* item_chunk;
   const int32_t* item_slot;
+  const int32_t* item_multi;
   float* partial;
   int item_chunk_edges;
-  const int32_t* multi_row;
   const int32_t* multi_base;
   const int32_t* multi_n;
-  int num_multi;
+  uint32_t* arrive;
   uint8_t* out_sp;
   int64_t ld_out_sp;
   float* inv_out;
   const float* fixed_inv;
-  tfgnn_aux_job* combine_job;
   bool multi_pairs;
 };
 
@@ -471,6 +470,100 @@
           vstore<VEC>(dst + i * LPR * VEC, o);
         }
     }
+  }
+}
+
+typedef unsigned uint4v __attribute__((ext_vector_type(4)));
+__device__ __forceinline__ float4 load_partial4(const GatherArgs& a, int64_t slot, int c) {
+  const __amdgpu_buffer_rsrc_t rs = __builtin_amdgcn_make_buffer_rsrc(a.partial + slot * a.width, (short)0, a.width * 4, 0x00020000);
+  const uint4v v = __builtin_amdgcn_raw_buffer_load_b128(rs, (unsigned)c * 4u, 0, 16 );
+  return make_float4(__uint_as_float(v.x), __uint_as_float(v.y), __uint_as_float(v.z), __uint_as_float(v.w));
+}
+__device__ __forceinline__ float load_partial1(const GatherArgs& a, int64_t slot, int f) {
+  return __hip_atomic_load(a.partial + slot * a.width + f, __ATOMIC_RELAXED, __HIP_MEMORY_SCOPE_AGENT);
+}
+
+__device__ __forceinline__ void combine_sp_row(const GatherArgs& a, int64_t row, int32_t base, int32_t n, float rs, int lane) {
+  float4 sum[8];
+  float mx = 0.f;
+#pragma unroll
+  for (int i = 0; i < 8; ++i) {
+    const int c = (lane + i * 64) * 4;
+    sum[i] = make_float4(0.f, 0.f, 0.f, 0.f);
+    if (c < a.width) {
+      int k = 0;
+      for (; k + 4 <= n; k += 4) {
+        float4 p[4];
+#pragma unroll
+        for (int u = 0; u < 4; ++u) p[u] = load_partial4(a, base + k + u, c);
+#pragma unroll
+        for (int u = 0; u < 4; ++u) { sum[i].x += p[u].x; sum[i].y += p[u].y; sum[i].z += p[u].z; sum[i].w += p[u].w; }
+      }
+      for (; k < n; ++k) {
+        const float4 p = load_partial4(a, base + k, c);
+        sum[i].x += p.x; sum[i].y += p.y; sum[i].z += p.z; sum[i].w += p.w;
+      }
+      sum[i].x *= rs; sum[i].y *= rs; sum[i].z *= rs; sum[i].w *= rs;
+      mx = fmaxf(mx, fmaxf(fmaxf(fabsf(sum[i].x), fabsf(sum[i].y)), fmaxf(fabsf(sum[i].z), fabsf(sum[i].w))));
+    }
+  }
+  const int64_t orow = a.out_row_map ? a.out_row_map[row] : row;
+  float iv, sc;
+  if (a.fixed_inv) {
+    iv = a.fixed_inv[0];
+    sc = 1.f / iv;
+  } else {
+#pragma unroll
+    for (int o = 32; o; o >>= 1) mx = fmaxf(mx, __shfl_xor(mx, o, 64));
+    sc = sp_scale_for_max(mx, &iv);
+    if (lane == 0) a.inv_out[orow] = iv;
+  }
+  uint8_t* drow = a.out_sp + orow * a.ld_out_sp;
+#pragma unroll
+  for (int i = 0; i < 8; ++i) {
+    const int c = (lane + i * 64) * 4;
+    if (c < a.width) sp_store4(drow, c, sum[i], sc);
+  }
+}
+
+__device__ __forceinline__ void combine_fp32_row(const GatherArgs& a, int64_t row, int32_t base, int32_t n, float rs, bool is_max,
+                                                 int f0, int f1) {
+  const int64_t orow = a.out_row_map ? a.out_row_map[row] : row;
+  for (int f = f0 + (int)threadIdx.x; f < f1; f += 256) {
+    float s = load_partial1(a, base, f);
+    for (int k = 1; k < n; ++k) {
+      const float p = load_partial1(a, base + k, f);
+      s = is_max ? fmaxf(s, p) : s + p;
+    }
+    a.out[orow * a.ld_out + f] = act_apply(a.post_act, s * rs);
+  }
+}
+
+template <int WINDOW, bool SP>
+__device__ __forceinline__ void finish_multi_row(const GatherArgs& a, int item, int64_t row, float rs, unsigned window, bool is_max,
+                                                 unsigned* flag) {
+  const int m = a.item_multi[item];
+  const int32_t n = a.multi_n[m];
+  const unsigned windows = gridDim.y;
+  const unsigned cls = window % ARRIVE_WINDOWS;
+  const unsigned sharing = (windows - cls + ARRIVE_WINDOWS - 1) / ARRIVE_WINDOWS;
+  asm volatile("s_waitcnt vmcnt(0)" ::: "memory");
+  __syncthreads();
+  if (threadIdx.x == 0) {
+    uint32_t* ctr = a.arrive + (size_t)m * ARRIVE_WINDOWS + cls;
+    const unsigned old = __hip_atomic_fetch_add(ctr, 1u, __ATOMIC_RELAXED, __HIP_MEMORY_SCOPE_AGENT);
+    const bool last = old == (unsigned)n * sharing - 1u;
+    if (last) __hip_atomic_store(ctr, 0u, __ATOMIC_RELAXED, __HIP_MEMORY_SCOPE_AGENT);
+    *flag = last ? 1u : 0u;
+  }
+  __syncthreads();
+  if (*flag == 0u) return;
+  const int32_t base = a.multi_base[m];
+  if constexpr (SP) {
+    if (threadIdx.x < 64) combine_sp_row(a, row, base, n, rs, (int)threadIdx.x);
+  } else {
+    for (unsigned w = cls; w < windows; w += ARRIVE_WINDOWS)
+      combine_fp32_row(a, row, base, n, rs, is_max, (int)(w * WINDOW), min(a.width, (int)((w + 1) * WINDOW)));
   }
 }
 
@@ -553,37 +646,11 @@
       const int64_t orow = a.out_row_map ? a.out_row_map[row] : row;
       a.out[orow * a.ld_out + w0 + f] = act_apply(a.post_act, s * rs);
     } else {
-      a.partial[(int64_t)slot * a.width + w0 + f] = s;
-    }
-  }
-}
-
-__global__ void __launch_bounds__(256) csr_gather_combine_kernel(GatherArgs a) {
-  const int64_t total = (int64_t)a.num_multi * a.width;
-  for (int64_t i = (int64_t)blockIdx.x * blockDim.x + threadIdx.x; i < total; i += (int64_t)gridDim.x * blockDim.x) {
-    const int m = (int)(i / a.width);
-    const int f = (int)(i - (int64_t)m * a.width);
-    const int64_t row = a.multi_row[m];
-    const int32_t base = a.multi_base[m], n = a.multi_n[m];
-    float s = a.partial[(int64_t)base * a.width + f];
-    for (int k = 1; k < n; ++k) {
-      const float p = a.partial[(int64_t)(base + k) * a.width + f];
-      s = a.is_max ? fmaxf(s, p) : s + p;
-    }
-    const float rs = a.row_scale ? a.row_scale[row] : 1.f;
-    const int64_t orow = a.out_row_map ? a.out_row_map[row] : row;
-    a.out[orow * a.ld_out + f] = act_apply(a.post_act, s * rs);
-  }
-}
-
-static AuxCombineSp combine_sp_args(const GatherArgs& a) {
-  AuxCombineSp c{};
-  c.multi_row = a.multi_row; c.multi_base = a.multi_base; c.multi_n = a.multi_n; c.num_multi = a.num_multi;
-  c.row_scale = a.row_scale; c.partial = a.partial; c.width = a.width; c.out_row_map = a.out_row_map;
-  c.out_sp = a.out_sp; c.ld_out_sp = a.ld_out_sp; c.inv_out = a.inv_out; c.fixed_inv = a.fixed_inv;
-  return c;
-}
-__global__ void __launch_bounds__(256) csr_gather_combine_sp_kernel(AuxCombineSp a) { combine_sp_body(a, blockIdx.x); }
+      __hip_atomic_store(a.partial + (int64_t)slot * a.width + w0 + f, s, __ATOMIC_RELAXED, __HIP_MEMORY_SCOPE_AGENT);
+    }
+  }
+  if (slot >= 0) finish_multi_row<WINDOW, SP>(a, item, row, rs, window, is_max, reinterpret_cast<unsigned*>(&red[0][0]));
+}
 
 template <int LPR, int VPL, int VEC, int UNROLL, int MODE, bool SP = false>
 __global__ void __launch_bounds__(256) csr_gather_reduce_kernel(GatherArgs a, int num_items) {
@@ -633,25 +700,12 @@
     if (!multi_done)
       hipLaunchKernelGGL((csr_gather_reduce_kernel<LPR, VPL, VEC, UNROLL, MODE, true>), dim3(units, 1), block, 0, s, a, num_items);
     TFGNN_LAUNCH_CHECK();
-    if (a.num_multi > 0) {
-      if (a.combine_job) {
-        aux_job_set(a.combine_job, AUX_COMBINE_SP, (unsigned)ceil_div(a.num_multi, 4), combine_sp_args(a));
-      } else {
-        hipLaunchKernelGGL(csr_gather_combine_sp_kernel, dim3((unsigned)ceil_div(a.num_multi, 4)), block, 0, s, combine_sp_args(a));
-        TFGNN_LAUNCH_CHECK();
-      }
-    }
     return TFGNN_OK;
   }
   if (!multi_done)
     hipLaunchKernelGGL((csr_gather_reduce_kernel<LPR, VPL, VEC, UNROLL, MODE>), dim3(units, windows), block, 0, s, a,
                        num_items);
   TFGNN_LAUNCH_CHECK();
-  if (a.num_multi > 0) {
-    const int64_t total = (int64_t)a.num_multi * a.width;
-    hipLaunchKernelGGL(csr_gather_combine_kernel, dim3((unsigned)std::min<int64_t>(ceil_div(total, 256), 4096)), block, 0, s, a);
-    TFGNN_LAUNCH_CHECK();
-  }
   return TFGNN_OK;
 }
 
@@ -792,8 +846,7 @@
   a.row_scale = d_row_scale; a.num_rows = gv.num_rows; a.in = d_in; a.ld_in = ld_in; a.width = width;
   a.out = d_out; a.ld_out = d_out_sp ? (int64_t)width : ld_out; a.pre_act = pre_act; a.post_act = post_act;
   a.out_sp = (uint8_t*)d_out_sp; a.ld_out_sp = ld_out_sp; a.inv_out = d_inv_scale; a.fixed_inv = d_fixed_inv;
-  a.combine_job = combine_job;
-  if (combine_job) combine_job->kind = 0, combine_job->num_blocks = 0;
+  if (combine_job) memset(combine_job, 0, sizeof(*combine_job));
   a.is_max = reduce_op == TFGNN_REDUCE_MAX; a.ew_heads = ew_heads; a.head_width = width / ew_heads;
   a.long_threshold = p.long_threshold;
   a.out_row_map = out_map;
@@ -805,9 +858,9 @@
     a.dot_rows = d_dot_rows; a.ld_dot = ld_dot; a.dot_out = d_dot_out; a.dot_pos = d_dot_pos;
     a.dot_lph_log2 = 31 - __builtin_clz((unsigned)lph);
   }
-  a.item_row = p.item_row; a.item_chunk = p.item_chunk; a.item_slot = p.item_slot;
+  a.item_row = p.item_row; a.item_chunk = p.item_chunk; a.item_slot = p.item_slot; a.item_multi = p.item_multi;
   a.partial = (float*)d_workspace; a.item_chunk_edges = p.item_chunk_edges;
-  a.multi_row = p.multi_row; a.multi_base = p.multi_base; a.multi_n = p.multi_n; a.num_multi = p.num_multi;
+  a.multi_base = p.multi_base; a.multi_n = p.multi_n; a.arrive = p.arrive;
   a.short_rows = p.short_rows;
   a.num_short = p.num_short;
   if (compact_nz >= 0) a.num_short = std::max<int64_t>(0, (int64_t)p.num_short - (gv.num_rows - compact_nz));
diff --git a/tf2_gnn_amd/layers/gnn.py b/tf2_gnn_amd/layers/gnn.py
--- a/tf2_gnn_amd/layers/gnn.py
+++ b/tf2_gnn_amd/layers/gnn.py
@@ -194,6 +194,24 @@
             return False
         return ops.get_gemm_mode() == ops.GEMM_F16X2 and in_dim % 16 == 0 and in_dim >= 32 and ops.sp_tiles(out_dim)
 
+    def _presplit_weights(self, graph, V: int, backward: bool, need_input_grad: bool = False) -> None:
+        if V <= 0 or ops.get_gemm_mode() != ops.GEMM_F16X2 or not ops.aux_enabled() or ops.env("TFGNN_PRESPLIT", "1") == "0":
+            return
+        H = self._hidden_dim
+        reqs = []
+        dense = [self._initial_projection_layer] + [self._dense_layers[k] for k in sorted(self._dense_layers, key=int)]
+        for i, w in enumerate(dense):
+            d_in, d_out = w.value.shape
+            if not self._dense_f16x2(d_in, d_out):
+                continue
+            if not backward:
+                reqs.append((w.value, "cols", lambda w=w: ops.sp_split_cols(w.value, defer=True)))
+            elif ops.sp_tiles(d_in) and (i > 0 or need_input_grad):
+                reqs.append((w.value, "rows", lambda w=w: ops.sp_split_rows(w.value, defer=True)))
+        for mp in self._mp_layers:
+            reqs.extend(mp.weight_operand_requests(graph, V, H, backward))
+        ops.presplit_weight_operands(reqs)
+
     def _dense(self, x, w: Variable, act_name, drop=None):
         if x.shape[0] > 0 and self._dense_f16x2(w.value.shape[0], w.value.shape[1]):
             wt = ops.sp_weight_operand(w.value, "cols", lambda: ops.sp_split_cols(w.value, defer=True))
@@ -274,9 +292,10 @@
                 return None
             return (rate, drop_seed[i])
 
+        self._presplit_weights(graph, V, backward=False)
         cur, pre0, dropped = self._dense(X, self._initial_projection_layer, self._init_act,
                                          drop=drop_for(0, need_all_representations))
-        ctx = {"X": X, "h0": cur, "pre0": pre0, "steps": steps, "h0_scale": (1.0 - rate) if dropped else 1.0,
+        ctx = {"X": X, "graph": graph, "h0": cur, "pre0": pre0, "steps": steps, "h0_scale": (1.0 - rate) if dropped else 1.0,
                "all_representations": need_all_representations}
         last = cur
         all_reprs = [cur]
@@ -453,6 +472,7 @@
         return ops.activation_backward(act, g, spec[1])
 
     def _backward_walk(self, ctx, g, g_is_pre, g_last, extras, need_input_grad):
+        self._presplit_weights(ctx["graph"], int(ctx["X"].shape[0]), backward=True, need_input_grad=need_input_grad)
         for layer_idx in range(self._num_layers - 1, -1, -1):
             st = ctx["steps"][layer_idx]
             mp = self._mp_layers[layer_idx]
diff --git a/tf2_gnn_amd/layers/message_passing/gnn_edge_mlp.py b/tf2_gnn_amd/layers/message_passing/gnn_edge_mlp.py
--- a/tf2_gnn_amd/layers/message_passing/gnn_edge_mlp.py
+++ b/tf2_gnn_amd/layers/message_passing/gnn_edge_mlp.py
@@ -339,6 +339,20 @@
     def _f16x2_eligible(self, V, D, L, H) -> bool:
         return (ops.get_gemm_mode() == ops.GEMM_F16X2 and not self._use_target_state_as_input and L > 0 and V > 0
                 and D % 16 == 0 and D <= 512 and 32 <= H <= 512 and ops.sp_tiles(H) and ops.sp_tiles(D))
+
+    def weight_operand_requests(self, graph, num_nodes: int, in_dim: int, backward: bool):
+        if (not getattr(self, "built", False) or self._user_message_function() or self._path() != "A"
+                or self._use_target_state_as_input or self._compact_opt_in):
+            return []
+        W = self._edge_type_mlps.kernels[0]
+        L, Din, H = (int(v) for v in W.shape)
+        if L != graph.num_edge_types or Din != in_dim or not self._f16x2_eligible(num_nodes, in_dim, L, H):
+            return []
+        if backward:
+            return [(W, "rows", lambda: ops.sp_split_rows(W[0], segments=(H, Din * H, L * H), defer=True))]
+        if messages_per_edge(self, graph, in_dim, H):
+            return []
+        return [(W, "cols", lambda: ops.sp_split_cols(W.view(L * Din, H), defer=True))]
 
     def _forward_A(self, X, g, fuse_act, want_split=False, drop=None):
         if self._use_compact_buckets(g):
diff --git a/tf2_gnn_amd/layers/message_passing/message_passing.py b/tf2_gnn_amd/layers/message_passing/message_passing.py
--- a/tf2_gnn_amd/layers/message_passing/message_passing.py
+++ b/tf2_gnn_amd/layers/message_passing/message_passing.py
@@ -358,6 +358,9 @@
     def recomputes_input_dropout(self, num_nodes: int, in_dim: int, num_edge_types: int) -> bool:
         return False
 
+    def weight_operand_requests(self, graph, num_nodes: int, in_dim: int, backward: bool):
+        return []
+
     def call_with_epilogue(self, inputs: MessagePassingInput, training: bool = False, *, want_split_output: bool = False,
                            output_dropout=None):
         return self(inputs, training=training), False
diff --git a/tf2_gnn_amd/ops.py b/tf2_gnn_amd/ops.py
--- a/tf2_gnn_amd/ops.py
+++ b/tf2_gnn_amd/ops.py
@@ -181,6 +181,7 @@
  G_NZ_OFF_BY_DST, G_NZ_NODEPTR_BY_DST, G_NZ_COL_BY_DST, G_NZ_CPOS_BY_SRC, G_NZ_ROW_BY_SRC, G_NZ_NODE_BY_SRC,
  G_NZ_OFF_BY_SRC, G_NZ_NODEPTR_BY_SRC, G_NZ_COL_BY_SRC, G_PATTERN_POS_BY_DST, G_PATTERN_NODE_BY_DST,
  G_PATTERN_TILEMASK_BY_DST, G_PATTERN_NODE_BY_SRC, G_PATTERN_TILEMASK_BY_SRC) = range(32)
+G_GATHER_ARRIVALS_VIEW0 = 32
 _FLOAT_ARRAYS = {G_INVDEG_BY_DST, G_INVDEG_EDGE_BY_SRC, G_INVDEG_EDGE_BY_DST}
 _BYTE_ARRAYS = {G_PATTERN_TILEMASK_BY_DST, G_PATTERN_TILEMASK_BY_SRC}
 G_PART_PLAN_TYPED, G_PART_PLAN_NODE, G_PART_COMPACT, G_PART_EDGE_MAPS, G_PART_EDGE_IDS, G_PART_DST_PATTERN, G_PARTS_ALL = 1, 2, 4, 8, 16, 32, 63
@@ -197,6 +198,8 @@
         return G_PART_EDGE_IDS
     if G_PATTERN_POS_BY_DST <= array_id <= G_PATTERN_TILEMASK_BY_SRC:
         return G_PART_DST_PATTERN
+    if G_GATHER_ARRIVALS_VIEW0 <= array_id <= G_GATHER_ARRIVALS_VIEW0 + 3:
+        return _VIEW_PARTS[array_id - G_GATHER_ARRIVALS_VIEW0]
     return G_PART_COMPACT if G_NZ_CPOS_BY_DST <= array_id <= G_NZ_COL_BY_SRC else 0
 
 
@@ -1873,6 +1876,21 @@
     return op
 
 
+def presplit_weight_operands(requests) -> int:
+    made, seen = [], set()
+    for w, kind, build in requests:
+        key = _weight_key(w, kind)
+        if key in seen or _cached_weight_operand(w, kind) is not None:
+            continue
+        seen.add(key)
+        made.append((w, kind, build()))
+    if made:
+        aux_flush()
+        for w, kind, op in made:
+            _cache_weight_operand(w, kind, op)
+    return len(made)
+
+
 def _cached_weight_operand(w: torch.Tensor, kind: str):
     hit = _sp_weight_cache.get(_weight_key(w, kind))
     if hit is not None and hit[0] == w._version and hit[2]() is not None:
```

Result: faster. 386.0 million edges/s (median of 6 runs) (+2.8%).
